# knights-lab/UTree

Hardware: AMD Instinct MI355X
Metric: reads classified/sec, 8 GB L2 CTR, 150 bp reads (higher is better)
Workload: dtype u64; 1 GPU; configs[1]: 1.22e+09-node synthetic L2 CTR (k=32, 21844 labels, image 40.8 GiB, fine_bits=8), 1152000000 x 150 bp reads per GPU (72 steps x 16000000-read batches, 41 distinct batches resident in HBM), RC=0

## Files before the change

### utree_amd/csrc/dev_image.c

```c
#define _FILE_OFFSET_BITS 64
#define _GNU_SOURCE
#define __HIP_PLATFORM_AMD__ 1
#include <hip/hip_runtime_api.h>
#include <fcntl.h>
#include <math.h>
#include <stddef.h>
#include <stdio.h>
#include <stdlib.h>
#include <string.h>
#include <unistd.h>
#include "ctr_host.h"
#include "dev_image.h"

#define HIPCHK(x) do { hipError_t e_ = (x); if (e_ != hipSuccess) { utree_dev_set_hip_error((int)e_, #x); rc = e_ == hipErrorOutOfMemory ? UTREE_E_NOMEM : UTREE_E_HIP; goto fail; } } while (0)
#define KCHK(x) do { int e_ = (x); if (e_ != 0) { utree_dev_set_hip_error(e_, #x); rc = e_ == (int)hipErrorOutOfMemory ? UTREE_E_NOMEM : UTREE_E_HIP; goto fail; } } while (0)

static __thread char g_hip_msg[256];
void utree_dev_set_hip_error(int err, const char *what) {
    snprintf(g_hip_msg, sizeof g_hip_msg, "%s (%d) in %s", hipGetErrorString((hipError_t)err), err, what);
    if (getenv("UTREE_DEBUG")) fprintf(stderr, "[utree_amd] HIP error: %s\n", g_hip_msg);
}
const char *utree_last_hip_error(void) { return g_hip_msg; }
void utree_set_error_text(const char *msg) { snprintf(g_hip_msg, sizeof g_hip_msg, "%s", msg); }

// ... 328 lines not shown
    if (e) { utree_dev_set_hip_error(e, "utk_repack"); return UTREE_E_HIP; }
    return UTREE_OK;
}

static int build_finish(builder *b, const void *d_binix_raw) {
    int rc = UTREE_OK;
    utree_dev *d = b->d;
    const utree_ctr *ctr = b->ctr;
    hipStream_t st = b->stream;
    char *img = (char *)d->image;
    uint64_t *recs = (uint64_t *)(img + d->hdr.off_recs);
    void *coarse = img + d->hdr.off_coarse;
    const int off64 = (d->hdr.flags & UTREE_F_OFF64) != 0;
    unsigned long long counters[2] = {0, 0}, invalid = 0;
    HIPCHK(hipMemcpyAsync(&invalid, b->d_invalid, 8, hipMemcpyDeviceToHost, st));
    HIPCHK(hipMalloc((void **)&b->d_counters, 16));
    HIPCHK(hipMemsetAsync(b->d_counters, 0, 16, st));
    KCHK(utk_fill_recs_pad(recs + d->hdr.n_nodes * d->hdr.rec_words, 8 * d->hdr.rec_words, st));
    KCHK(utk_widen_binix(d_binix_raw, ctr->info.binix_width, off64, coarse, st));
    KCHK(utk_validate(d->hdr.W, d->hdr.I, off64, coarse, recs, d->hdr.n_nodes, (uint32_t *)(img + d->hdr.off_irreg),
                      b->d_counters, st));
    HIPCHK(hipMemcpyAsync(counters, b->d_counters, 16, hipMemcpyDeviceToHost, st));
    HIPCHK(hipStreamSynchronize(st));
    if (timing_on()) fprintf(stderr, "[utree_amd] image: bin table checked (%llu irregular bins%s)\n", counters[0], counters[1] ? ", not monotone" : "");
    d->hdr.n_irregular = counters[0];
    if (invalid) d->hdr.flags |= UTREE_F_INVALID_RANKS;
    uint64_t full_bytes = d->hdr.total_bytes;
    if (d->hdr.W == 4) {
        uint64_t c0 = 0, cN = 0;
        if (!counters[1]) {
            if (ctr->info.binix_width == 4) { uint32_t a, z; memcpy(&a, ctr->binix_raw, 4); memcpy(&z, (const char *)ctr->binix_raw + 4 * (size_t)(UTREE_NUMBINS - 1), 4); c0 = a; cN = z; }
            else { memcpy(&c0, ctr->binix_raw, 8); memcpy(&cN, (const char *)ctr->binix_raw + 8 * (size_t)(UTREE_NUMBINS - 1), 8); }
        } else HIPCHK(hipMemsetAsync(img + d->hdr.off_irreg, 0xFF, (1u << 24) / 8, st));
        KCHK(utk_build_direct(d->hdr.I, off64, counters[1] != 0, coarse, recs, d->hdr.n_nodes, c0, cN - c0, (const uint32_t *)(img + d->hdr.off_irreg), counters[0],
                              img + d->hdr.off_table, st));
        HIPCHK(hipStreamSynchronize(st));
        if (counters[1]) d->hdr.flags |= UTREE_F_GENERIC; else if (counters[0]) d->hdr.flags |= UTREE_F_IRREGULAR;
        d->hdr.n_min = 0;
        d->hdr.total_bytes = d->hdr.off_recs;
        if (timing_on()) fprintf(stderr, "[utree_amd] image: direct-address table of 2^32 x %u bytes built (%llu irregular bins%s answered by the reference's probe order)\n",
                                 d->hdr.I, counters[0], counters[1] ? ", bin table not monotone: every bin" : "");
    } else
    if (counters[1]) {
        d->hdr.flags |= UTREE_F_GENERIC;
        d->hdr.fine_bits = 0;
        d->hdr.n_min = 0;
        HIPCHK(hipMemsetAsync(img + d->hdr.off_irreg, 0xFF, (1u << 24) / 8, st));
    } else {
        if (counters[0]) d->hdr.flags |= UTREE_F_IRREGULAR;
        uint64_t c0, cN;
        if (ctr->info.binix_width == 4) { uint32_t a, z; memcpy(&a, ctr->binix_raw, 4); memcpy(&z, (const char *)ctr->binix_raw + 4 * (size_t)(UTREE_NUMBINS - 1), 4); c0 = a; cN = z; }
        else { memcpy(&c0, ctr->binix_raw, 8); memcpy(&cN, (const char *)ctr->binix_raw + 8 * (size_t)(UTREE_NUMBINS - 1), 8); }
        d->hdr.n_min = cN - c0;
        HIPCHK(hipMemsetAsync(b->d_counters, 0, 16, st));
        HIPCHK(hipMemcpyAsync(img, &d->hdr, sizeof d->hdr, hipMemcpyHostToDevice, st));
        {
            uint64_t n_min = 0;
            int views = 0;
            KCHK(utk_build_min(d->hdr.W, d->hdr.I, off64, coarse, recs, c0, d->hdr.n_min, dup_capacity(d->hdr.n_nodes), (const uint64_t *)(img + offsetof(utree_image_header, regions)),
                               d->hdr.regions, d->hdr.n_slots, d->hdr.bucket_words, (uint64_t *)(img + d->hdr.off_table), (uint64_t *)(img + d->hdr.off_mrecs),
                               (uint32_t *)(img + d->hdr.off_irreg), b->d_counters, &n_min, &views, st));
            if (timing_on()) fprintf(stderr, "[utree_amd] image: %llu records for %llu nodes (second views%s)\n", (unsigned long long)n_min, (unsigned long long)d->hdr.n_min, views ? "" : ": too many, none stored");
            d->hdr.n_min = n_min;
            if (views) d->hdr.flags |= UTREE_F_STRAND_VIEWS;
        }
        KCHK(utk_fill_recs_pad((uint64_t *)(img + d->hdr.off_mrecs) + d->hdr.n_min * d->hdr.rec_words, 8 * d->hdr.rec_words, st));
        HIPCHK(hipMemcpyAsync(counters, b->d_counters, 16, hipMemcpyDeviceToHost, st));
        HIPCHK(hipStreamSynchronize(st));
        if (counters[0]) {
            d->hdr.flags |= UTREE_F_IRREGULAR;
            d->hdr.n_irregular += counters[1];
            if (timing_on()) fprintf(stderr, "[utree_amd] image: %llu bucket(s) beyond the overflow descriptor's range: %llu bins take the exact-probe path\n", counters[0], counters[1]);
        }
        {
            uint64_t kept = 0;
            const utree_image_header o = d->hdr;
            int chains = 0;
            KCHK(utk_compact_overflow(o.W, o.I, (uint64_t *)(img + o.off_table), o.n_slots, o.bucket_words, (uint64_t *)(img + o.off_mrecs), &kept, &chains, st));
            if (chains) d->hdr.flags |= UTREE_F_OVF_CHAINS;
            KCHK(utk_fill_recs_pad((uint64_t *)(img + o.off_mrecs) + kept * o.rec_words, 8 * o.rec_words, st));
            utree_image_header *h = &d->hdr;
            const uint64_t coarse_b = (uint64_t)UTREE_NUMBINS * ((o.flags & UTREE_F_OFF64) ? 8 : 4), irreg_b = (1u << 24) / 8;
            const uint64_t loff_b = ((uint64_t)o.n_labels + 1) * 4, blob_b = o.label_blob_bytes + 64, r2i_b = (uint64_t)o.n_labels * 4;
            const uint64_t vote_b = (uint64_t)o.n_labels * sizeof(utk_vote_rec);
            const uint64_t recs_b = (o.n_nodes + 8) * o.rec_words * 8;
            uint64_t off = align_up(o.off_mrecs + (kept + 8) * o.rec_words * 8, 4096);
            h->n_min = kept;
            h->off_coarse = off; off = align_up(off + coarse_b, 256);
            h->off_irreg = off; off = align_up(off + irreg_b, 256);
            h->off_label_off = off; off = align_up(off + loff_b, 256);
            h->off_label_blob = off; off = align_up(off + blob_b, 256);
            h->off_rank2ix = off; off = align_up(off + r2i_b, 256);
            h->off_vote = off; off = align_up(off + vote_b, 4096);
            h->off_recs = off;
            if (h->flags & UTREE_F_IRREGULAR) off = align_up(off + recs_b, 4096);
            h->total_bytes = off;
            if (move_down(img, h->off_coarse, o.off_coarse, coarse_b, st) || move_down(img, h->off_irreg, o.off_irreg, irreg_b, st) ||
                move_down(img, h->off_label_off, o.off_label_off, loff_b, st) || move_down(img, h->off_label_blob, o.off_label_blob, blob_b, st) ||
                move_down(img, h->off_rank2ix, o.off_rank2ix, r2i_b, st) || move_down(img, h->off_vote, o.off_vote, vote_b, st) ||
                ((h->flags & UTREE_F_IRREGULAR) && move_down(img, h->off_recs, o.off_recs, recs_b, st))) { rc = UTREE_E_HIP; goto fail; }
            HIPCHK(hipStreamSynchronize(st));
            if (timing_on()) fprintf(stderr, "[utree_amd] image: %llu of %llu nodes in overflow runs; packed image %.2f GiB (built in %.2f GiB)\n",
                                     (unsigned long long)kept, (unsigned long long)o.n_nodes, (double)h->total_bytes / 1073741824.0, (double)full_bytes / 1073741824.0);
        }
    }
    d->image_bytes = d->hdr.total_bytes;
    HIPCHK(hipMemcpyAsync(img, &d->hdr, sizeof d->hdr, hipMemcpyHostToDevice, st));
    HIPCHK(hipStreamSynchronize(st));
    if (d->owns && d->hdr.total_bytes + ((uint64_t)256 << 20) < full_bytes && !getenv("UTREE_KEEP_BUILD_AREA")) {
        void *small = NULL;
        if (hipMalloc(&small, d->hdr.total_bytes) == hipSuccess) {
            hipError_t e1 = hipMemcpyAsync(small, d->image, d->hdr.total_bytes, hipMemcpyDeviceToDevice, st), e2 = hipStreamSynchronize(st);
            if (e1 == hipSuccess && e2 == hipSuccess) { hipFree(d->image); d->image = small; }
            else { hipFree(small); (void)hipGetLastError(); }
        } else (void)hipGetLastError();
    }
    bind_image(d);
fail:
    if (b->d_counters) hipFree(b->d_counters);
    if (b->d_ix2rank) hipFree(b->d_ix2rank);
    if (b->d_invalid) hipFree(b->d_invalid);
    b->d_counters = NULL; b->d_ix2rank = NULL; b->d_invalid = NULL;
    if (rc) { utree_dev_free(d); b->d = NULL; }
    return rc;
}

int utree_dev_build(const utree_ctr *ctr, int device, int fine_bits, const void *d_binix, const void *d_records,
                    void *d_image, size_t image_bytes, void *stream, utree_dev **out) {
    if (!ctr || !d_binix || !d_records || !out) return UTREE_E_ARG;
    *out = NULL;
    builder b;
    int rc = build_begin(&b, ctr, device, fine_bits, d_image, image_bytes, (hipStream_t)stream);
    if (rc) return rc;
    rc = build_chunk(&b, d_records, 0, ctr->info.n_nodes);
    if (rc) { hipFree(b.d_ix2rank); hipFree(b.d_invalid); utree_dev_free(b.d); return rc; }
    rc = build_finish(&b, d_binix);
    if (rc) return rc;
    *out = b.d;
    return UTREE_OK;
}

static double g_upload_s[4];
int utree_dev_upload_seconds(double *h_out4) {
    if (!h_out4) return UTREE_E_ARG;
    for (int i = 0; i < 4; ++i) h_out4[i] = g_upload_s[i];
    return UTREE_OK;
}

int utree_dev_upload(const utree_ctr *ctr, int device, int fine_bits, utree_dev **out) {
    if (!ctr || !out) return UTREE_E_ARG;
    *out = NULL;
    if (!ctr->path && !ctr->h_records) return UTREE_E_ARG;
    builder b;
    double t0 = now_s();
    int rc = build_begin(&b, ctr, device, fine_bits, NULL, 0, NULL);
    if (rc) return rc;
    double t1 = now_s(), t2 = t1, t3 = t1;
    const size_t SZ = ctr->info.SZ;
    const size_t chunk_recs = ((size_t)128 << 20) / SZ;
    const size_t chunk_bytes = chunk_recs * SZ;
    void *h_pin[2] = {NULL, NULL}, *d_raw[2] = {NULL, NULL}, *d_binix = NULL;
    hipEvent_t ev[2] = {NULL, NULL};
    int fd = -1;
    for (int i = 0; i < 2; ++i) {
        HIPCHK(hipHostMalloc(&h_pin[i], chunk_bytes, hipHostMallocDefault));
        HIPCHK(hipMalloc(&d_raw[i], chunk_bytes));
        HIPCHK(hipEventCreateWithFlags(&ev[i], hipEventDisableTiming));
    }
    if (ctr->path) {
        fd = open(ctr->path, O_RDONLY);
        if (fd < 0) { rc = UTREE_E_IO; goto fail; }
    }
    uint64_t done = 0, N = ctr->info.n_nodes;
    for (int slot = 0; done < N; slot ^= 1) {
        uint64_t cnt = N - done < chunk_recs ? N - done : chunk_recs;
        size_t bytes = (size_t)cnt * SZ;
        HIPCHK(hipEventSynchronize(ev[slot]));
        if (fd >= 0) {
            int T = 8, bad = 0;
            if ((size_t)T > bytes / ((size_t)4 << 20) + 1) T = (int)(bytes / ((size_t)4 << 20) + 1);
#pragma omp parallel for num_threads(T) schedule(static, 1) reduction(| : bad)
            for (int t = 0; t < T; ++t) {
                size_t a = bytes * (size_t)t / (size_t)T, e = bytes * (size_t)(t + 1) / (size_t)T;
                while (a < e) {
                    ssize_t r = pread(fd, (char *)h_pin[slot] + a, e - a, (off_t)(ctr->records_file_off + done * SZ + a));
                    if (r <= 0) { bad |= 1; break; }
                    a += (size_t)r;
                }
            }
            if (bad) { rc = UTREE_E_FORMAT; goto fail; }
        } else memcpy(h_pin[slot], ctr->h_records + done * SZ, bytes);
        HIPCHK(hipMemcpyAsync(d_raw[slot], h_pin[slot], bytes, hipMemcpyHostToDevice, NULL));
        rc = build_chunk(&b, d_raw[slot], done, cnt);
        if (rc) goto fail;
        HIPCHK(hipEventRecord(ev[slot], NULL));
        done += cnt;
    }
    HIPCHK(hipDeviceSynchronize());
    t2 = now_s();
    if (timing_on()) fprintf(stderr, "[utree_amd] image: %llu nodes streamed and repacked in %.3f s\n", (unsigned long long)N, t2 - t1);
    HIPCHK(hipMalloc(&d_binix, (size_t)UTREE_NUMBINS * ctr->info.binix_width));
    HIPCHK(hipMemcpyAsync(d_binix, ctr->binix_raw, (size_t)UTREE_NUMBINS * ctr->info.binix_width, hipMemcpyHostToDevice, NULL));
    rc = build_finish(&b, d_binix);
    t3 = now_s();
    if (timing_on()) fprintf(stderr, "[utree_amd] image: alloc+labels %.3f s, stream+repack nodes %.3f s, validate+sort+table %.3f s\n", t1 - t0, t2 - t1, t3 - t2);
    g_upload_s[0] = t1 - t0; g_upload_s[1] = t2 - t1; g_upload_s[2] = t3 - t2; g_upload_s[3] = t3 - t0;
    if (!rc) *out = b.d;
    b.d = NULL;
fail:
    if (fd >= 0) close(fd);
    hipDeviceSynchronize();
    for (int i = 0; i < 2; ++i) {
        if (h_pin[i]) hipHostFree(h_pin[i]);
        if (d_raw[i]) hipFree(d_raw[i]);
        if (ev[i]) hipEventDestroy(ev[i]);
    }
    if (d_binix) hipFree(d_binix);
    if (rc && b.d) { if (b.d_ix2rank) hipFree(b.d_ix2rank); if (b.d_invalid) hipFree(b.d_invalid); utree_dev_free(b.d); }
    return rc;
}

int utree_dev_image(const utree_dev *dev, void **d_image, size_t *bytes) {
    if (!dev) return UTREE_E_ARG;
    if (d_image) *d_image = dev->image;
    if (bytes) *bytes = dev->image_bytes;
    return UTREE_OK;
}

int utree_dev_attach(const utree_ctr *ctr, int device, void *d_image, size_t bytes, utree_dev **out) {
    int rc = UTREE_OK, n_cu = 0;
    if (!d_image || !out || bytes < UTREE_IMG_HEADER_BYTES || ((uintptr_t)d_image & 127u)) return UTREE_E_ARG;
    *out = NULL;
    if ((rc = device_ok(device, &n_cu))) return rc;
    utree_dev *d = (utree_dev *)calloc(1, sizeof *d);
    if (!d) return UTREE_E_NOMEM;
    d->device = device; d->n_cu = n_cu; d->image = d_image; d->owns = 0;
    lanes_ring_init(d);
    HIPCHK(hipMemcpy(&d->hdr, d_image, sizeof d->hdr, hipMemcpyDeviceToHost));
    if (d->hdr.magic != UTREE_IMG_MAGIC || d->hdr.version != UTREE_IMG_VERSION || d->hdr.total_bytes > bytes ||
        (d->hdr.bucket_words != 8 && d->hdr.bucket_words != 16)) { rc = UTREE_E_FORMAT; goto fail; }
    if (ctr && (ctr->info.W != d->hdr.W || ctr->info.I != d->hdr.I || ctr->info.n_nodes != d->hdr.n_nodes ||
                ctr->info.n_labels != d->hdr.n_labels)) { rc = UTREE_E_ARG; goto fail; }
    d->image_bytes = d->hdr.total_bytes;
    bind_image(d);
    *out = d;
    return UTREE_OK;
fail:
    if (d->lanes_ring) hipHostFree((void *)d->lanes_ring);
    free(d);
    return rc;
}

static void lanes_ring_init(utree_dev *d) {
    void *p = NULL;
    if (hipSetDevice(d->device) == hipSuccess && hipHostMalloc(&p, 128 * sizeof(unsigned long long), hipHostMallocDefault) == hipSuccess) {
        memset(p, 0xFF, 128 * sizeof(unsigned long long));
        d->lanes_ring = (volatile unsigned long long *)p;
    }
}

void utree_dev_free(utree_dev *d) {
    if (!d) return;
    hipSetDevice(d->device);
    if (d->lanes_ring) hipHostFree((void *)d->lanes_ring);
    for (int i = 0; i < d->n_events; ++i) hipEventDestroy(d->events[i]);
    if (d->search_ctx) utree_search_ctx_free(d->search_ctx);
    if (d->owns && d->image) hipFree(d->image);
    if (d->rank_state) hipFree(d->rank_state);
    free(d);
}

int utree_dev_get_info(const utree_dev *d, utree_dev_info *info) {
    if (!d || !info) return UTREE_E_ARG;
    info->fine_bits = d->hdr.fine_bits;
    info->record_bytes = d->hdr.rec_words * 8;
    info->image_bytes = d->image_bytes;
    info->irregular_bins = d->hdr.n_irregular;
    info->generic_mode = (d->hdr.flags & UTREE_F_GENERIC) != 0;
    info->device = d->device;
    info->vote_table = d->kimg.vote_tab != NULL;
    info->lane_pass = utk_lanes_image_ok(&d->kimg) != 0;
    info->bucket_bytes = 8u * d->hdr.bucket_words;
    info->strand_views = (d->hdr.flags & UTREE_F_STRAND_VIEWS) ? 1u : 0u;
    if (d->hdr.flags & UTREE_F_DIRECT) info->bucket_bytes = 0;
    info->overflow_chains = (d->hdr.flags & UTREE_F_OVF_CHAINS) ? 1u : 0u;
    info->pad0 = 0;
    info->overflow_bytes = (d->hdr.flags & UTREE_F_DIRECT) ? 0 : d->hdr.n_min * d->hdr.rec_words * 8;
    return UTREE_OK;
}

#define LONG_BLOCKS_PER_CU 8

static uint32_t mid_limit(void) {
    static uint32_t v = 0;
    if (!v) {
        const char *e = getenv("UTREE_MID_LIMIT");
        v = UTREE_MID_DEFAULT;
        if (e && atoi(e) >= (int)UTREE_SHORT2_CAP && atoi(e) <= (int)UTREE_MID_CAP) v = (uint32_t)atoi(e);
    }
    return v;
}

static int lanes_enabled(void) { const char *e = getenv("UTREE_LANE_PASS"); return !(e && e[0] == '0'); }

static void ring_lock(utree_dev *d) { while (__atomic_test_and_set(&d->ring_busy, __ATOMIC_ACQUIRE)) ; }
static void ring_unlock(utree_dev *d) { __atomic_clear(&d->ring_busy, __ATOMIC_RELEASE); }

static void ring_collect(utree_dev *d) {
    if (!d->lanes_ring) return;
    ring_lock(d);
    for (unsigned i = 0; i < 64; ++i) {
        const unsigned long long left = d->lanes_ring[2 * i], err = d->lanes_ring[2 * i + 1];
        if (left == ~0ull || err == ~0ull) continue;
        d->lanes_ring[2 * i] = ~0ull; d->lanes_ring[2 * i + 1] = ~0ull;
        d->ring_inflight[i] = 0;
        if (err && !d->dev_error) d->dev_error = err;
        if (timing_on()) fprintf(stderr, "[utree_amd] batch report: %llu of %u reads left by the lane pass, error word %llu\n", left, d->lanes_ring_reads[i], err);
        if (d->lanes_ring_reads[i]) {
            if (left * 4 <= d->lanes_ring_reads[i]) { unsigned long long n = 0, l = 0; for (unsigned w = 0; w < UTREE_LANES_WINDOW; ++w) { n += d->win_reads[w]; l += d->win_left[w]; }
                if (n >= (1u << 18) && l * 4 > n) { memset(d->win_left, 0, sizeof d->win_left); memset(d->win_reads, 0, sizeof d->win_reads); } }
            const unsigned w = d->win_next++ % UTREE_LANES_WINDOW;
            d->win_left[w] = left; d->win_reads[w] = d->lanes_ring_reads[i];
        }
        d->lanes_ring_reads[i] = 0;
    }
    ring_unlock(d);
}
static int lanes_worth(utree_dev *d) {
    unsigned long long n = 0, l = 0;
    ring_lock(d);
    for (unsigned w = 0; w < UTREE_LANES_WINDOW; ++w) { n += d->win_reads[w]; l += d->win_left[w]; }
    int go = !(n >= (1u << 18) && l * 4 > n);
    if (!go && (++d->lanes_skipped & 7u) == 0) go = 1;
    ring_unlock(d);
    return go;
}
static int ring_post(utree_dev *d, const utk_workspace *w, uint32_t lane_reads, hipStream_t st) {
    if (!d->lanes_ring) return 0;
    ring_lock(d);
    unsigned slot = 64;
    for (unsigned k = 0; k < 64; ++k) {
        const unsigned c = (d->lanes_ring_next + k) & 63u;
        if (!d->ring_inflight[c]) { slot = c; break; }
    }
    if (slot < 64) { d->lanes_ring_next = slot + 1; d->ring_inflight[slot] = 1; d->lanes_ring_reads[slot] = lane_reads; }
    ring_unlock(d);
    if (slot == 64) {
        unsigned long long two[2] = {0, 0};
        if (hipMemcpyAsync(two, w->cursors + UTREE_CUR_MID, 16, hipMemcpyDeviceToHost, st) != hipSuccess || hipStreamSynchronize(st) != hipSuccess) return 1;
        ring_lock(d);
        if (two[1] && !d->dev_error) d->dev_error = two[1];
        ring_unlock(d);
        ring_collect(d);
        return 0;
    }
    if (hipMemcpyAsync((void *)&d->lanes_ring[2 * slot], w->cursors + UTREE_CUR_MID, 16, hipMemcpyDeviceToHost, st) != hipSuccess) {
        ring_lock(d);
        d->ring_inflight[slot] = 0; d->lanes_ring_reads[slot] = 0;
        ring_unlock(d);
        return 1;
    }
    return 0;
}

int utree_classify_poll(utree_dev *d) {
    if (!d) return UTREE_E_ARG;
    ring_collect(d);
    ring_lock(d);
    const unsigned long long e = d->dev_error;
    d->dev_error = 0;
    ring_unlock(d);
    if (e) {
        snprintf(g_hip_msg, sizeof g_hip_msg, "a batch's kernels reported error %llu (%s)", e,
                 e == UTREE_DEVERR_TALLY_CAP ? "tally lists beyond the workspace: total_bases / max_len did not describe the batch" :
                 e == UTREE_DEVERR_LONG_CAP ? "more long reads than the workspace holds" :
                 e == UTREE_DEVERR_PIECES_CAP ? "more pieces of long reads than the workspace holds" : "unknown");
        return UTREE_E_DEVICE;
    }
    return UTREE_OK;
}

static uint32_t lanes_long_min(const utree_dev *d, int do_rc) {
    const uint32_t a = utk_lanes_max_len(&d->kimg), b = do_rc ? (UTREE_MID_CAP - 1u) / 2u : UTREE_MID_CAP;
    return (a < b ? a : b) + 1u;
}

static void carve(const utree_dev *d, void *ws, uint32_t n_reads, uint64_t total_bases, uint32_t max_len, int do_rc,
                  utk_workspace *w, size_t *bytes) {
    uint64_t off = 0;
    char *b = (char *)ws;
    w->cursors = (unsigned long long *)(b + off); off = align_up(off + UTREE_CURSOR_BYTES, 256);
    const uint64_t waves_per_cu = 32 + 20 + 5 * 12;
    w->tally_cap = ((do_rc ? 2 : 1) * total_bases + (uint64_t)n_reads) * 9 / 8 + (uint64_t)d->n_cu * waves_per_cu * UTREE_TALLY_CHUNK + 4096;
    { const char *e = getenv("UTREE_TEST_TALLY_CAP"); if (e && atoll(e) > 0 && (uint64_t)atoll(e) < w->tally_cap) w->tally_cap = (uint64_t)atoll(e); }
    { uint64_t room = w->tally_cap; if (room < UTREE_TALLY_CHUNK) room = UTREE_TALLY_CHUNK; if (room < d->hdr.n_labels) room = d->hdr.n_labels;
      w->tally = (uint64_t *)(b + off); off = align_up(off + room * 8, 256); }
    w->long_list = (uint32_t *)(b + off); off = align_up(off + (uint64_t)n_reads * 4, 256);
    w->mid_list = (uint32_t *)(b + off); off = align_up(off + (uint64_t)n_reads * 4, 256);
    uint64_t max_total = do_rc ? 2 * (uint64_t)max_len + 1 : max_len;
    w->long_blocks = 0; w->hist = NULL; w->touch = NULL;
    w->short_cap = max_total > UTREE_SHORT_CAP ? UTREE_SHORT2_CAP : UTREE_SHORT_CAP;
    w->mid_reads = max_total > w->short_cap;
    w->mid_limit = mid_limit();
    const int lanes_img = utk_lanes_image_ok(&d->kimg);
    if (max_total > w->mid_limit || (lanes_img && max_len > utk_lanes_max_len(&d->kimg))) {
        w->long_blocks = (uint32_t)d->n_cu * LONG_BLOCKS_PER_CU;
        if (w->long_blocks > n_reads) w->long_blocks = n_reads;
        w->hist = (uint32_t *)(b + off); off = align_up(off + (uint64_t)w->long_blocks * d->hdr.n_labels * 4, 256);
        w->touch = (uint32_t *)(b + off); off = align_up(off + (uint64_t)w->long_blocks * ((d->hdr.n_labels + 31) / 32) * 4, 256);
    }
    w->pieces = NULL; w->ltab_rank = w->ltab_cnt = w->lflag = w->long_left = NULL; w->n_long_cap = 0; w->ltally_base = 0;
    w->cls_list = NULL; w->cls_stride = 0; w->n_pieces_cap = 0;
    if (lanes_img && max_len > UTREE_LANES_CAP) {
        w->cls_stride = (n_reads + 63u) & ~63u;
        w->cls_list = (uint32_t *)(b + off); off = align_up(off + (uint64_t)5 * w->cls_stride * 4, 256);
    }
    if (lanes_img && w->long_blocks) {
        uint64_t cap = total_bases / lanes_long_min(d, do_rc) + 1;
        if (cap > n_reads) cap = n_reads;
        const uint64_t piece_windows = 16ull * (UTREE_LANES_CAP - 4 * d->hdr.W + 1);
        const uint64_t n_pieces = total_bases / piece_windows + cap + 1;
        w->n_long_cap = (uint32_t)cap;
        w->n_pieces_cap = n_pieces;
        w->pieces = (uint64_t *)(b + off); off = align_up(off + n_pieces * 8, 256);
        w->ltab_rank = (uint32_t *)(b + off); off = align_up(off + cap * UTREE_LONG_SLOTS * 4, 256);
        w->ltab_cnt = (uint32_t *)(b + off); off = align_up(off + cap * UTREE_LONG_SLOTS * 4, 256);
        w->lflag = (uint32_t *)(b + off); off = align_up(off + cap * 4, 256);
        w->long_left = (uint32_t *)(b + off); off = align_up(off + cap * 4, 256);
        w->ltally_base = (uint64_t)((uint64_t *)(b + off) - w->tally); off = align_up(off + cap * UTREE_LONG_SLOTS * 8, 256);
        { const char *e = getenv("UTREE_TEST_LONG_CAP"); if (e && atoll(e) > 0 && (uint64_t)atoll(e) < w->n_long_cap) w->n_long_cap = (uint32_t)atoll(e); }
        { const char *e = getenv("UTREE_TEST_PIECES_CAP"); if (e && atoll(e) > 0 && (uint64_t)atoll(e) < w->n_pieces_cap) w->n_pieces_cap = (uint64_t)atoll(e); }
    }
    *bytes = (size_t)off;
}

size_t utree_classify_workspace_bytes(const utree_dev *dev, uint32_t n_reads, uint64_t total_bases, uint32_t max_len, int do_rc) {
    if (!dev) return 0;
    utk_workspace w; size_t bytes;
    carve(dev, NULL, n_reads, total_bases, max_len, do_rc, &w, &bytes);
    return bytes;
}

int utree_classify_batch(utree_dev *d, const uint8_t *d_bases, const uint64_t *d_off, const uint32_t *d_len,
                         uint32_t n_reads, uint64_t total_bases, uint32_t max_len, int do_rc, utree_result *d_out,
                         void *d_workspace, size_t workspace_bytes, void *stream) {
    int rc = UTREE_OK;
    if (!d || !d_out || (!d_workspace && n_reads)) return UTREE_E_ARG;
    if (!n_reads) return UTREE_OK;
    if (!d_bases || !d_off || !d_len) return UTREE_E_ARG;
    hipStream_t st = (hipStream_t)stream;
    utk_workspace w; size_t need;
    carve(d, d_workspace, n_reads, total_bases, max_len, do_rc, &w, &need);
    if (workspace_bytes < need) return UTREE_E_ARG;
    HIPCHK(hipSetDevice(d->device));
    HIPCHK(hipMemsetAsync(w.cursors, 0, UTREE_CURSOR_BYTES, st));
    if (w.long_blocks) {
        HIPCHK(hipMemsetAsync(w.hist, 0, (size_t)w.long_blocks * d->hdr.n_labels * 4, st));
        HIPCHK(hipMemsetAsync(w.touch, 0, (size_t)w.long_blocks * ((d->hdr.n_labels + 31) / 32) * 4, st));
    }
    hipEvent_t e0 = NULL, e1 = NULL;
    int tslot = -1;
    if (__atomic_load_n(&d->timing_on, __ATOMIC_ACQUIRE)) {
        tslot = __atomic_fetch_add(&d->n_claimed, 1, __ATOMIC_RELAXED);
        if (tslot >= 0 && tslot < UTREE_MAX_PENDING && 2 * tslot + 1 < d->n_events) { e0 = d->events[2 * tslot]; e1 = d->events[2 * tslot + 1]; }
        else tslot = -1;
    }
    ring_collect(d);
    const int lanes = lanes_enabled() && utk_lanes_image_ok(&d->kimg) && lanes_worth(d);
    if (lanes) {
        const int mixed = max_len > UTREE_LANES_CAP;
        d->last_long = w.long_blocks != 0; d->last_mid = 0; d->last_rc = do_rc; d->last_short_cap = w.short_cap;
        d->last_lanes = utk_lanes_segs(&d->kimg, max_len); d->last_mixed = mixed; d->last_pieces = w.long_blocks != 0;
        if (e0 && !w.long_blocks) HIPCHK(hipEventRecord(e0, st));
        if (!mixed) KCHK(utk_classify_lanes(&d->kimg, d_bases, d_off, d_len, n_reads, max_len, do_rc, d_out, &w, d->n_cu, st));
        else KCHK(utk_classify_lanes_mixed(&d->kimg, d_bases, d_off, d_len, n_reads, max_len, do_rc, d_out, &w, d->n_cu, st));
        if (w.long_blocks) {
            if (e0) HIPCHK(hipEventRecord(e0, st));
            HIPCHK(hipMemsetAsync(w.ltab_rank, 0xFF, (size_t)w.n_long_cap * UTREE_LONG_SLOTS * 4, st));
            HIPCHK(hipMemsetAsync(w.ltab_cnt, 0, (size_t)w.n_long_cap * UTREE_LONG_SLOTS * 4, st));
            HIPCHK(hipMemsetAsync(w.lflag, 0, (size_t)w.n_long_cap * 4, st));
            KCHK(utk_classify_long_pieces(&d->kimg, d_bases, d_off, d_len, do_rc, d_out, &w, d->n_cu, st));
            utk_workspace wl = w;
            wl.long_list = w.long_left;
            wl.long_blocks = w.long_blocks >= 8 ? w.long_blocks / 8 : 1;
            KCHK(utk_classify_long(&d->kimg, d_bases, d_off, d_len, do_rc, d_out, &wl, d->n_cu, st));
            if (e0) { HIPCHK(hipEventRecord(e1, st)); d->recorded[tslot] = 1; }
        }
        KCHK(utk_classify_listed(&d->kimg, d_bases, d_off, d_len, n_reads, max_len, do_rc, d_out, &w, d->n_cu, st));
        if (e0 && !w.long_blocks) { HIPCHK(hipEventRecord(e1, st)); d->recorded[tslot] = 1; }
    } else {
        const int dominant = w.long_blocks ? 2 : (w.mid_reads ? 1 : 0);
        d->last_long = dominant == 2; d->last_mid = dominant == 1; d->last_rc = do_rc; d->last_short_cap = w.short_cap;
        d->last_lanes = 0; d->last_mixed = 0; d->last_pieces = 0;
        if (w.mid_reads) KCHK(utk_route(d_len, n_reads, do_rc, &w, st));
        if (e0 && dominant == 0) HIPCHK(hipEventRecord(e0, st));
        KCHK(utk_classify_short(&d->kimg, d_bases, d_off, d_len, n_reads, do_rc, d_out, &w, d->n_cu, st));
        if (e0 && dominant == 0) { HIPCHK(hipEventRecord(e1, st)); d->recorded[tslot] = 1; }
        if (w.mid_reads) {
            if (e0 && dominant == 1) HIPCHK(hipEventRecord(e0, st));
            KCHK(utk_classify_mid(&d->kimg, d_bases, d_off, d_len, n_reads, do_rc, d_out, &w, d->n_cu, st));
            if (e0 && dominant == 1) { HIPCHK(hipEventRecord(e1, st)); d->recorded[tslot] = 1; }
        }
        if (w.long_blocks) {
            if (e0) HIPCHK(hipEventRecord(e0, st));
            KCHK(utk_classify_long(&d->kimg, d_bases, d_off, d_len, do_rc, d_out, &w, d->n_cu, st));
            if (e0) { HIPCHK(hipEventRecord(e1, st)); d->recorded[tslot] = 1; }
        }
    }
    KCHK(utk_vote(&d->kimg, d_out, &w, n_reads, st));
    if (ring_post(d, &w, lanes ? n_reads : 0, st)) { (void)hipGetLastError(); }
    { ring_lock(d); const unsigned long long pe = d->dev_error; ring_unlock(d);
      if (pe) { rc = UTREE_E_DEVICE; snprintf(g_hip_msg, sizeof g_hip_msg, "an earlier batch's kernels reported error %llu: utree_classify_poll returns (and clears) it", pe); } }
#ifdef UTREE_LANES_TIMERS
    { extern void utk_lanes_phase_dump(void); static int lcalls; if (++lcalls == 6) utk_lanes_phase_dump(); }
#endif
#ifdef UTREE_PHASE_TIMERS
    { extern void utk_phase_dump(void); static int calls; if (++calls == 12) utk_phase_dump(); }
#endif
fail:
    return rc;
}

int utree_lookup_words(utree_dev *d, const uint64_t *d_hi, const uint64_t *d_lo, uint64_t n, uint32_t *d_ix, void *stream) {
    int rc = UTREE_OK;
    if (!d || !d_lo || !d_ix) return UTREE_E_ARG;
    if (d->hdr.W == 16 && !d_hi) return UTREE_E_ARG;
    HIPCHK(hipSetDevice(d->device));
    KCHK(utk_lookup(&d->kimg, d_hi, d_lo, n, d_ix, (hipStream_t)stream));
fail:
    return rc;
}

const char *utree_classify_kernel_name(const utree_dev *dc) {
    if (!dc) return "";
    utree_dev *d = (utree_dev *)dc;
    if (d->last_lanes && d->last_pieces) {
        snprintf(d->kernel_sig, sizeof d->kernel_sig, "classify_lanes_k<%u, %u, 16, %s, 2, %u, %s>", d->hdr.W, d->hdr.I, d->kimg.irr_n ? "true" : "false", d->hdr.bucket_words / 8,
                 utk_lanes_both_strands(&d->kimg, d->last_rc) ? "true" : "false");
        return d->kernel_sig;
    }
    if (d->last_lanes && d->last_mixed) {
        snprintf(d->kernel_sig, sizeof d->kernel_sig, "classify_lanes_mixed_k<%u, %u, %s, %u, %s>", d->hdr.W, d->hdr.I, d->kimg.irr_n ? "true" : "false",
                 d->hdr.bucket_words / 8, utk_lanes_both_strands(&d->kimg, d->last_rc) ? "true" : "false");
        return d->kernel_sig;
    }
    if (d->last_lanes) {
        snprintf(d->kernel_sig, sizeof d->kernel_sig, "classify_lanes_k<%u, %u, 1, %s, 0, %u, %s>", d->hdr.W, d->hdr.I, d->kimg.irr_n ? "true" : "false",
                 d->hdr.bucket_words / 8, utk_lanes_both_strands(&d->kimg, d->last_rc) ? "true" : "false");
        return d->kernel_sig;
    }
    return d->last_long ? utk_classify_long_name(&d->kimg, d->kernel_sig, sizeof d->kernel_sig)
                        : utk_classify_short_name(&d->kimg, d->last_short_cap ? d->last_short_cap : UTREE_SHORT_CAP, d->last_mid, d->last_rc,
                                                  d->kernel_sig, sizeof d->kernel_sig);
}

int utree_model_counts(utree_dev *d, const uint8_t *d_bases, const uint64_t *d_off, const uint32_t *d_len, uint32_t n_reads,
                       int do_rc, uint64_t *h_counts5, void *stream) {
    int rc = UTREE_OK;
    unsigned long long *dc = NULL;
    if (!d || !d_bases || !d_off || !d_len || !h_counts5) return UTREE_E_ARG;
    HIPCHK(hipSetDevice(d->device));
    HIPCHK(hipMalloc((void **)&dc, 64));
    HIPCHK(hipMemsetAsync(dc, 0, 64, (hipStream_t)stream));
    KCHK(utk_model_counts(&d->kimg, d_bases, d_off, d_len, n_reads, do_rc, dc, stream));
    HIPCHK(hipMemcpyAsync(h_counts5, dc, 40, hipMemcpyDeviceToHost, (hipStream_t)stream));
    HIPCHK(hipStreamSynchronize((hipStream_t)stream));
fail:
    if (dc) hipFree(dc);
    return rc;
}

int utree_classify_kernel_time(utree_dev *d, int reset, double *ms_total, uint64_t *launches) {
    int rc = UTREE_OK;
    if (!d) return UTREE_E_ARG;
    HIPCHK(hipSetDevice(d->device));
    int claimed = __atomic_load_n(&d->n_claimed, __ATOMIC_RELAXED);
    if (claimed > UTREE_MAX_PENDING) claimed = UTREE_MAX_PENDING;
    for (int i = 0; i < claimed; ++i) {
        float ms = 0.f;
        if (!d->recorded[i]) continue;
        d->recorded[i] = 0;
        HIPCHK(hipEventSynchronize(d->events[2 * i + 1]));
        HIPCHK(hipEventElapsedTime(&ms, d->events[2 * i], d->events[2 * i + 1]));
        d->ms_total += ms; d->launches++;
    }
    while (d->n_events < 2 * UTREE_MAX_PENDING) { HIPCHK(hipEventCreate((hipEvent_t *)&d->events[d->n_events])); d->n_events++; }
    __atomic_store_n(&d->n_claimed, 0, __ATOMIC_RELAXED);
    if (ms_total) *ms_total = d->ms_total;
    if (launches) *launches = d->launches;
    if (reset) { d->ms_total = 0; d->launches = 0; }
    __atomic_store_n(&d->timing_on, 1, __ATOMIC_RELEASE);
fail:
    return rc;
}
```

### utree_amd/csrc/kernels.hip

```cpp
#include <hip/hip_runtime.h>
#include <stdint.h>
#include <stdio.h>
#include <string.h>
#include "device_common.hpp"
#include "wave_common.hpp"

using namespace utk;

namespace {

#ifdef UTREE_PHASE_TIMERS
__device__ unsigned long long g_phase[16];
struct PhaseT { unsigned long long t, acc[12]; };
#define PH_DECL PhaseT ph_; ph_.t = __builtin_readcyclecounter(); for (int q_ = 0; q_ < 12; ++q_) ph_.acc[q_] = 0;
#define TICKP(ph, i) do { const unsigned long long n_ = __builtin_readcyclecounter(); (ph).acc[i] += n_ - (ph).t; (ph).t = n_; } while (0)
#define TICK(i) TICKP(ph_, i)
#define PH_ARG , PhaseT &ph_
#define PH_PASS , ph_
#define PH_WAITVM asm volatile("s_waitcnt vmcnt(0)" ::: "memory")
#else
#define PH_DECL
#define TICK(i)
#define PH_ARG
#define PH_PASS
#define PH_WAITVM
#endif


constexpr uint32_t KEY_TILE = 128;

struct LaneBits {
    const uint32_t *swl;
    uint32_t sh;
};
__device__ __forceinline__ LaneBits lane_bits(const uint32_t *sw, uint32_t lane) {
    LaneBits b;
    const uint32_t r = lane & 15u;
    b.swl = sw + (lane >> 4) - (r == 0 ? 1u : 0u);
    b.sh = (32u - 2u * r) & 31u;
    return b;
}
__device__ __forceinline__ uint32_t mmer_l(const uint32_t *s, uint32_t word, uint32_t sh) {
    return __builtin_amdgcn_alignbit(s[word], s[word + 1], sh);
}

constexpr uint32_t MIN_POS_MASK = (1u << MIN_LOW_BITS) - 1u;
template <int W> struct MinWin { static constexpr uint32_t FIRST = UTREE_MIN_MARGIN(W), NEXT = (W == 16) ? 13u : 1u; };
template <int W, uint32_t NCH>
__device__ __forceinline__ void build_minkeys_n(const uint32_t *s, uint32_t sh, uint32_t *Kl, uint32_t *Hl, uint64_t *Ob, uint32_t lane) {
    uint32_t x[NCH];
#pragma unroll
    for (uint32_t c = 0; c < NCH; ++c) x[c] = mmer_l(s, 4 * c, sh);
    uint32_t lo = lane;
    asm volatile("" : "+v"(lo));
#pragma unroll
    for (uint32_t c = 0; c < NCH; ++c) {
        uint32_t o;
        const uint32_t h = canon_hash(x[c], o);
        Kl[c * 64] = ((h & ~MIN_POS_MASK) | lo) + c * 64;
        Hl[c * 64] = h;
        Ob[c] = __builtin_amdgcn_ballot_w64(o != 0u);
    }
    Kl[NCH * 64] = ~0u;
    wave_lds_fence();
#pragma unroll
    for (uint32_t st = 1; st <= ((W == 16) ? 16u : 8u); st <<= 1) {
        uint32_t a[NCH], b[NCH];
#pragma unroll
        for (uint32_t c = 0; c < NCH; ++c) { a[c] = Kl[c * 64]; b[c] = Kl[c * 64 + st]; }
        wave_lds_fence();
#pragma unroll
        for (uint32_t c = 0; c < NCH; ++c) Kl[c * 64] = b[c] < a[c] ? b[c] : a[c];
        wave_lds_fence();
    }
}
template <int W, uint32_t TILE>
__device__ __forceinline__ void build_minkeys(const uint32_t *s, uint32_t sh, uint32_t *Kl, uint32_t *Hl, uint64_t *Ob, uint32_t npos, uint32_t lane) {
    constexpr uint32_t MAXCH = (TILE + 4 * W - 16 + 63) / 64;
    static_assert(MAXCH <= 5, "tile too large");
    const uint32_t nch = (npos + 63) >> 6;
    if (nch <= 1) build_minkeys_n<W, 1>(s, sh, Kl, Hl, Ob, lane);
    else if (nch == 2) build_minkeys_n<W, 2>(s, sh, Kl, Hl, Ob, lane);
    else if (nch == 3 || MAXCH == 3) build_minkeys_n<W, 3>(s, sh, Kl, Hl, Ob, lane);
    else if (nch == 4) build_minkeys_n<W, MAXCH >= 4 ? 4 : 3>(s, sh, Kl, Hl, Ob, lane);
    else build_minkeys_n<W, MAXCH >= 5 ? 5 : 3>(s, sh, Kl, Hl, Ob, lane);
}

struct RegionLds { const uint64_t *reg; uint64_t table; uint32_t bshift; };

template <int W, int I, bool EXC, typename OFF, uint32_t TILE, bool CHECKBAD, typename HitFn>
__device__ __forceinline__ void wave_scan_windows(const utk_image &im, const LaneBits &lb, const uint64_t *sbad, uint64_t *Kk,
                                                  uint32_t w0, uint32_t n, const RegionLds &rg, uint32_t lane, HitFn &&on_rank PH_ARG) {
    constexpr uint32_t K = 4 * W;
    if constexpr (W == 4) {
        for (uint32_t it = 0; it * 64 < n; ++it) {
            bool ok = lane < n - it * 64;
            if constexpr (CHECKBAD) {
                const uint32_t ch = (w0 + it * 64) >> 6;
                const uint64_t b0 = sbad[ch], b1 = sbad[ch + 1];
                const uint64_t x = (b0 >> lane) | (lane ? (b1 << (64u - lane)) : 0ull);
                ok = ok && ((uint32_t)x & 0xFFFFu) == 0u;
            }
            uint32_t rank = INVALID;
            if (ok) rank = direct_rank<I>(im, mmer_l(lb.swl + ((w0 + it * 64) >> 4), 0, lb.sh));
            on_rank(rank);
        }
        return;
    }
    static_assert(TILE + 64 <= (1u << MIN_LOW_BITS), "tile positions must fit the key's position field");
    uint32_t *Kp = (uint32_t *)Kk;
    uint32_t *Kl = Kp + lane, *Hl = Kp + (TILE + 128) + lane;
    const uint32_t *Hh = Kp + (TILE + 128);
    uint64_t *Ob = Kk + (TILE + 128) - 8;
    static_assert(((TILE + 4 * W - 16 + 63) / 64) * 64 + 16 <= TILE + 128, "the ballots share the hash area");
    const uint32_t nlane = 0u - lane;
    for (uint32_t wb = 0; wb < n; wb += TILE) {
        const uint32_t tn = n - wb < TILE ? n - wb : TILE;
        const uint32_t *st = lb.swl + ((w0 + wb) >> 4);
        build_minkeys<W, TILE>(st, lb.sh, Kl, Hl, Ob, tn + K - 16, lane);
        TICK(2);
        auto locate = [&](uint32_t it, uint64_t &baddr, uint32_t &tag) {
            const uint32_t *Kr = Kl + it * 64;
            const uint32_t ka = Kr[MinWin<W>::FIRST], kb = Kr[MinWin<W>::FIRST + MinWin<W>::NEXT];
            const uint32_t p = (kb < ka ? kb : ka) & MIN_POS_MASK;
            const uint32_t h = Hh[p];
            const uint32_t o = (uint32_t)(Ob[p >> 6] >> (p & 63u)) & 1u;
            const uint32_t pos = p + nlane - it * 64;
            const uint64_t re = rg.reg[h >> 24];
            uint32_t bl = __umulhi(h << 8, (uint32_t)re & ((1u << UTREE_REGION_NB_BITS) - 1u));
            if constexpr (W == 16) {
                const uint32_t *sr = st + it * 4;
                const uint32_t x0 = mmer_l(sr, 0, lb.sh), x1 = mmer_l(sr, 1, lb.sh), x2 = mmer_l(sr, 2, lb.sh), x3 = mmer_l(sr, 3, lb.sh);
                const unsigned __int128 w = ((unsigned __int128)(((uint64_t)x0 << 32) | x1) << 64) | (((uint64_t)x2 << 32) | x3);
                const uint64_t v = (uint64_t)(w >> (92u - 2u * pos));
                const uint32_t sub = (uint32_t)(re >> UTREE_REGION_NB_BITS) & ((1u << UTREE_REGION_SUB_BITS) - 1u);
                bl = bl * sub + ((ext_canon((uint32_t)((v >> 32) & 0xF0u) | (uint32_t)(v & 0xFu), o) * sub) >> 8);
            }
            baddr = rg.table + ((2u * ((re >> UTREE_REGION_BASE_SHIFT) + bl) + o) << rg.bshift);
            tag = ((h & 0xFFu) << 6) | pos;
        };
        auto resolve = [&](uint32_t it, const Bucket<W, I> &bk, uint64_t baddr, uint32_t tag) -> uint32_t {
            const uint32_t *sr = st + it * 4;
            const uint32_t pos = tag & 63u, hlow = tag >> 6;
            if constexpr (W == 8) {
                const uint32_t x0 = mmer_l(sr, 0, lb.sh), x1 = mmer_l(sr, 1, lb.sh);
                const uint32_t M = (uint32_t)(0xFFFFFFFFull >> (2 * pos));
                const uint32_t rest = x0 ^ ((x0 ^ x1) & M);
                return resolve_bucket8<I, EXC, OFF>(im, bk, baddr, hlow, pos, rest, x0, x1);
            } else {
                const uint32_t x0 = mmer_l(sr, 0, lb.sh), x1 = mmer_l(sr, 1, lb.sh), x2 = mmer_l(sr, 2, lb.sh), x3 = mmer_l(sr, 3, lb.sh);
                const uint64_t wh = ((uint64_t)x0 << 32) | x1, wl = ((uint64_t)x2 << 32) | x3;
                uint32_t rh; uint64_t rl;
                min_rest<W>(wh, wl, pos, rh, rl);
                MinKey<W> mk;
                mk.lo = rl; mk.hi = ((uint64_t)hlow << 38) | ((uint64_t)pos << 32) | rh;
                return resolve_bucket<W, I, EXC, OFF>(im, bk, baddr, mk, wh, wl);
            }
        };
        auto window_ok = [&](uint32_t it, uint32_t left) -> bool {
            bool ok = lane < left;
            if constexpr (CHECKBAD) {
                const uint32_t ch = (w0 + wb + it * 64) >> 6;
                const uint64_t b0 = sbad[ch], b1 = sbad[ch + 1];
                const uint64_t x = (b0 >> lane) | (lane ? (b1 << (64u - lane)) : 0ull);
                ok = ok && ((K == 64) ? (x == 0) : ((uint32_t)x == 0));
            }
            return ok;
        };
        for (uint32_t it = 0; it * 64 < tn; ++it) {
            const bool ok = window_ok(it, tn - it * 64);
            uint64_t baddr = 0; uint32_t tag = 0;
            Bucket<W, I> bk;
            if (ok) { locate(it, baddr, tag); bk = load_bucket_at<W, I>(baddr); }
            TICK(3);
            PH_WAITVM;
            TICK(4);
            uint32_t rank = INVALID;
            if (ok) rank = resolve(it, bk, baddr, tag);
            TICK(5);
            on_rank(rank);
            TICK(6);
        }
        wave_lds_fence();
    }
}

__device__ __forceinline__ void stage_regions(const utk_image &im, uint64_t *s_reg) {
    for (uint32_t x = threadIdx.x; x < 256; x += blockDim.x) s_reg[x] = im.regions[x];
    __syncthreads();
}

__device__ __forceinline__ unsigned long long reserve_tally(const utk_workspace &ws, unsigned long long n) {
    unsigned long long nb = atomicAdd(&ws.cursors[0], n);
    if (nb + n > ws.tally_cap) { ws.cursors[UTREE_CUR_ERROR] = UTREE_DEVERR_TALLY_CAP; nb = 0; }
    return nb;
}

__device__ __forceinline__ void store_result(utree_result *out, uint32_t label, int32_t cut, uint32_t found,
                                             uint32_t uix, uint32_t sl, uint32_t ol) {
    uint32_t *o = (uint32_t *)out;
    uint32_t v0 = label, v1 = (uint32_t)cut, v2 = found, v3 = uix, v4 = sl, v5 = ol;
    asm volatile("" : "+v"(v0), "+v"(v1), "+v"(v2), "+v"(v3), "+v"(v4), "+v"(v5));
    o[0] = v0; o[1] = v1; o[2] = v2; o[3] = v3; o[4] = v4; o[5] = v5;
}

__global__ __launch_bounds__(256) void route_k(const uint32_t *__restrict__ len, uint32_t n_reads, int do_rc, utk_workspace ws) {
    const uint32_t r = blockIdx.x * blockDim.x + threadIdx.x;
    uint64_t total = 0;
    if (r < n_reads) total = do_rc ? 2 * (uint64_t)len[r] + 1 : len[r];
    const bool mid = total > ws.short_cap && total <= ws.mid_limit, lng = total > ws.mid_limit;
    const uint64_t mm = __ballot(mid), ml = __ballot(lng);
    const uint32_t lane = lane_id();
    if (mm) {
        unsigned long long b = 0;
        if (lane == 0) b = atomicAdd(&ws.cursors[UTREE_CUR_MID], (unsigned long long)__popcll(mm));
        b = __shfl(b, 0);
        if (mid) ws.mid_list[b + lanes_below(mm)] = r;
    }
    if (ml) {
        unsigned long long b = 0;
        if (lane == 0) b = atomicAdd(&ws.cursors[UTREE_CUR_LONG], (unsigned long long)__popcll(ml));
        b = __shfl(b, 0);
        if (lng) ws.long_list[b + lanes_below(ml)] = r;
    }
}

template <int CAP> struct RawBuf { static constexpr uint32_t DW = ((CAP / 4 + 1 + 63) / 64) * 64; };

__device__ __forceinline__ uint32_t low_bytes(uint32_t n) {
    return n >= 4u ? 0xFFFFFFFFu : ((1u << (8u * n)) - 1u);
}

template <int CAP>
__device__ __forceinline__ void fetch_raw(const uint8_t *__restrict__ bases, uint64_t o, uint32_t L, uint32_t *raw, uint32_t lane) {
    const uint32_t mf = (uint32_t)(uintptr_t)(bases + o) & 3u;
    const uint32_t nd = (L + mf + 3u) >> 2;
    const uint8_t *p = bases + o - mf;
    for (uint32_t d0 = 0; d0 < nd; d0 += 64) {
        const uint32_t d = d0 + lane;
        if (d < nd) {
            const uint8_t *src = p + 4ull * d;
            const uint32_t dst = (uint32_t)(uintptr_t)(__attribute__((address_space(3))) void *)(raw + 1 + d0);
            asm volatile("s_mov_b32 m0, %1\n\ts_nop 0\n\tglobal_load_lds_dword %0, off" : : "v"(src), "s"(dst) : "memory");
        }
    }
}

template <int CAP>
__device__ __forceinline__ bool stage_read(const uint32_t *raw, uint32_t mf, uint32_t L, uint32_t total, int do_rc,
                                           uint8_t *sb, uint8_t *sbadb, uint32_t lane) {
    constexpr uint32_t DW = RawBuf<CAP>::DW;
    const uint32_t ngroups = (total + 3u) >> 2;
    bool any = false;
    const uint32_t mr = (mf + 2u * L + 1u) & 3u;
    for (uint32_t g0 = 0; g0 < ngroups; g0 += 64) {
        const uint32_t g = g0 + lane;
        const uint32_t gi = g < DW ? g : DW - 1u;
        const uint32_t fm = low_bytes(4u * g < L ? L - 4u * g : 0u);
        uint32_t word = __builtin_amdgcn_alignbyte(raw[2u + gi], raw[1u + gi], mf) & fm;
        uint32_t rm = 0;
        if (do_rc) {
            int32_t i4 = ((int32_t)(mf + 2u * L) - 3 - (int32_t)(4u * g)) >> 2;
            i4 = i4 < -1 ? -1 : (i4 > (int32_t)DW - 1 ? (int32_t)DW - 1 : i4);
            const uint32_t w = __builtin_amdgcn_alignbyte(raw[2 + i4], raw[1 + i4], mr);
            const uint32_t rev = __builtin_amdgcn_perm(0u, w, 0x00010203u);
            const uint32_t from = L + 1u > 4u * g ? L + 1u - 4u * g : 0u, to = 2u * L + 1u > 4u * g ? 2u * L + 1u - 4u * g : 0u;
            rm = low_bytes(to) & ~low_bytes(from);
            word |= rev & rm;
        }
        const uint32_t g2 = (word >> 1) & 0x03030303u;
        const uint32_t letter = __builtin_amdgcn_perm(0u, 0x47544341u, g2);
        const uint32_t z = (word & 0xDFDFDFDFu) ^ letter;
        const uint32_t nz = (((z & 0x7F7F7F7Fu) + 0x7F7F7F7Fu) | z) & 0x80808080u;
        any = any || (nz & low_bytes(total > 4u * g ? total - 4u * g : 0u)) != 0u;
        const uint32_t nib = (nz * 0x00204081u) >> 28;
        const uint32_t nib_next = (uint32_t)__builtin_amdgcn_update_dpp(0, (int)nib, 0x101, 0xF, 0xF, true);
        uint32_t code = g2 ^ ((g2 >> 1) & 0x01010101u);
        code ^= rm & 0x03030303u;
        const uint32_t packed = (code * 0x40100401u) >> 24;
        if (g < ngroups) {
            sb[g ^ 3u] = (uint8_t)packed;
            if (!(lane & 1u)) sbadb[g >> 1] = (uint8_t)(nib | (nib_next << 4));
        }
    }
    return __ballot(any) != 0ull;
}

constexpr int SHORT_CAP = UTREE_SHORT_CAP;
constexpr int SHORT2_CAP = UTREE_SHORT2_CAP;
constexpr int MID_CAP = UTREE_MID_CAP;
constexpr int WAVES_PER_BLOCK = 4;
constexpr uint32_t WORK_GRAB = 32;
constexpr uint32_t TALLY_CHUNK = UTREE_TALLY_CHUNK;
constexpr uint32_t TALLY_DIRECT = UTREE_TALLY_CHUNK / 16;
constexpr int32_t CUT_PENDING = -3;
constexpr int32_t RANK_PENDING = -4;

constexpr int SHORT_MIN_WAVES = 8;
template <int W, int I, bool EXC, typename OFF, int CAP, bool LISTED, int RCMODE = 2>
__global__ __launch_bounds__(256, CAP > SHORT2_CAP ? (I == 2 ? 4 : 3) : (I == 2 ? SHORT_MIN_WAVES : 5))
void classify_short_k(utk_image im, const uint8_t *__restrict__ bases, const uint64_t *__restrict__ off,
                      const uint32_t *__restrict__ len, uint32_t n_reads, int do_rc_arg, utree_result *__restrict__ out,
                      utk_workspace ws) {
    if constexpr (LISTED) { if (!ws.cursors[UTREE_CUR_MID]) return; }
    const int do_rc = RCMODE == 2 ? do_rc_arg : RCMODE;
    constexpr uint32_t K = 4 * W;
    constexpr int NCH = CAP / 64, NWORDS = CAP / 16 + 6;
    __shared__ uint32_t s_words[WAVES_PER_BLOCK][NWORDS + 2];
// ... 31 lines not shown
        const uint32_t total_ = do_rc ? 2 * L_ + 1 : L_;
        asm volatile("s_waitcnt vmcnt(0)" ::: "memory");
        wave_lds_fence();
        const bool any_ = stage_read<CAP>(raw, (uint32_t)(uintptr_t)(bases + o_) & 3u, L_, total_, do_rc, sb, (uint8_t *)sbad, lane);
        if (lane == 0) sbad[(total_ + 63) >> 6] = ~0ull;
        wave_lds_fence();
        return any_;
    };
    auto finish = [&](uint32_t r, uint32_t F) {
            if (F == 0) { if (lane == 0) store_result(&out[r], 0, -2, 0, 0, 0, 0); return; }
            const uint32_t h0 = hits[0];
            if (F == 1) { if (lane == 0) store_result(&out[r], h0, RANK_PENDING, 1, 1, 0, 0); return; }
            if (F <= 64) {
                const bool mine = lane < F;
                const uint32_t hv = mine ? hits[lane] : 0u;
                uint64_t left = __ballot(mine);
                uint32_t nu = 0, myv = 0, myc = 0;
                while (left) {
                    const uint32_t lead = (uint32_t)__builtin_ctzll(left);
                    const uint32_t v = (uint32_t)__builtin_amdgcn_readlane((int)hv, (int)lead);
                    const uint64_t m = __ballot(mine && hv == v) & left;
                    if (lane == nu) { myv = v; myc = (uint32_t)__popcll(m); }
                    ++nu; left &= ~m;
                }
                if (nu == 1) { if (lane == 0) store_result(&out[r], h0, RANK_PENDING, F, 1, 0, 0); return; }
                if (nu > chunk_left) {
                    unsigned long long nb = 0;
                    if (lane == 0) nb = reserve_tally(ws, (unsigned long long)TALLY_CHUNK);
                    chunk_base = uni64(nb);
                    chunk_left = TALLY_CHUNK;
                }
                uint32_t place = 0;
                for (uint32_t u = 0; u < nu; ++u) place += (uint32_t)__builtin_amdgcn_readlane((int)myv, (int)u) < myv;
                if (lane < nu) ws.tally[chunk_base + place] = (uint64_t)myv | ((uint64_t)myc << 32);
                if (lane == 0) store_result(&out[r], 0, CUT_PENDING, F, nu, (uint32_t)chunk_base, (uint32_t)(chunk_base >> 32));
                chunk_base += nu; chunk_left -= nu;
                return;
            }
            uint32_t mn = INVALID, mx = 0;
            for (uint32_t j = lane; j < F; j += 64) { uint32_t h = hits[j]; mn = h < mn ? h : mn; mx = h > mx ? h : mx; }
            mn = wave_min_u32(mn);
            mx = ~wave_min_u32(~mx);
            if (mn == mx) { if (lane == 0) store_result(&out[r], h0, RANK_PENDING, F, 1, 0, 0); return; }
            unsigned long long base;
            const bool direct = (uint32_t)CAP >= TALLY_DIRECT && F >= TALLY_DIRECT;
            if (direct) {
                unsigned long long nb = 0;
                if (lane == 0) nb = reserve_tally(ws, (unsigned long long)F);
                base = uni64(nb);
            } else {
                if (F > chunk_left) {
                    unsigned long long nb = 0;
                    if (lane == 0) nb = reserve_tally(ws, (unsigned long long)TALLY_CHUNK);
                    chunk_base = uni64(nb);
                    chunk_left = TALLY_CHUNK;
                }
                base = chunk_base;
            }
            uint32_t uix = 0, cur = mn;
            for (;;) {
                uint32_t c = 0, nxt = INVALID;
                for (uint32_t j = lane; j < F; j += 64) {
                    uint32_t h = hits[j];
                    c += h == cur;
                    if (h > cur && h < nxt) nxt = h;
                }
                c = wave_sum_u32(c);
                nxt = wave_min_u32(nxt);
                if (lane == 0) ws.tally[base + uix] = (uint64_t)cur | ((uint64_t)c << 32);
                ++uix;
                if (nxt == INVALID) break;
                cur = nxt;
            }
            if (!direct) { chunk_base += uix; chunk_left -= uix; }
            if (lane == 0) store_result(&out[r], 0, CUT_PENDING, F, uix, (uint32_t)base, (uint32_t)(base >> 32));
    };
    uint32_t item = 0, item_end = 0;
    PH_DECL
    bool ahead = false;
    bool bad_cur = true, bad_next = true;
    uint32_t r = 0, L = 0;
    uint64_t o = 0;
    uint32_t grab0 = 0, g_r = 0, g_len = 0;
    uint64_t g_off = 0;
    auto params = [&](uint32_t it_, uint32_t &r_, uint32_t &L_, uint64_t &o_) {
        const int k_ = (int)(it_ - grab0);
        r_ = LISTED ? (uint32_t)__builtin_amdgcn_readlane((int)g_r, k_) : it_;
        L_ = (uint32_t)__builtin_amdgcn_readlane((int)g_len, k_);
        o_ = ((uint64_t)(uint32_t)__builtin_amdgcn_readlane((int)(uint32_t)(g_off >> 32), k_) << 32) |
             (uint32_t)__builtin_amdgcn_readlane((int)(uint32_t)g_off, k_);
    };
    static_assert(WORK_GRAB <= 64, "a grab's parameters live in the lanes of one register");
    for (;;) {
        if (item == item_end) {
            bool got = false;
            while (parts_left) {
                unsigned long long *ctr = parts + part * UTREE_WORK_STRIDE;
                const uint64_t lo = (uint64_t)part * part_len;
                const uint32_t avail = lo >= n_items ? 0u : (uint32_t)(n_items - lo < part_len ? n_items - lo : part_len);
                unsigned long long g = ~0ull;
                if (lane == 0 && __hip_atomic_load(ctr, __ATOMIC_RELAXED, __HIP_MEMORY_SCOPE_AGENT) < avail)
                    g = atomicAdd(ctr, (unsigned long long)WORK_GRAB);
                const uint32_t taken = uni32((uint32_t)(g > 0xFFFFFFFFull ? 0xFFFFFFFFull : g));
                if (taken < avail) {
                    item = (uint32_t)lo + taken;
                    item_end = taken + WORK_GRAB < avail ? item + WORK_GRAB : (uint32_t)lo + avail;
                    got = true;
                    break;
                }
                part = part + 1 == UTREE_WORK_PARTS ? 0 : part + 1;
                --parts_left;
            }
            if (!got) break;
            ahead = false;
            grab0 = item;
            if (item + lane < item_end) {
                g_r = LISTED ? ws.mid_list[item + lane] : item + lane;
                g_len = len[g_r]; g_off = off[g_r];
            }
            TICK(0);
        }
        if (!ahead) {
            params(item, r, L, o);
            if (stageable(L)) { fetch_raw<CAP>(bases, o, L, raw, lane); bad_cur = stage(o, L); }
        }
        ++item;
        ahead = PREFETCH && item < item_end;
        uint32_t r_next = 0, L_next = 0;
        uint64_t o_next = 0;
        bool stage_next = false;
        if (ahead) {
            params(item, r_next, L_next, o_next);
            stage_next = stageable(L_next);
            if (stage_next) fetch_raw<CAP>(bases, o_next, L_next, raw, lane);
        }
        TICK(1);
        const uint64_t total64 = do_rc ? 2 * (uint64_t)L + 1 : L;
        if (total64 <= (uint64_t)CAP) {
            const uint32_t total = (uint32_t)total64;
            uint32_t F = 0;
            if (total >= K) {
                auto on_rank = [&](uint32_t rank) {
                    const bool hit = rank != INVALID;
                    const uint64_t hm = __ballot(hit);
                    if (hit) hits[F + lanes_below(hm)] = (HIT)rank;
                    F += (uint32_t)__popcll(hm);
                };
                if constexpr (RCMODE == 1) wave_scan_windows<W, I, EXC, OFF, TILE, true>(im, lb, sbad, Kk, 0u, total - K + 1, rg, lane, on_rank PH_PASS);
                else if (!bad_cur) wave_scan_windows<W, I, EXC, OFF, TILE, false>(im, lb, sbad, Kk, 0u, total - K + 1, rg, lane, on_rank PH_PASS);
                else wave_scan_windows<W, I, EXC, OFF, TILE, true>(im, lb, sbad, Kk, 0u, total - K + 1, rg, lane, on_rank PH_PASS);
                wave_lds_fence();
            }
            TICK(9);
            if (stage_next) bad_next = stage(o_next, L_next);
            TICK(7);
            finish(r, F);
            TICK(8);
        } else if (stage_next) bad_next = stage(o_next, L_next);
        r = r_next; L = L_next; o = o_next; bad_cur = bad_next;
    }
#ifdef UTREE_PHASE_TIMERS
    if (lane == 0) { for (int q = 0; q < 12; ++q) atomicAdd(&g_phase[q], ph_.acc[q]); atomicAdd(&g_phase[12], 1ull); }
#endif
}

constexpr int LONG_TILE = 2048;
constexpr int LONG_THREADS = 256;
constexpr uint32_t LONG_LDS_BITWORDS = 2048;

template <int W, int I, bool EXC, typename OFF>
__global__ __launch_bounds__(LONG_THREADS, EXC ? 5 : 8) void classify_long_k(utk_image im, const uint8_t *__restrict__ bases,
                                                                const uint64_t *__restrict__ off,
                                                                const uint32_t *__restrict__ len, int do_rc,
                                                                utree_result *__restrict__ out, utk_workspace ws) {
    constexpr uint32_t K = 4 * W;
    constexpr uint32_t STAGE = LONG_TILE + 64;
    __shared__ uint32_t s_words_pad[STAGE / 16 + 8 + 2];
    __shared__ uint64_t s_bad[STAGE / 64 + 2];
    __shared__ uint32_t s_scan[LONG_THREADS / 64 + 1];
    __shared__ uint32_t s_touch[LONG_LDS_BITWORDS];
    __shared__ uint64_t s_keys[LONG_THREADS / 64][KEY_TILE + 128];
    __shared__ unsigned long long s_base;
    __shared__ uint64_t s_reg[256];
    __shared__ uint32_t s_work, s_single;
    const uint32_t tid = threadIdx.x, lane = tid & 63u, wv = uni32(tid >> 6);
    uint32_t *s_words = s_words_pad + 2;
    uint8_t *sb = (uint8_t *)s_words;
    const LaneBits lb = lane_bits(s_words, lane);
    const uint32_t nl = im.n_labels, nbw = (nl + 31) >> 5;
    uint32_t *hist = ws.hist + (size_t)blockIdx.x * nl;
    uint32_t *touch = nbw <= LONG_LDS_BITWORDS ? s_touch : ws.touch + (size_t)blockIdx.x * nbw;
    const uint32_t n_long = (uint32_t)ws.cursors[UTREE_CUR_LONG];
    if (nbw <= LONG_LDS_BITWORDS) for (uint32_t x = tid; x < nbw; x += LONG_THREADS) s_touch[x] = 0;
    stage_regions(im, s_reg);
    const RegionLds rg = {s_reg, (uint64_t)(uintptr_t)im.table, im.bucket_words == 16u ? 7u : 6u};

    for (;;) {
        __syncthreads();
        if (tid == 0) s_work = (uint32_t)atomicAdd(&ws.cursors[UTREE_CUR_WORK_LONG], 1ull);
        __syncthreads();
        const uint32_t li = s_work;
        if (li >= n_long) break;
        const uint32_t r = ws.long_list[li];
        const uint64_t L64 = len[r];
        const uint64_t o = off[r];
        const uint64_t total = do_rc ? 2 * L64 + 1 : L64;
        const uint64_t nwin = total >= K ? total - K + 1 : 0;
        uint32_t my_hits = 0;
        if (tid == 0) s_single = INVALID;
        for (uint64_t w0 = 0; w0 < nwin; w0 += LONG_TILE) {
            constexpr uint32_t NW = LONG_THREADS / 64, PER = (STAGE / 64 + NW - 1) / NW;
            uint32_t rawb[PER];
#pragma unroll
            for (uint32_t q = 0; q < PER; ++q) {
                const uint32_t c = wv + q * NW;
                const uint64_t j = w0 + (uint64_t)c * 64 + lane;
                rawb[q] = 0x200u;
                if (c < STAGE / 64) {
                    if (j < L64) rawb[q] = bases[o + j];
                    else if (j > L64 && j < total) rawb[q] = 0x100u | bases[o + (2 * L64 - j)];
                }
            }
#pragma unroll
            for (uint32_t q = 0; q < PER; ++q) {
                const uint32_t c = wv + q * NW;
                if (c >= STAGE / 64) break;
                uint32_t code = 0; bool bad = true;
                if (!(rawb[q] & 0x200u)) { base_code(rawb[q] & 0xFFu, code, bad); code ^= (rawb[q] >> 8) * 3u; }
                uint64_t bm = __ballot(bad);
                uint32_t t = (code << 2) | (uint32_t)__shfl_down((int)code, 1);
                uint32_t u = (t << 4) | (uint32_t)__shfl_down((int)t, 2);
                if ((lane & 3u) == 0) sb[(c * 16 + (lane >> 2)) ^ 3u] = (uint8_t)u;
                if (lane == 0) s_bad[c] = bm;
            }
            if (tid == 0) s_bad[STAGE / 64] = ~0ull;
            __syncthreads();
            const uint32_t tile_n = (uint32_t)(nwin - w0 < LONG_TILE ? nwin - w0 : LONG_TILE);
            constexpr uint32_t PER_WAVE = LONG_TILE / (LONG_THREADS / 64);
            const uint32_t a = wv * PER_WAVE < tile_n ? wv * PER_WAVE : tile_n;
            const uint32_t b = a + PER_WAVE < tile_n ? a + PER_WAVE : tile_n;
            PH_DECL
            wave_scan_windows<W, I, EXC, OFF, KEY_TILE, true>(im, lb, s_bad, s_keys[wv], a, b - a, rg, lane, [&](uint32_t rank) {
                const bool hit = rank != INVALID;
                uint64_t left = __ballot(hit);
                my_hits += hit;
                while (left) {
                    const uint32_t lead = (uint32_t)__builtin_ctzll(left);
                    const uint32_t v = (uint32_t)__builtin_amdgcn_readlane((int)rank, (int)lead);
                    const uint64_t m = __ballot(hit && rank == v) & left;
                    if (lane == lead) {
                        atomicAdd(&hist[v], (uint32_t)__popcll(m));
                        atomicOr(&touch[v >> 5], 1u << (v & 31u));
                    }
                    left &= ~m;
                }
            } PH_PASS);
            __syncthreads();
        }
        uint32_t f = wave_sum_u32(my_hits);
        if (lane == 0) s_scan[wv] = f;
        __syncthreads();
        uint32_t F = 0;
        for (uint32_t w = 0; w < LONG_THREADS / 64; ++w) F += s_scan[w];
        __syncthreads();
        if (F == 0) { if (tid == 0) store_result(&out[r], 0, -2, 0, 0, 0, 0); continue; }
        const uint32_t per = (nbw + LONG_THREADS - 1) / LONG_THREADS;
        const uint32_t lo = tid * per < nbw ? tid * per : nbw, hi = lo + per < nbw ? lo + per : nbw;
        uint32_t cnt = 0;
        for (uint32_t x = lo; x < hi; ++x) cnt += (uint32_t)__popc(__hip_atomic_load(&touch[x], __ATOMIC_RELAXED, __HIP_MEMORY_SCOPE_AGENT));
        uint32_t inc = cnt;
#pragma unroll
        for (int d = 1; d < 64; d <<= 1) { uint32_t t = __shfl_up(inc, d); if (lane >= (uint32_t)d) inc += t; }
        if (lane == 63) s_scan[wv] = inc;
        __syncthreads();
        uint32_t wbase = 0, uix = 0;
        for (uint32_t w = 0; w < LONG_THREADS / 64; ++w) { if (w < wv) wbase += s_scan[w]; uix += s_scan[w]; }
        uint32_t pos = wbase + inc - cnt;
        if (tid == 0) s_base = uix > 1 ? reserve_tally(ws, (unsigned long long)uix) : 0ull;
        __syncthreads();
        const unsigned long long base = s_base;
        for (uint32_t x = lo; x < hi; ++x) {
            uint32_t bits = __hip_atomic_load(&touch[x], __ATOMIC_RELAXED, __HIP_MEMORY_SCOPE_AGENT);
            if (!bits) continue;
            __hip_atomic_store(&touch[x], 0u, __ATOMIC_RELAXED, __HIP_MEMORY_SCOPE_AGENT);
            while (bits) {
                const uint32_t rk = x * 32 + (uint32_t)__builtin_ctz(bits);
                bits &= bits - 1;
                const uint32_t c = __hip_atomic_load(&hist[rk], __ATOMIC_RELAXED, __HIP_MEMORY_SCOPE_AGENT);
                __hip_atomic_store(&hist[rk], 0u, __ATOMIC_RELAXED, __HIP_MEMORY_SCOPE_AGENT);
                if (uix > 1) ws.tally[base + pos] = (uint64_t)rk | ((uint64_t)c << 32);
                else s_single = rk;
                ++pos;
            }
        }
        __syncthreads();
        if (tid == 0) {
            if (uix == 1) store_result(&out[r], im.rank2ix[s_single], -2, F, 1, 0, 0);
            else store_result(&out[r], 0, CUT_PENDING, F, uix, (uint32_t)base, (uint32_t)(base >> 32));
        }
        __syncthreads();
    }
}

__device__ __forceinline__ uint32_t cut_of(uint32_t x) {
    uint32_t c = x - x / 4;
    c += (x >> 1) >= c;
    return c;
}

__device__ __forceinline__ void label16(const char *s, uint32_t p, uint64_t &x, uint64_t &y) {
    typedef unsigned long long u64x2 __attribute__((ext_vector_type(2), aligned(1)));
    const u64x2 v = *(const u64x2 *)(s + p);
    x = v.x; y = v.y;
}

__device__ __forceinline__ uint64_t stop_flags(uint64_t x1, uint64_t x2) {
    const uint64_t semi = x1 ^ 0x3B3B3B3B3B3B3B3Bull, d = x1 ^ x2;
    uint64_t m = (((x1 - 0x0101010101010101ull) & ~x1) | ((semi - 0x0101010101010101ull) & ~semi)) & 0x8080808080808080ull;
    m |= (((d & 0x7F7F7F7F7F7F7F7Full) + 0x7F7F7F7F7F7F7F7Full) | d) & 0x8080808080808080ull;
    return m;
}

__device__ __forceinline__ void pair_scan(const char *s1, const char *s2, uint32_t start, uint32_t &td, uint32_t &a, uint32_t &b, uint32_t &before) {
    uint32_t base = start, prevlast = start ? (uint32_t)(uint8_t)s1[start - 1] : 0u;
    for (;;) {
        uint64_t x1, y1, x2, y2;
        label16(s1, base, x1, y1); label16(s2, base, x2, y2);
        uint64_t m = stop_flags(x1, x2);
        if (!m) { prevlast = (uint32_t)(x1 >> 56); base += 8; x1 = y1; x2 = y2; m = stop_flags(x1, x2); }
        if (m) {
            const uint32_t idx = (uint32_t)(__builtin_ctzll(m) >> 3);
            td = base + idx;
            a = (uint32_t)(x1 >> (8 * idx)) & 0xFFu; b = (uint32_t)(x2 >> (8 * idx)) & 0xFFu;
            before = idx ? ((uint32_t)(x1 >> (8 * idx - 8)) & 0xFFu) : prevlast;
            return;
        }
        prevlast = (uint32_t)(x1 >> 56); base += 8;
    }
}

struct VRec { uint64_t w[4]; };
__device__ __forceinline__ VRec vrec(const uint64_t *vt, uint32_t rank) {
    typedef unsigned long long u64x2 __attribute__((ext_vector_type(2)));
    const u64x2 *p = (const u64x2 *)(vt + (size_t)rank * 4);
    const u64x2 a = p[0], b = p[1];
    VRec v; v.w[0] = a.x; v.w[1] = a.y; v.w[2] = b.x; v.w[3] = b.y;
    return v;
}
__device__ __forceinline__ uint32_t v_pid(const VRec &v, uint32_t t) { return (uint32_t)((t < 4 ? v.w[0] : v.w[1]) >> (16u * (t & 3u))) & 0xFFFFu; }
__device__ __forceinline__ uint32_t v_end(const VRec &v, uint32_t t) { return (uint32_t)(v.w[2] >> (8u * t)) & 0xFFu; }
__device__ __forceinline__ bool v_exists(const VRec &v, uint32_t t) { return ((uint32_t)v.w[3] >> t) & 1u; }
__device__ __forceinline__ bool v_more(const VRec &v, uint32_t t) { return ((uint32_t)v.w[3] >> (8u + t)) & 1u; }
__device__ __forceinline__ bool v_us(const VRec &v, uint32_t t) { return ((uint32_t)v.w[3] >> (16u + t)) & 1u; }
__device__ __forceinline__ uint32_t v_len(const VRec &v) { return (uint32_t)(v.w[3] >> 32) & 0xFFu; }
__device__ __forceinline__ uint32_t v_ix(const VRec &v) { return (uint32_t)(v.w[3] >> 48); }

__device__ __forceinline__ void vote_table(const utk_image &im, utree_result *out_r, const uint64_t *T, uint32_t F, uint32_t uix) {
    const uint64_t *vt = im.vote_tab;
    const char *blob = im.label_blob;
    const uint32_t *loff = im.label_off;
    constexpr uint32_t NONE = 0xFFFFFFFFu;
    uint32_t cutoff = cut_of(F);
    uint32_t st = 0, ed = uix, dv = NONE, t = 0, orun = F, sl, ol;
    uint32_t ix_last, n_last, len_last;
    for (;;) {
        const uint64_t t_st = T[st];
        VRec pv = vrec(vt, (uint32_t)t_st);
        const uint64_t t_ed = ed - 1u == st ? t_st : T[ed - 1u];
        const VRec lv = ed - 1u == st ? pv : vrec(vt, (uint32_t)t_ed);
        {
            const uint64_t d0 = pv.w[0] ^ lv.w[0], d1 = pv.w[1] ^ lv.w[1];
            const uint32_t same = d0 ? (uint32_t)__builtin_ctzll(d0) >> 4 : 4u + (d1 ? (uint32_t)__builtin_ctzll(d1) >> 4 : 4u);
            const uint32_t both = ((uint32_t)(pv.w[3] & lv.w[3]) >> 8) & 0xFFu;
            const uint32_t semis = (uint32_t)__builtin_ctz(~both);
            const uint32_t L = same < semis ? same : semis;
            if (L > t) { dv = v_end(pv, L - 1u); t = L; }
        }
        uint32_t run = (uint32_t)(t_st >> 32), td = dv, c1 = run, rp = (uint32_t)t_st;
        bool td_is_end = false;
        bool stopped = false;
        for (uint32_t z = st + 1; z < ed; ++z) {
            const bool is_last = z == ed - 1u;
            const uint64_t tz = is_last ? t_ed : T[z];
            const uint32_t nz = (uint32_t)(tz >> 32), rc = (uint32_t)tz;
            const VRec cv = is_last ? lv : vrec(vt, rc);
            bool aside = false, stop = false;
            if (t >= 8u || !v_exists(pv, t) || (dv == NONE && v_end(pv, 0) == 0u && !v_more(pv, 0))) aside = true;
            else {
                uint32_t a, b, before;
                bool known = true;
                if (v_exists(cv, t) && v_pid(cv, t) == v_pid(pv, t)) {
                    td = v_end(pv, t); td_is_end = true;
                    a = v_more(pv, t) ? ';' : 0u; b = v_more(cv, t) ? ';' : 0u; before = v_us(pv, t) ? '_' : 'x';
                } else if (v_us(pv, t) || !v_exists(cv, t)) {
                    pair_scan(blob + loff[rp], blob + loff[rc], dv + 1u, td, a, b, before);
                    td_is_end = td == v_end(pv, t);
                } else { a = 'a'; b = 'b'; before = 'x'; known = false; }
                if (a == b) run += nz;
                else if ((!a && b == ';') || ((a == ';' || !a) && before == '_')) aside = true;
                else if (run >= cutoff) {
                    ed = z; stop = true;
                    if (!known) {
                        pair_scan(blob + loff[rp], blob + loff[rc], dv + 1u, td, a, b, before);
                        td_is_end = td == v_end(pv, t);
                    }
                } else { run = nz; st = z; }
            }
            if (aside) {
                run = nz; st = z;
                orun -= c1;
                cutoff = cut_of(orun);
            }
            if (stop) { stopped = true; break; }
            pv = cv; c1 = nz; rp = rc;
        }
        ix_last = stopped ? v_ix(pv) : v_ix(lv);
        n_last = stopped ? c1 : (uint32_t)(t_ed >> 32);
        len_last = stopped ? v_len(pv) : v_len(lv);
        sl = run; ol = orun;
        if (run < cutoff) break;
        if (st + 1 >= ed) {
            if (n_last >= cutoff) dv = 0xFFFFFFFEu;
            break;
        }
        orun = run; cutoff = cut_of(run);
        if (td != dv) { dv = td; if (td_is_end) ++t; }
    }
    int32_t cut;
    if (dv == NONE) cut = -1;
    else if (dv == 0xFFFFFFFEu) cut = -2;
    else cut = (int32_t)(dv < len_last ? dv : len_last);
    store_result(out_r, ix_last, cut, F, uix, sl, ol);
}

__global__ __launch_bounds__(256) void vote_table_k(utk_image im, utree_result *__restrict__ out, utk_workspace ws, uint32_t n_reads) {
    __shared__ uint32_t s_n[2][4];
    __shared__ uint16_t s_who[256];
    const uint32_t tid = threadIdx.x, wv = tid >> 6, lane = tid & 63u;
    const uint32_t r0 = blockIdx.x * blockDim.x + tid;
    uint32_t cls = 2;
    if (r0 < n_reads) {
        const uint32_t *res = (const uint32_t *)&out[r0];
        const int32_t cut = (int32_t)res[1];
        if (cut == RANK_PENDING) {
            uint32_t *o = (uint32_t *)&out[r0];
            o[0] = im.rank2ix[res[0]]; o[1] = (uint32_t)-2;
        } else if (cut == CUT_PENDING) cls = res[3] == 2u ? 0u : 1u;
    }
    const uint64_t m0 = __builtin_amdgcn_ballot_w64(cls == 0u), m1 = __builtin_amdgcn_ballot_w64(cls == 1u);
    s_who[tid] = 0xFFFFu;
    if (lane == 0) { s_n[0][wv] = (uint32_t)__popcll(m0); s_n[1][wv] = (uint32_t)__popcll(m1); }
    __syncthreads();
    if (cls < 2u) {
        uint32_t before = 0;
        for (uint32_t w = 0; w < wv; ++w) before += s_n[cls][w];
        before += (uint32_t)__popcll((cls ? m1 : m0) & ((1ull << lane) - 1ull));
        s_who[cls ? 255u - before : before] = (uint16_t)tid;
    }
    __syncthreads();
    const uint32_t who = s_who[tid];
    if (who == 0xFFFFu) return;
    const uint32_t r = blockIdx.x * blockDim.x + who;
    const uint32_t *res = (const uint32_t *)&out[r];
    vote_table(im, &out[r], ws.tally + ((uint64_t)res[4] | ((uint64_t)res[5] << 32)), res[2], res[3]);
}

__global__ __launch_bounds__(256) void vote_k(utk_image im, utree_result *__restrict__ out, utk_workspace ws, uint32_t n_reads) {
    const uint32_t r = blockIdx.x * blockDim.x + threadIdx.x;
    if (r >= n_reads) return;
    const uint32_t *res = (const uint32_t *)&out[r];
    if ((int32_t)res[1] == RANK_PENDING) {
        uint32_t *o = (uint32_t *)&out[r];
        o[0] = im.rank2ix[res[0]]; o[1] = (uint32_t)-2;
        return;
    }
    if ((int32_t)res[1] != CUT_PENDING) return;
    const uint32_t F = res[2], uix = res[3];
    const uint64_t *T = ws.tally + ((uint64_t)res[4] | ((uint64_t)res[5] << 32));
    const char *blob = im.label_blob;
    const uint32_t *loff = im.label_off;
    uint32_t cutoff = cut_of(F);
    uint32_t st = 0, ed = uix, dv = 0xFFFFFFFFu, orun = F, sl, ol;
    for (;;) {
        const uint64_t t_st = T[st];
        {
            const char *sa = blob + loff[(uint32_t)t_st], *sz = blob + loff[(uint32_t)T[ed - 1]];
            uint32_t base = dv + (dv == 0xFFFFFFFFu), q = 0xFFFFFFFFu;
            bool first = dv != 0xFFFFFFFFu;
            for (;;) {
                uint64_t a[2], b[2];
                label16(sa, base, a[0], a[1]); label16(sz, base, b[0], b[1]);
                bool stop = false;
#pragma unroll
                for (int h = 0; h < 2; ++h) {
                    const uint64_t x = a[h], d = a[h] ^ b[h], sx = a[h] ^ 0x3B3B3B3B3B3B3B3Bull;
                    uint64_t end = ((x - 0x0101010101010101ull) & ~x) & 0x8080808080808080ull;
                    end |= (((d & 0x7F7F7F7F7F7F7F7Full) + 0x7F7F7F7F7F7F7F7Full) | d) & 0x8080808080808080ull;
                    uint64_t semi = ~(((sx & 0x7F7F7F7F7F7F7F7Full) + 0x7F7F7F7F7F7F7F7Full) | sx) & 0x8080808080808080ull;
                    if (h == 0 && first) { end &= ~0xFFull; semi &= ~0xFFull; }
                    if (end) semi &= (end & (0ull - end)) - 1ull;
                    if (semi) q = base + 8u * (uint32_t)h + ((63u - (uint32_t)__builtin_clzll(semi)) >> 3);
                    if (end) { stop = true; break; }
                }
                if (stop) break;
                base += 16; first = false;
            }
            if (q != 0xFFFFFFFFu) dv = q;
        }
        uint32_t run = (uint32_t)(t_st >> 32), td = dv;
        const char *s1 = blob + loff[(uint32_t)t_st];
        uint32_t c1 = run;
        const uint32_t probe = dv + (dv == 0xFFFFFFFFu);
        const bool skip0 = dv != 0xFFFFFFFFu;
        uint64_t x1_first, y1_first;
        label16(s1, probe, x1_first, y1_first);
        for (uint32_t z = st + 1; z < ed; ++z) {
            const uint64_t tz = T[z];
            const uint32_t nz = (uint32_t)(tz >> 32);
            const char *s2 = blob + loff[(uint32_t)tz];
            uint64_t x1 = x1_first, y1 = y1_first;
            uint64_t x2_first, y2_first;
            label16(s2, probe, x2_first, y2_first);
            bool aside = false, stop = false;
            if (!(x1 & 0xFFull)) aside = true;
            else {
                uint64_t x2 = x2_first, y2 = y2_first;
                uint32_t base = probe, idx, prevlast = 0;
                bool first = true;
                for (;;) {
                    uint64_t m = stop_flags(x1, x2);
                    if (first && skip0) m &= ~0xFFull;
                    if (m) { idx = (uint32_t)(__builtin_ctzll(m) >> 3); break; }
                    prevlast = (uint32_t)(x1 >> 56);
                    base += 8; first = false;
                    m = stop_flags(y1, y2);
                    x1 = y1; x2 = y2;
                    if (m) { idx = (uint32_t)(__builtin_ctzll(m) >> 3); break; }
                    prevlast = (uint32_t)(x1 >> 56);
                    base += 8;
                    label16(s1, base, x1, y1); label16(s2, base, x2, y2);
                }
                td = base + idx;
                const uint32_t a = (uint32_t)(x1 >> (8 * idx)) & 0xFFu, b = (uint32_t)(x2 >> (8 * idx)) & 0xFFu;
                const uint32_t before = idx ? ((uint32_t)(x1 >> (8 * idx - 8)) & 0xFFu) : (first ? 0u : prevlast);
                if (a == b) run += nz;
                else if ((!a && b == ';') || ((a == ';' || !a) && before == '_')) aside = true;
                else if (run >= cutoff) { ed = z; stop = true; }
                else { run = nz; st = z; }
            }
            if (aside) {
                run = nz; st = z;
                orun -= c1;
                cutoff = cut_of(orun);
            }
            if (stop) break;
            s1 = s2; c1 = nz; x1_first = x2_first; y1_first = y2_first;
        }
        sl = run; ol = orun;
        if (run < cutoff) break;
        if (st + 1 >= ed) {
            if ((uint32_t)(T[ed - 1] >> 32) >= cutoff) dv = 0xFFFFFFFEu;
            break;
        }
        orun = run; dv = td; cutoff = cut_of(run);
    }
    const uint32_t rk = (uint32_t)T[ed - 1];
    int32_t cut;
    if (dv == 0xFFFFFFFFu) cut = -1;
    else if (dv == 0xFFFFFFFEu) cut = -2;
    else { uint32_t Ls = loff[rk + 1] - loff[rk] - 1; cut = (int32_t)(dv < Ls ? dv : Ls); }
    store_result(&out[r], im.rank2ix[rk], cut, F, uix, sl, ol);
}

template <int W, int I, bool EXC, typename OFF>
__global__ void lookup_k(utk_image im, const uint64_t *__restrict__ hi, const uint64_t *__restrict__ lo, uint64_t n,
                         uint32_t *__restrict__ ix) {
    for (uint64_t i = (uint64_t)blockIdx.x * blockDim.x + threadIdx.x; i < n; i += (uint64_t)gridDim.x * blockDim.x) {
        uint32_t rank = lookup_word<W, I, EXC, OFF>(im, W == 16 ? hi[i] : 0ull, lo[i]);
        ix[i] = rank == INVALID ? INVALID : im.rank2ix[rank];
    }
}

constexpr uint32_t MODEL_CAP = 640;
template <int W, int I>
__global__ __launch_bounds__(256) void model_k(utk_image im, const uint8_t *__restrict__ bases, const uint64_t *__restrict__ off,
                                               const uint32_t *__restrict__ len, uint32_t n_reads, int do_rc,
                                               unsigned long long *__restrict__ counts) {
    constexpr uint32_t K = 4 * W;
    __shared__ uint64_t s_b[4][MODEL_CAP];
    const uint32_t lane = lane_id(), wv = threadIdx.x >> 6;
    unsigned long long c_reads = 0, c_win = 0, c_buck = 0, c_line = 0, c_over = 0;
    for (uint32_t r = blockIdx.x * 4 + wv; r < n_reads; r += gridDim.x * 4) {
        const uint32_t L = len[r];
        const uint64_t o = off[r];
        const uint64_t total = do_rc ? 2ull * L + 1 : L;
        ++c_reads;
        if (total < K) continue;
        const uint64_t nwin_all = total - K + 1;
        for (uint64_t w0 = 0; w0 < nwin_all; w0 += MODEL_CAP) {
            const uint32_t nwin = (uint32_t)(nwin_all - w0 < MODEL_CAP ? nwin_all - w0 : MODEL_CAP);
            for (uint32_t i = lane; i < nwin; i += 64) {
                uint64_t khi = 0, klo = 0;
                bool ok = true;
                for (uint64_t j = w0 + i; j < w0 + i + K; ++j) {
                    uint32_t code = 0; bool bad = true;
                    if (j < L) base_code(bases[o + j], code, bad);
                    else if (j > L) { base_code(bases[o + (2ull * L - j)], code, bad); code ^= 3u; }
                    ok = ok && !bad;
                    khi = (khi << 2) | (klo >> 62); klo = (klo << 2) | code;
                }
                uint64_t bucket = ~0ull;
                if (ok) { MinKey<W> mk; min_split<W>(W == 16 ? khi : 0ull, klo, im.regions, bucket, mk); }
                s_b[wv][i] = bucket;
            }
            wave_lds_fence();
            for (uint32_t i = lane; i < nwin; i += 64) {
                const uint64_t b = s_b[wv][i];
                if (b == ~0ull) continue;
                ++c_win;
                bool first_b = true, first_l = true;
                for (uint32_t j = 0; j < i; ++j) { const uint64_t x = s_b[wv][j]; first_b = first_b && x != b; }
                if (im.bucket_words == 16u) first_l = first_b;
                else for (uint32_t j = 0; j < i; ++j) { const uint64_t x = s_b[wv][j]; first_l = first_l && (x == ~0ull || (x >> 1) != (b >> 1)); }
                c_buck += first_b; c_line += first_l;
                if (first_b) {
                    constexpr int EW = RecTraits<W, I>::EW, KW = RecTraits<W, I>::KW;
                    c_over += (im.table[b * im.bucket_words + (uint64_t)(im.bucket_words / EW - 1) * EW + KW] >> 62) == 2;
                }
            }
            wave_lds_fence();
        }
    }
    unsigned long long v[4] = {c_win, c_buck, c_line, c_over};
#pragma unroll
    for (int q = 0; q < 4; ++q) {
        unsigned long long x = v[q];
#pragma unroll
        for (int d = 32; d > 0; d >>= 1) x += __shfl_xor(x, d);
        if (lane == 0 && x) atomicAdd(&counts[1 + q], x);
    }
    if (lane == 0 && c_reads) atomicAdd(&counts[0], c_reads);
}

}

extern "C" {

int utk_classify_short(const utk_image *im, const uint8_t *d_bases, const uint64_t *d_off, const uint32_t *d_len,
                       uint32_t n_reads, int do_rc, utree_result *d_out, const utk_workspace *ws, int n_cu, void *stream) {
    if (!n_reads) return 0;
    uint32_t blocks = (n_reads + WAVES_PER_BLOCK - 1) / WAVES_PER_BLOCK;
    uint32_t cap = (uint32_t)n_cu * 8u;
    if (blocks > cap) blocks = cap;
    return dispatch_img_all(im, [&](auto w, auto i, auto exc, auto offt) {
        if (ws->short_cap == UTREE_SHORT2_CAP)
            classify_short_k<decltype(w)::value, decltype(i)::value, decltype(exc)::value, decltype(offt), SHORT2_CAP, false>
                <<<dim3(blocks), dim3(256), 0, (hipStream_t)stream>>>(*im, d_bases, d_off, d_len, n_reads, do_rc, d_out, *ws);
        else if (do_rc)
            classify_short_k<decltype(w)::value, decltype(i)::value, decltype(exc)::value, decltype(offt), SHORT_CAP, false, 1>
                <<<dim3(blocks), dim3(256), 0, (hipStream_t)stream>>>(*im, d_bases, d_off, d_len, n_reads, do_rc, d_out, *ws);
        else
            classify_short_k<decltype(w)::value, decltype(i)::value, decltype(exc)::value, decltype(offt), SHORT_CAP, false, 0>
                <<<dim3(blocks), dim3(256), 0, (hipStream_t)stream>>>(*im, d_bases, d_off, d_len, n_reads, do_rc, d_out, *ws);
    });
}

int utk_route(const uint32_t *d_len, uint32_t n_reads, int do_rc, const utk_workspace *ws, void *stream) {
    if (!n_reads) return 0;
    route_k<<<dim3((n_reads + 255) / 256), dim3(256), 0, (hipStream_t)stream>>>(d_len, n_reads, do_rc, *ws);
    return (int)hipGetLastError();
}

int utk_classify_mid(const utk_image *im, const uint8_t *d_bases, const uint64_t *d_off, const uint32_t *d_len,
                     uint32_t n_reads, int do_rc, utree_result *d_out, const utk_workspace *ws, int n_cu, void *stream) {
    if (!n_reads) return 0;
    uint32_t blocks = (n_reads + WAVES_PER_BLOCK - 1) / WAVES_PER_BLOCK;
    uint32_t cap = (uint32_t)n_cu * 5u;
    if (blocks > cap) blocks = cap;
    return dispatch_img_all(im, [&](auto w, auto i, auto exc, auto offt) {
        classify_short_k<decltype(w)::value, decltype(i)::value, decltype(exc)::value, decltype(offt), MID_CAP, true>
            <<<dim3(blocks), dim3(256), 0, (hipStream_t)stream>>>(*im, d_bases, d_off, d_len, n_reads, do_rc, d_out, *ws);
    });
}

int utk_classify_listed(const utk_image *im, const uint8_t *d_bases, const uint64_t *d_off, const uint32_t *d_len,
                        uint32_t n_reads, uint32_t max_len, int do_rc, utree_result *d_out, const utk_workspace *ws, int n_cu, void *stream) {
    if (!n_reads) return 0;
    uint32_t blocks = (n_reads + WAVES_PER_BLOCK - 1) / WAVES_PER_BLOCK;
    uint32_t cap = (uint32_t)n_cu * 2u;
    if (blocks > cap) blocks = cap;
    const uint64_t total = do_rc ? 2ull * max_len + 1 : max_len;
    return dispatch_img(im, [&](auto w, auto i, auto exc, auto offt) {
        if (total > SHORT2_CAP)
            classify_short_k<decltype(w)::value, decltype(i)::value, decltype(exc)::value, decltype(offt), MID_CAP, true>
                <<<dim3(blocks), dim3(256), 0, (hipStream_t)stream>>>(*im, d_bases, d_off, d_len, n_reads, do_rc, d_out, *ws);
        else if (do_rc || total > SHORT_CAP)
            classify_short_k<decltype(w)::value, decltype(i)::value, decltype(exc)::value, decltype(offt), SHORT2_CAP, true>
                <<<dim3(blocks), dim3(256), 0, (hipStream_t)stream>>>(*im, d_bases, d_off, d_len, n_reads, do_rc, d_out, *ws);
        else
            classify_short_k<decltype(w)::value, decltype(i)::value, decltype(exc)::value, decltype(offt), SHORT_CAP, true, 0>
                <<<dim3(blocks), dim3(256), 0, (hipStream_t)stream>>>(*im, d_bases, d_off, d_len, n_reads, do_rc, d_out, *ws);
    });
}

int utk_classify_long(const utk_image *im, const uint8_t *d_bases, const uint64_t *d_off, const uint32_t *d_len,
                      int do_rc, utree_result *d_out, const utk_workspace *ws, int n_cu, void *stream) {
    (void)n_cu;
    if (!ws->long_blocks) return 0;
    return dispatch_img_all(im, [&](auto w, auto i, auto exc, auto offt) {
        classify_long_k<decltype(w)::value, decltype(i)::value, decltype(exc)::value, decltype(offt)>
            <<<dim3(ws->long_blocks), dim3(LONG_THREADS), 0, (hipStream_t)stream>>>(*im, d_bases, d_off, d_len, do_rc, d_out, *ws);
    });
}

int utk_vote(const utk_image *im, utree_result *d_out, const utk_workspace *ws, uint32_t n_reads, void *stream) {
    if (!n_reads) return 0;
    if (im->vote_tab) vote_table_k<<<dim3((n_reads + 255) / 256), dim3(256), 0, (hipStream_t)stream>>>(*im, d_out, *ws, n_reads);
    else vote_k<<<dim3((n_reads + 255) / 256), dim3(256), 0, (hipStream_t)stream>>>(*im, d_out, *ws, n_reads);
    return (int)hipGetLastError();
}

int utk_lookup(const utk_image *im, const uint64_t *d_hi, const uint64_t *d_lo, uint64_t n, uint32_t *d_ix, void *stream) {
    if (!n) return 0;
    uint64_t blocks = (n + 255) / 256;
    if (blocks > 8192) blocks = 8192;
    return dispatch_img_all(im, [&](auto w, auto i, auto exc, auto offt) {
        lookup_k<decltype(w)::value, decltype(i)::value, decltype(exc)::value, decltype(offt)>
            <<<dim3((unsigned)blocks), dim3(256), 0, (hipStream_t)stream>>>(*im, d_hi, d_lo, n, d_ix);
    });
}

#ifdef UTREE_PHASE_TIMERS
void utk_phase_dump(void) {
    unsigned long long h[16];
    static const char *nm[12] = {"grab", "next read's len/off + fetch issue", "minimizers", "round: address (LDS chain) + load issue", "round: wait for the bucket",
                                 "round: scan", "round: hit compaction", "stage next read (waits for its bytes)", "tally + result", "after windows", "", ""};
    if (hipDeviceSynchronize() != hipSuccess || hipMemcpyFromSymbol(h, HIP_SYMBOL(g_phase), sizeof h) != hipSuccess) return;
    unsigned long long tot = 0;
    for (int q = 0; q < 12; ++q) tot += h[q];
    fprintf(stderr, "[phase timers] %llu waves, %.3g cycles per wave\n", h[12], h[12] ? (double)tot / h[12] : 0.0);
    for (int q = 0; q < 10; ++q) fprintf(stderr, "  %-45s %5.1f %%\n", nm[q], tot ? 100.0 * h[q] / tot : 0.0);
    memset(h, 0, sizeof h);
    (void)hipMemcpyToSymbol(HIP_SYMBOL(g_phase), h, sizeof h);
}
#endif

int utk_model_counts(const utk_image *im, const uint8_t *d_bases, const uint64_t *d_off, const uint32_t *d_len, uint32_t n_reads,
                     int do_rc, unsigned long long *d_counts, void *stream) {
    if (!n_reads) return 0;
    uint32_t blocks = (n_reads + 3) / 4;
    if (blocks > 4096) blocks = 4096;
    return dispatch_wi(im->W, im->I, [&](auto w, auto i) {
        model_k<decltype(w)::value, decltype(i)::value><<<dim3(blocks), dim3(256), 0, (hipStream_t)stream>>>(*im, d_bases, d_off, d_len, n_reads,
                                                                                                      do_rc, d_counts);
    });
}

static const char *kernel_signature(char *buf, size_t cap, const char *name, const utk_image *im, int slice, int listed, int rcmode) {
    const bool exc = (im->flags & (UTREE_F_IRREGULAR | UTREE_F_GENERIC)) != 0, o64 = (im->flags & UTREE_F_OFF64) != 0;
    if (slice) snprintf(buf, cap, "%s<%u, %u, %s, %s, %d, %s, %d>", name, im->W, im->I, exc ? "true" : "false", o64 ? "unsigned long" : "unsigned int",
                        slice, listed ? "true" : "false", rcmode);
    else snprintf(buf, cap, "%s<%u, %u, %s, %s>", name, im->W, im->I, exc ? "true" : "false", o64 ? "unsigned long" : "unsigned int");
    return buf;
}
const char *utk_classify_short_name(const utk_image *im, uint32_t short_cap, int mid, int do_rc, char *buf, size_t cap) {
    if (mid) return kernel_signature(buf, cap, "classify_short_k", im, MID_CAP, 1, 2);
    if (short_cap == UTREE_SHORT2_CAP) return kernel_signature(buf, cap, "classify_short_k", im, SHORT2_CAP, 0, 2);
    return kernel_signature(buf, cap, "classify_short_k", im, SHORT_CAP, 0, do_rc ? 1 : 0);
}
const char *utk_classify_long_name(const utk_image *im, char *buf, size_t cap) { return kernel_signature(buf, cap, "classify_long_k", im, 0, 0, 0); }

}
```

### utree_amd/csrc/lanes_core.hpp

```cpp
#pragma once
#include <hip/hip_runtime.h>
#include <stdint.h>
#include <stdio.h>
#include <string.h>
#include "device_common.hpp"
#include "wave_common.hpp"

using namespace utk;

namespace {

#ifdef UTREE_LANES_TIMERS
__device__ unsigned long long g_lphase[8];
#define LT_DECL unsigned long long lt_t = __builtin_readcyclecounter(), lt_acc[6] = {0, 0, 0, 0, 0, 0};
#define LT(i) do { const unsigned long long n_ = __builtin_readcyclecounter(); lt_acc[i] += n_ - lt_t; lt_t = n_; } while (0)
#else
#define LT_DECL
#define LT(i)
#endif

constexpr int LANES_WAVES = 4;
constexpr int LANES_WPS = 3;
constexpr uint32_t LCAP = UTREE_LANES_CAP;
constexpr uint32_t NWORD = LCAP / 16;
static_assert(LCAP % 32 == 0, "slot geometry");
static_assert(LCAP + 16 + 48 <= 256, "positions are 8-bit fields of a run record");
template <int W> struct Geo {
    static constexpr uint32_t K = 4 * W, OFS = UTREE_MIN_MARGIN(W), NB = K - 15 - 2 * OFS;
    static constexpr uint32_t NA = W == 16 ? 3 : 1;
    static constexpr uint32_t FRONT = NA;
    static constexpr uint32_t STRIDE = NWORD + FRONT + 2;
    static constexpr uint32_t RUNS = W == 16 ? 512 : 1280;
    static constexpr uint32_t DNONE = 63;
    static_assert((STRIDE & 1) == 1, "slot geometry");
};
constexpr uint32_t TSLOTS = 12;
constexpr uint32_t T_EMPTY = 0xFFFFFFFFu;
constexpr int32_t CUT_PENDING = -3, RANK_PENDING = -4;

__device__ __forceinline__ uint32_t low_bytes(uint32_t n) { return n >= 4u ? 0xFFFFFFFFu : ((1u << (8u * n)) - 1u); }
__device__ __forceinline__ uint64_t ballot64(bool p) { return __builtin_amdgcn_ballot_w64(p); }
__device__ __forceinline__ uint32_t umin(uint32_t a, uint32_t b) { return a < b ? a : b; }
__device__ __forceinline__ uint32_t wave_max_u32(uint32_t v) { return ~wave_min_u32(~v); }

__device__ __forceinline__ void store_result(utree_result *out, uint32_t label, int32_t cut, uint32_t found, uint32_t uix, uint32_t sl, uint32_t ol) {
    uint32_t *o = (uint32_t *)out;
    o[0] = label; o[1] = (uint32_t)cut; o[2] = found; o[3] = uix; o[4] = sl; o[5] = ol;
}

typedef const __attribute__((address_space(1))) uint32_t *gptr32;


__device__ __forceinline__ void rest96(const uint32_t (&A)[3], const uint32_t (&B)[3], uint32_t pos, uint32_t &r0, uint32_t &r1, uint32_t &r2) {
    const uint32_t sh = 2u * pos, bs = sh & 31u;
    const bool w1 = (sh & 32u) != 0u, w2 = (sh & 64u) != 0u;
    const uint32_t v[6] = {A[0], A[1], A[2], B[0], B[1], B[2]};
    uint32_t y[6];
#pragma unroll
    for (int t = 0; t < 6; ++t) y[t] = w1 ? (t ? v[t - 1] : 0u) : v[t];
    uint32_t x[4];
#pragma unroll
    for (int i = 0; i < 4; ++i) x[i] = w2 ? y[i] : y[2 + i];
    r0 = __builtin_amdgcn_alignbit(x[0], x[1], bs); r1 = __builtin_amdgcn_alignbit(x[1], x[2], bs); r2 = __builtin_amdgcn_alignbit(x[2], x[3], bs);
}

template <int W, int I, int SEGS, bool IRR, int MODE, int NL, bool BS>
__device__ __forceinline__ void lanes_body(const utk_image &im, const uint8_t *__restrict__ bases, const uint64_t *__restrict__ off, const uint32_t *__restrict__ len,
                                           uint32_t n_reads, const int do_rc, utree_result *__restrict__ out, const utk_workspace &ws, const uint32_t cls,
                                           uint32_t *stream, uint32_t *runs, uint32_t *tab, uint32_t *full, uint32_t *pref, uint64_t *ost, const uint64_t *s_reg,
                                           const uint32_t wv) {
    constexpr bool PIECE = MODE == 2, LISTED = MODE == 1;
    static_assert(!BS || NL == 1, "both strands in one pass: 64-byte buckets");
    constexpr int NLX = BS ? 2 : NL;
    using G = Geo<W>;
    constexpr uint32_t K = G::K, NB = G::NB, OFS = G::OFS, NA = G::NA, STRIDE = G::STRIDE, FRONT = G::FRONT, RUNS_CAP = G::RUNS;
    constexpr uint32_t SW = LCAP - K + 1, RPW = 64 / SEGS;
    constexpr uint32_t SEGSH = SEGS == 16 ? 4 : SEGS == 8 ? 3 : SEGS == 4 ? 2 : SEGS == 2 ? 1 : 0;
    constexpr uint32_t TSR = TSLOTS * SEGS < 48u ? TSLOTS * SEGS : 48u;
    static_assert(SEGS == 1 || SEGS == 2 || SEGS == 4 || SEGS == 8 || SEGS == 16, "lanes per read");
    constexpr int EW = RecTraits<W, I>::EW, KW = RecTraits<W, I>::KW;
    static_assert(EW <= 2, "entries of 8 or 16 bytes");
    constexpr uint32_t CB = I == 2 ? 16u : 13u, CMASK = (1u << CB) - 1u;
    constexpr uint32_t QS = I == 2 ? 16u : 20u, QMASK = (1u << QS) - 1u;
    const uint64_t tbl = (uint64_t)(uintptr_t)im.table;
    auto bucket_index = [&](uint32_t h, uint32_t o, uint32_t ext) -> uint32_t {
        const uint64_t re = s_reg[h >> 24];
        uint32_t slot = __umulhi(h << 8, (uint32_t)re & ((1u << UTREE_REGION_NB_BITS) - 1u));
        if constexpr (W == 16) {
            const uint32_t sub = (uint32_t)(re >> UTREE_REGION_NB_BITS) & ((1u << UTREE_REGION_SUB_BITS) - 1u);
            slot = slot * sub + ((ext * sub) >> 8);
        }
        return 2u * ((uint32_t)(re >> UTREE_REGION_BASE_SHIFT) + slot) + o;
    };
    auto bucket_addr = [&](uint32_t h, uint32_t o, uint32_t ext) -> uint64_t { return tbl + ((uint64_t)bucket_index(h, o, ext) << (NL == 2 ? 7 : 6)); };
    auto ext_of = [&](const uint32_t (&A)[G::NA], const uint32_t (&B)[G::NA], uint32_t o) -> uint32_t {
        if constexpr (W == 16) return ext_canon(((A[G::NA - 1u] & 0xFu) << 4) | (B[0] >> 28), o); else return 0u;
    };
    const uint32_t lane = lane_id();
    uint32_t *sl = stream + lane * STRIDE + FRONT;

    unsigned long long chunk_base = 0;
    uint32_t chunk_left = 0;
    const uint32_t wave_gid = blockIdx.x * LANES_WAVES + wv;
    if constexpr (PIECE) {
        const unsigned long long np = ws.cursors[UTREE_CUR_PIECES];
        n_reads = (uint32_t)(np < ws.n_pieces_cap ? np : ws.n_pieces_cap);
    }
    if constexpr (LISTED) n_reads = (uint32_t)ws.cursors[UTREE_CUR_CLASS + cls];
    if constexpr (MODE != 0) { if (!n_reads) return; }
    if constexpr (MODE == 0) { if (cls && !ws.cursors[UTREE_CUR_CLASS]) return; }
    const uint32_t *const lst = LISTED ? ws.cls_list + (size_t)cls * ws.cls_stride : nullptr;
    unsigned long long *parts = ws.cursors + 64 + (PIECE ? 2 : LISTED ? 3 + cls : 0) * (UTREE_WORK_PARTS * UTREE_WORK_STRIDE);
    const uint32_t part_len = ((n_reads + UTREE_WORK_PARTS - 1) / UTREE_WORK_PARTS + 63u) / 64u * 64u;
    uint32_t part = wave_gid % UTREE_WORK_PARTS, parts_left = UTREE_WORK_PARTS;

    LT_DECL
    for (;;) {
        uint32_t item = 0, item_end = 0;
        bool got = false;
        while (parts_left) {
            unsigned long long *ctr = parts + part * UTREE_WORK_STRIDE;
            const uint64_t lo = (uint64_t)part * part_len;
            const uint32_t avail = lo >= n_reads ? 0u : (uint32_t)(n_reads - lo < part_len ? n_reads - lo : part_len);
            unsigned long long g = ~0ull;
            if (lane == 0 && __hip_atomic_load(ctr, __ATOMIC_RELAXED, __HIP_MEMORY_SCOPE_AGENT) < avail) g = atomicAdd(ctr, (unsigned long long)RPW);
            const uint32_t taken = uni32((uint32_t)(g > 0xFFFFFFFFull ? 0xFFFFFFFFull : g));
            if (taken < avail) {
                item = (uint32_t)lo + taken;
                item_end = taken + RPW < avail ? item + RPW : (uint32_t)lo + avail;
                got = true;
                break;
            }
            part = part + 1 == UTREE_WORK_PARTS ? 0 : part + 1;
            --parts_left;
        }
        if (!got) break;
        LT(0);

        uint32_t L = 0;
        uint64_t o = 0;
        bool exc = false, other = false;
        {
            const uint32_t r0 = item + (lane >> SEGSH), piece = lane & (SEGS - 1u);
            if (r0 < item_end) {
                if constexpr (PIECE) {
                    const uint64_t pr = ws.pieces[r0];
                    const uint32_t rd = ws.long_list[(uint32_t)(pr >> 32)];
                    const uint64_t at = (uint64_t)(uint32_t)pr * (SEGS * SW) + piece * SW;
                    const uint64_t Lr = len[rd];
                    if (Lr > at) { L = (uint32_t)(Lr - at < LCAP ? Lr - at : LCAP); o = off[rd] + at; }
                } else {
                    const uint32_t rd = LISTED ? lst[r0] : r0;
                    const uint32_t Lr = len[rd];
                    if (Lr > (SEGS - 1u) * SW + LCAP) { if (MODE == 0 && SEGS == 1 && cls) other = true; else exc = true; }
                    else if (Lr > piece * SW) { L = umin(LCAP, Lr - piece * SW); o = off[rd] + piece * SW; }
                }
            }
        }
        uint32_t badpos;
        {
            const uint64_t a = (uint64_t)(uintptr_t)bases + o;
            const uint32_t mf = (uint32_t)a & 3u;
            const gptr32 p = (gptr32)(a - mf);
            const uint32_t nd = L ? (L + mf + 3u) >> 2 : 0u;
            uint32_t bad = 0, nbad = 0, badg = 0;
            constexpr uint32_t NRAW = LCAP / 4 + 1;
            uint32_t raw[NRAW];
#pragma unroll
            for (uint32_t d = 0; d < NRAW; ++d) raw[d] = 0u;
            if (nd) {
#pragma unroll
                for (uint32_t d = 0; d < NRAW; ++d) raw[d] = p[umin(d, nd - 1u)];
            }
            auto convert = [&](const uint32_t Lm) {
#pragma unroll
                for (uint32_t c = 0; c < NWORD / 2; ++c) {
                    uint32_t w[2] = {0u, 0u};
#pragma unroll
                    for (uint32_t g = 0; g < 8; ++g) {
                        const uint32_t gi = c * 8 + g;
                        const uint32_t fm = low_bytes(Lm > 4u * gi ? Lm - 4u * gi : 0u);
                        const uint32_t word = __builtin_amdgcn_alignbyte(raw[gi + 1], raw[gi], mf) & fm;
                        const uint32_t g2 = (word >> 1) & 0x03030303u;
                        const uint32_t letter = __builtin_amdgcn_perm(0u, 0x47544341u, g2);
                        const uint32_t z = (word & 0xDFDFDFDFu) ^ letter;
                        const uint32_t nz = (((z & 0x7F7F7F7Fu) + 0x7F7F7F7Fu) | z) & 0x80808080u;
                        bad |= nz & fm;
                        { const uint32_t pc = (uint32_t)__builtin_popcount(nz & fm); nbad += pc; badg += pc * gi; }
                        const uint32_t code = g2 ^ ((g2 >> 1) & 0x01010101u);
                        const uint32_t packed = (code * 0x40100401u) >> 24;
                        w[g >> 2] = (w[g >> 2] << 8) | packed;
                    }
                    sl[2 * c] = w[0]; sl[2 * c + 1] = w[1];
                }
            };
            const uint32_t L0 = uni32(L);
            if (ballot64(L != L0) == 0ull) convert(L0); else convert(L);
            if (nbad > 1u) { exc = true; L = 0; }
            badpos = nbad == 1u ? 4u * badg + ((uint32_t)__builtin_ctz(bad) >> 3) : 0xFFFF0000u;
        }
        const uint32_t nwin = L >= K ? L - (K - 1u) : 0u;
#pragma unroll
        for (uint32_t i = 0; i < TSLOTS; ++i) tab[i * 64u + lane] = T_EMPTY;
        if (lane < 2) full[lane] = 0;
        const uint32_t maxnwin = uni32(wave_max_u32(nwin));
        wave_lds_fence();
        LT(1);

        bool wave_full = false;
        for (int strand = 0; strand < (do_rc && !BS ? 2 : 1); ++strand) {
        if (strand) {
            uint32_t rw[NWORD];
#pragma unroll
            for (uint32_t i = 0; i < NWORD; ++i) {
                const uint32_t y = __builtin_bitreverse32(sl[NWORD - 1 - i]);
                rw[i] = ~(((y >> 1) & 0x55555555u) | ((y & 0x55555555u) << 1));
            }
            wave_lds_fence();
#pragma unroll
            for (uint32_t i = 0; i < NWORD; ++i) sl[i] = rw[i];
            wave_lds_fence();
            const uint32_t lead = 16u * NWORD - L, lw = lead >> 4, lb = 2u * (lead & 15u);
#pragma unroll
            for (uint32_t i = 0; i < NWORD; ++i) {
                const uint32_t a = sl[i + lw], b = sl[i + lw + 1];
                rw[i] = lb ? __builtin_amdgcn_alignbit(a, b, 32u - lb) : a;
            }
            wave_lds_fence();
#pragma unroll
            for (uint32_t i = 0; i < NWORD; ++i) sl[i] = rw[i];
            if (badpos < L) badpos = L - 1u - badpos;
            wave_lds_fence();
        }
        uint32_t nruns = 0;
        if (maxnwin) {
            uint32_t A[NB];
            uint32_t m16 = sl[0], r16 = rc16(sl[0]);
#define ROLL16(p_) { const uint32_t b_ = (sl[(p_) >> 4] >> (30u - 2u * ((p_) & 15u))) & 3u; m16 = (m16 << 2) | b_; r16 = __builtin_amdgcn_alignbit(b_ ^ 3u, r16, 2u); }
#define CKEY() (canon_key(m16, r16) & ~0x1FFu)
            auto irregular = [&](uint32_t m, uint32_t u) {
                if constexpr (IRR) {
                    const uint32_t pf = m >> 8;
                    if (u < nwin && (pf == im.irr_p[0] || pf == im.irr_p[1] || pf == im.irr_p[2] || pf == im.irr_p[3])) exc = true;
                }
            };
            irregular(m16, 0u);
#pragma unroll
            for (uint32_t p = 16; p < 16 + OFS; ++p) { ROLL16(p) irregular(m16, p - 15u); }
            A[0] = CKEY() | OFS;
#pragma unroll
            for (uint32_t p = 16 + OFS; p < K - OFS; ++p) {
                ROLL16(p)
                irregular(m16, p - 15u);
                A[p - 15 - OFS] = CKEY() | (p - 15u);
            }
            uint32_t run_first = 0, prev = 0xFFFFFFFFu;
            const uint32_t lanec = lane << 24;
            const uint32_t nwin_u = uni32(nwin);
#define PHASE_A_BLOCKS(CLEAN_) \
            for (uint32_t b = 0;; ++b) { \
_Pragma("unroll") \
                for (int rr = (int)NB - 2; rr >= 0; --rr) A[rr] = umin(A[rr], A[rr + 1]); \
                uint32_t P = 0; \
                bool done = false; \
_Pragma("unroll") \
                for (uint32_t rr = 0; rr < NB; ++rr) { \
                    const uint32_t s = NB * b + rr; \
                    uint32_t wmin; \
                    if (rr == 0) wmin = A[0]; \
                    else { \
                        const uint32_t p = s + (K - 1u - OFS); \
                        ROLL16(p) \
                        irregular(m16, s + (OFS + NB - 1u)); \
                        const uint32_t k = CKEY() | (s + (OFS + NB - 1u)); \
                        const uint32_t Sr = A[rr]; \
                        A[rr - 1] = k; \
                        P = rr == 1 ? k : umin(P, k); \
                        wmin = umin(Sr, P); \
                    } \
                    uint32_t wv; \
                    if (CLEAN_) wv = s < nwin_u ? wmin : 0xFFFFFFFFu; \
                    else wv = ((badpos - s) > (K - 1u) && s < nwin) ? wmin : 0xFFFFFFFFu; \
                    const bool changed = wv != prev; \
                    const bool emit = changed && prev != 0xFFFFFFFFu; \
                    const uint64_t em = ballot64(emit); \
                    if (em) { \
                        const uint32_t idx = __builtin_amdgcn_mbcnt_hi((uint32_t)(em >> 32), __builtin_amdgcn_mbcnt_lo((uint32_t)em, nruns)); \
 \
                        if (emit && idx < RUNS_CAP) runs[idx] = ((prev & 0xFFu) | (run_first << 8)) + ((s << 16) + lanec); \
                        nruns += (uint32_t)__popcll(em); \
                    } \
                    if (changed) run_first = s; \
                    prev = wv; \
                    if ((rr % 6u) == 0u && s >= maxnwin) { done = true; break; } \
                } \
                if (done) break; \
                const uint32_t p = NB * (b + 1u) + (K - 1u - OFS); \
                ROLL16(p) \
                irregular(m16, NB * (b + 1u) + (OFS + NB - 1u)); \
                A[NB - 1] = CKEY() | (NB * (b + 1u) + (OFS + NB - 1u)); \
            }
            const bool clean = ballot64(badpos < 0xFFFF0000u || nwin != nwin_u) == 0ull;
            if (clean) { PHASE_A_BLOCKS(true) } else { PHASE_A_BLOCKS(false) }
#undef PHASE_A_BLOCKS
#undef ROLL16
#undef CKEY
            nruns = uni32(nruns);
        }
        if (nruns > RUNS_CAP) { wave_full = true; nruns = 0; }
        wave_lds_fence();
        LT(2);

        uint32_t n_ovf = 0, ovf_room = 0;
        struct RunRegs { uint32_t b, pk, t, A[NA], B[NA], tr, RA[NA], RB[NA]; };
        constexpr uint32_t TSH = W == 8 ? 1u : 0u, PB = W == 8 ? 5u : 6u;
        constexpr uint32_t KM = K - 16u;
        auto rev_context = [&](const uint32_t (&A)[NA], const uint32_t (&B)[NA], uint32_t (&RA)[NA], uint32_t (&RB)[NA]) {
#pragma unroll
            for (uint32_t i = 0; i < NA; ++i) { RA[i] = rc16(B[NA - 1u - i]); RB[i] = rc16(A[NA - 1u - i]); }
        };
        auto context = [&](uint32_t q, uint32_t ustar, uint32_t &m, uint32_t (&A)[NA], uint32_t (&B)[NA]) {
            const uint32_t *sq = stream + q * STRIDE + FRONT + (ustar >> 4);
            const uint32_t rr = ustar & 15u, sh = (32u - 2u * rr) & 31u;
            uint32_t w[2 * NA + 2];
#pragma unroll
            for (uint32_t t = 0; t < 2 * NA + 2; ++t) w[t] = sq[(int)t - (int)NA];
#pragma unroll
            for (uint32_t i = 0; i < NA; ++i) {
                A[i] = rr ? __builtin_amdgcn_alignbit(w[i], w[i + 1], sh) : w[i];
                B[i] = rr ? __builtin_amdgcn_alignbit(w[NA + 1 + i], w[NA + 2 + i], sh) : w[NA + 1 + i];
            }
            m = rr ? __builtin_amdgcn_alignbit(w[NA], w[NA + 1], sh) : w[NA];
        };
        auto prepare = [&](uint32_t it, RunRegs &c) {
            const uint32_t idx = it * 64u + lane;
            const bool act = idx < nruns;
            const uint32_t rec = runs[act ? idx : nruns - 1u];
            const uint32_t q = rec >> 24, ustar = rec & 0xFFu, first = (rec >> 8) & 0xFFu;
            const uint32_t end = (rec >> 16) & 0xFFu;
            uint32_t m, o;
            context(q, ustar, m, c.A, c.B);
            const uint32_t h = canon_hash(m, o);
            c.b = bucket_index(h, o, ext_of(c.A, c.B, o));
            const uint32_t dl = act ? ((ustar - first) << 8) | ((end - 1u - first) << 14) : (G::DNONE << 8);
            c.pk = first | dl | (q << 20) | (o << 31);
            c.t = act ? (((((h & 0xFFu) << PB) | (ustar - (end - 1u))) << TSH) | (((end - 1u - first) << TSH) << 16)) : 0xFFFFu;
            if constexpr (BS) {
                rev_context(c.A, c.B, c.RA, c.RB);
                c.tr = act ? (((((h & 0xFFu) << PB) | (KM - (ustar - first))) << TSH) | (((end - 1u - first) << TSH) << 16)) : 0xFFFFu;
            }
        };
        typedef uint32_t u32x4 __attribute__((ext_vector_type(4)));
        typedef const __attribute__((address_space(1))) u32x4 *gptr128;
#define QUAD_BCAST(v, k) ((uint32_t)__builtin_amdgcn_mov_dpp((int)(v), (k) * 0x55, 0xF, 0xF, true))
#define ISSUE_K(k, at) { const uint64_t b_ = ((uint64_t)QUAD_BCAST(ahi, k) << 32) | (QUAD_BCAST(alo, k) | mine); \
                         P[at] = *(gptr128)b_; if constexpr (NL == 2) P[at + 1] = *(gptr128)(b_ | 64u); if constexpr (BS) P[at + 1] = *(gptr128)(b_ ^ 64u); }
        auto issue = [&](const RunRegs &c, const uint32_t half, u32x4 (&P)[4]) {
            const uint64_t a = tbl + ((uint64_t)c.b << (NL == 2 ? 7 : 6));
            const uint32_t alo = (uint32_t)a, ahi = (uint32_t)(a >> 32), mine = 16u * (lane & 3u);
            if constexpr (NLX == 1) { ISSUE_K(0, 0) ISSUE_K(1, 1) ISSUE_K(2, 2) ISSUE_K(3, 3) }
            else if (half == 0u) { ISSUE_K(0, 0) ISSUE_K(1, 2) } else { ISSUE_K(2, 0) ISSUE_K(3, 2) }
        };
#undef ISSUE_K
        auto push = [&](uint32_t q, uint32_t rank) {
            const uint32_t rd = q >> SEGSH;
            uint32_t *t = tab + rd;
            uint32_t i = 0;
            for (; i < TSR; ++i) {
                uint32_t cur = t[i * RPW];
                if (cur == T_EMPTY) {
                    cur = atomicCAS(&t[i * RPW], T_EMPTY, (rank << CB) | 1u);
                    if (cur == T_EMPTY) break;
                }
                if ((cur >> CB) == rank) { atomicAdd(&t[i * RPW], 1u); break; }
// ... 64 lines not shown
            if constexpr (NLX == 1) { SCAN_K(0, 0) SCAN_K(1, 1) SCAN_K(2, 2) SCAN_K(3, 3) }
            else if (half == 0u) { SCAN_K(0, 0) SCAN_K(1, 2) } else { SCAN_K(2, 0) SCAN_K(3, 2) }
#undef SCAN_K
            if (ballot64(np != 0u)) {
                if (np >= 1u) push(p0 >> QS, p0 & QMASK);
                if (ballot64(np >= 2u)) { if (np >= 2u) push(p1 >> QS, p1 & QMASK); }
            }
        };
        if (nruns) {
            const uint32_t nit = (nruns + 63u) >> 6;
            RunRegs R0, R1, R2;
            u32x4 P0[4], P1[4], P2[4];
            if constexpr (NLX == 1) {
                prepare(0u, R0); issue(R0, 0u, P0);
                prepare(1u, R1); issue(R1, 0u, P1);
                for (uint32_t it = 0; it < nit; it += 3) {
                    prepare(it + 2, R2); issue(R2, 0u, P2);
                    ovf_room = umin(nruns, 64u * (it + 3u));
                    scan(R0, 0u, P0);
                    prepare(it + 3, R0); issue(R0, 0u, P0);
                    ovf_room = umin(nruns, 64u * (it + 4u));
                    if (it + 1 < nit) scan(R1, 0u, P1);
                    prepare(it + 4, R1); issue(R1, 0u, P1);
                    ovf_room = umin(nruns, 64u * (it + 5u));
                    if (it + 2 < nit) scan(R2, 0u, P2);
                }
            } else {
                prepare(0u, R0); issue(R0, 0u, P0); issue(R0, 1u, P1);
                for (uint32_t it = 0; it < nit; it += 3) {
                    prepare(it + 1, R1); issue(R1, 0u, P2);
                    ovf_room = umin(nruns, 64u * (it + 2u));
                    scan(R0, 0u, P0);
                    issue(R1, 1u, P0);
                    scan(R0, 1u, P1);
                    prepare(it + 2, R2); issue(R2, 0u, P1);
                    ovf_room = umin(nruns, 64u * (it + 3u));
                    if (it + 1 < nit) scan(R1, 0u, P2);
                    issue(R2, 1u, P2);
                    if (it + 1 < nit) scan(R1, 1u, P0);
                    prepare(it + 3, R0); issue(R0, 0u, P0);
                    ovf_room = umin(nruns, 64u * (it + 4u));
                    if (it + 2 < nit) scan(R2, 0u, P1);
                    issue(R0, 1u, P1);
                    if (it + 2 < nit) scan(R2, 1u, P2);
                }
            }
        }
#undef QUAD_BCAST
        LT(5);
        constexpr uint32_t OVF_WAYS = 4;
        const uint32_t OVF_SCAN = im.ovf_scan;
        const bool OVF_CHAINS = W == 8 && (im.flags & UTREE_F_OVF_CHAINS) != 0u;
        auto fetch_desc = [&](uint32_t i) -> uint64_t {
            uint64_t dsc = 0;
            if (i < n_ovf) {
                const uint32_t rec = runs[i];
                uint32_t m, o, A[NA], B[NA];
                context((rec >> 24) & 63u, rec & 0xFFu, m, A, B);
                const uint32_t h = canon_hash(m, o);
                const uint64_t baddr = bucket_addr(h, o ^ (rec >> 31), ext_of(A, B, o));
                dsc = *(const __attribute__((address_space(1))) uint64_t *)(baddr + (64u * NL - 8u * EW + 8u * KW));
            }
            return dsc;
        };
        uint64_t dsc_next = 0;
        for (uint32_t ib = 0; ib < n_ovf; ib += 64) {
            wave_lds_fence();
            const uint32_t i = ib + lane;
            uint32_t nrec = 0, wn = 0;
            uint64_t dsc = ib == 0u ? ost[lane] : dsc_next;
            if (ib + 64u < n_ovf) dsc_next = fetch_desc(i + 64u);
            if (i < n_ovf) {
                const uint32_t rec = runs[i];
                const uint64_t n = ovf_count(dsc);
                ost[lane] = dsc;
                if (n <= OVF_SCAN && !(OVF_CHAINS && (dsc & OVF_HAS_DIR))) nrec = (uint32_t)n; else wn = ((rec >> 16) & 0xFFu) - ((rec >> 8) & 0xFFu);
            }
            auto spread = [&](uint32_t mine) -> uint32_t {
                uint32_t incl = mine;
#pragma unroll
                for (int dd = 1; dd < 64; dd <<= 1) { const uint32_t t = __shfl_up(incl, dd); if (lane >= (uint32_t)dd) incl += t; }
                wave_lds_fence();
                pref[lane] = incl;
                wave_lds_fence();
                return uni32((uint32_t)__shfl(incl, 63));
            };
            auto item_of = [&](uint32_t t, uint32_t &within) -> uint32_t {
                uint32_t lo = 0, hi = 63;
#pragma unroll
                for (int st = 0; st < 6; ++st) { const uint32_t mid = (lo + hi) >> 1; if (pref[mid] <= t) lo = mid + 1; else hi = mid; }
                within = t - (lo ? pref[lo - 1] : 0u);
                return lo;
            };
            const uint32_t total_rec = spread(nrec);
            constexpr uint32_t RB = W == 16 ? 2 : 1;
            for (uint32_t t0 = 0; t0 < total_rec; t0 += 64 * RB) {
                Entry<W, I> e[RB];
                uint32_t recs[RB];
#pragma unroll
                for (uint32_t u = 0; u < RB; ++u) {
                    const uint32_t t = t0 + 64u * u + lane;
                    recs[u] = 0;
#pragma unroll
                    for (int x = 0; x < EW; ++x) e[u].w[x] = 0;
                    if (t < total_rec) {
                        uint32_t j;
                        const uint32_t it_ = item_of(t, j);
                        recs[u] = runs[ib + it_];
                        e[u] = load_entry<W, I>(im.mrecs, ovf_first<W, I>(ost[it_]) + j);
                    }
                }
#pragma unroll
                for (uint32_t u = 0; u < RB; ++u) {
                    const uint32_t t = t0 + 64u * u + lane;
                    if (t < total_rec) {
                        const uint32_t rec = recs[u];
                        const uint32_t q = (rec >> 24) & 63u, ustar = rec & 0xFFu, first = (rec >> 8) & 0xFFu, lenm1 = ((rec >> 16) & 0xFFu) - 1u - first;
                        const bool rev = BS && (rec >> 31) != 0u;
                        uint32_t m, o, A[NA], B[NA];
                        context(q, ustar, m, A, B);
                        if constexpr (BS) { if (rev) { uint32_t RA[NA], RB[NA]; rev_context(A, B, RA, RB);
_Pragma("unroll") for (uint32_t x = 0; x < NA; ++x) { A[x] = RA[x]; B[x] = RB[x]; } } }
                        const uint32_t h = canon_hash(m, o);
                        const uint32_t hlow = h & 0xFFu;
                        const uint32_t wbase = rev ? ustar - first - KM : ustar - first;
                        bool hit;
                        uint32_t rank;
                        if constexpr (W == 8) {
                            const uint32_t lo = (uint32_t)e[u].w[0], hi = (uint32_t)(e[u].w[0] >> 32), pos = (hi >> 17) & 31u;
                            hit = (hi >> 22) == hlow && (rev ? wbase + pos : wbase - pos) <= lenm1 && (uint32_t)((((uint64_t)A[0] << 32) | B[0]) >> (2u * pos)) == lo;
                            if constexpr (I == 2) rank = hi & 0xFFFFu; else { rank = (uint32_t)e[u].w[1]; hit = hit && rank != INVALID; }
                        } else {
                            const uint32_t z = (uint32_t)e[u].w[1], wq = (uint32_t)(e[u].w[1] >> 32), pos = (wq >> 16) & 63u;
                            uint32_t r0, r1, r2;
                            rest96(A, B, pos, r0, r1, r2);
                            hit = (wq >> 22) == hlow && (rev ? wbase + pos : wbase - pos) <= lenm1 && r0 == __builtin_amdgcn_alignbit(wq, z, 16u) &&
                                  r1 == (uint32_t)(e[u].w[0] >> 32) && r2 == (uint32_t)e[u].w[0];
                            rank = z & 0xFFFFu;
                        }
                        if (hit && (I == 4 || rank != 0xFFFFu)) push(q, rank);
                    }
                }
            }
            const uint32_t total_win = spread(wn);
            for (uint32_t t0 = 0; t0 < total_win; t0 += 64 * OVF_WAYS) {
                uint64_t lo[OVF_WAYS], hi[OVF_WAYS];
                MinKey<W> mk[OVF_WAYS];
                uint32_t qs[OVF_WAYS];
                const uint16_t *dirp[OVF_WAYS];
                const uint64_t *chp[OVF_WAYS];
                uint32_t chn[OVF_WAYS], chat[OVF_WAYS];
#pragma unroll
                for (uint32_t u = 0; u < OVF_WAYS; ++u) {
                    const uint32_t t = t0 + 64u * u + lane;
                    lo[u] = hi[u] = 0; qs[u] = 0; mk[u].lo = mk[u].hi = 0;
                    dirp[u] = nullptr;
                    chp[u] = im.mrecs; chn[u] = 0; chat[u] = ~0u;
                    if (t < total_win) {
                        uint32_t j;
                        const uint32_t it_ = item_of(t, j);
                        const uint32_t rec = runs[ib + it_];
                        const uint32_t q = (rec >> 24) & 63u, ustar = rec & 0xFFu, first = (rec >> 8) & 0xFFu;
                        const bool rev = BS && (rec >> 31) != 0u;
                        const uint32_t pos = rev ? KM - (ustar - (first + j)) : ustar - (first + j);
                        uint32_t m, o, A[NA], B[NA];
                        context(q, ustar, m, A, B);
                        if constexpr (BS) { if (rev) { uint32_t RA[NA], RB[NA]; rev_context(A, B, RA, RB);
_Pragma("unroll") for (uint32_t x = 0; x < NA; ++x) { A[x] = RA[x]; B[x] = RB[x]; } } }
                        const uint32_t h = canon_hash(m, o);
                        const uint32_t hlow = h & 0xFFu;
                        const uint64_t dsc = ost[it_];
                        lo[u] = ovf_first<W, I>(dsc); hi[u] = lo[u] + ovf_count(dsc); qs[u] = q;
                        if (OVF_CHAINS && (dsc & OVF_HAS_DIR)) { chp[u] = im.mrecs + (dsc & M39) * EW; chn[u] = (uint32_t)ovf_count(dsc); hi[u] = lo[u]; }
                        else if (dsc & OVF_HAS_DIR) dirp[u] = (const uint16_t *)(im.mrecs + (dsc & M39) * EW) + pos;
                        if constexpr (W == 8) {
                            const uint32_t rest = (uint32_t)((((uint64_t)A[0] << 32) | B[0]) >> (2u * pos));
                            mk[u].hi = 0; mk[u].lo = ((uint64_t)((hlow << 5) | pos) << 32) | rest;
                        } else {
                            uint32_t r0, r1, r2;
                            rest96(A, B, pos, r0, r1, r2);
                            mk[u].lo = ((uint64_t)r1 << 32) | r2; mk[u].hi = ((uint64_t)hlow << 38) | ((uint64_t)pos << 32) | r0;
                        }
                    }
                }
                if constexpr (W == 8) {
                    bool anych = false;
#pragma unroll
                    for (uint32_t u = 0; u < OVF_WAYS; ++u) anych = anych || chn[u] != 0u;
                    if (OVF_CHAINS && ballot64(anych)) {
                        for (uint32_t c = 0;; c += 2) {
                            bool more = false;
#pragma unroll
                            for (uint32_t u = 0; u < OVF_WAYS; ++u) more = more || (c < chn[u] && chat[u] == ~0u);
                            if (!ballot64(more)) break;
                            uint64_t h0[OVF_WAYS][2], h1[OVF_WAYS][2];
#pragma unroll
                            for (uint32_t u = 0; u < OVF_WAYS; ++u) {
                                const uint32_t c0 = c < chn[u] ? c : 0u, c1 = c + 1u < chn[u] ? c + 1u : 0u;
                                h0[u][0] = chp[u][2u * c0]; h0[u][1] = chp[u][2u * c0 + 1u];
                                h1[u][0] = chp[u][2u * c1]; h1[u][1] = chp[u][2u * c1 + 1u];
                            }
#pragma unroll
                            for (uint32_t u = 0; u < OVF_WAYS; ++u) {
                                const uint32_t pos = (uint32_t)(mk[u].lo >> 32) & 31u, rest = (uint32_t)mk[u].lo;
                                const uint32_t a0 = chain_hit(h0[u][0], h0[u][1], pos, rest), a1 = chain_hit(h1[u][0], h1[u][1], pos, rest);
                                if (c < chn[u] && chat[u] == ~0u) chat[u] = a0;
                                if (c + 1u < chn[u] && chat[u] == ~0u) chat[u] = a1;
                            }
                        }
                        uint32_t rk[OVF_WAYS];
#pragma unroll
                        for (uint32_t u = 0; u < OVF_WAYS; ++u) {
                            const uint32_t at = chat[u] == ~0u ? 0u : chat[u];
                            if constexpr (I == 2) rk[u] = ((const uint16_t *)(chp[u] + 2u * chn[u]))[at]; else rk[u] = ((const uint32_t *)(chp[u] + 2u * chn[u]))[at];
                        }
#pragma unroll
                        for (uint32_t u = 0; u < OVF_WAYS; ++u)
                            if (chat[u] != ~0u && (I == 4 ? rk[u] != INVALID : rk[u] != 0xFFFFu)) push(qs[u], rk[u]);
                    }
                }
                bool anydir = false;
#pragma unroll
                for (uint32_t u = 0; u < OVF_WAYS; ++u) anydir = anydir || dirp[u] != nullptr;
                if (ballot64(anydir)) {
                    uint32_t da[OVF_WAYS], db[OVF_WAYS];
#pragma unroll
                    for (uint32_t u = 0; u < OVF_WAYS; ++u) {
                        const uint16_t *dp_ = dirp[u] ? dirp[u] : (const uint16_t *)im.mrecs;
                        da[u] = dp_[0]; db[u] = dp_[1];
                    }
#pragma unroll
                    for (uint32_t u = 0; u < OVF_WAYS; ++u) if (dirp[u]) { hi[u] = lo[u] + db[u]; lo[u] += da[u]; }
                }
                for (;;) {
                    bool any = false;
#pragma unroll
                    for (uint32_t u = 0; u < OVF_WAYS; ++u) any = any || lo[u] < hi[u];
                    if (!ballot64(any)) break;
                    Entry<W, I> e[OVF_WAYS];
                    uint64_t mid[OVF_WAYS];
#pragma unroll
                    for (uint32_t u = 0; u < OVF_WAYS; ++u) { mid[u] = lo[u] + ((hi[u] - lo[u]) >> 1); e[u] = load_entry<W, I>(im.mrecs, mid[u]); }
#pragma unroll
                    for (uint32_t u = 0; u < OVF_WAYS; ++u) {
                        if (lo[u] < hi[u]) {
                            const MinKey<W> k = mrec_key<W, I>(e[u]);
                            if (mkey_lt<W>(k, mk[u])) lo[u] = mid[u] + 1;
                            else if (mkey_eq<W>(k, mk[u])) { const uint32_t rank = mrec_rank<W, I>(e[u]); if (rank != INVALID) push(qs[u], rank); hi[u] = lo[u]; }
                            else hi[u] = mid[u];
                        }
                    }
                }
            }
        }
        wave_lds_fence();
        }
        LT(3);

        const uint64_t excm = ballot64(exc);
        const bool have = lane < RPW && item + lane < item_end && !other;
        const uint32_t r = LISTED ? (have ? lst[item + lane] : 0u) : item + lane;
        exc = ((excm >> ((lane * SEGS) & 63u)) & ((1ull << SEGS) - 1ull)) != 0ull || ((full[lane >> 5] >> (lane & 31u)) & 1u) != 0u || wave_full;
        if constexpr (PIECE) {
            if (have) pref[lane] = (uint32_t)(ws.pieces[r] >> 32);
            if (have && exc) ws.lflag[pref[lane]] = 1u;
            const uint64_t okm = ballot64(have && !exc);
            wave_lds_fence();
            for (uint32_t x0 = 0; x0 < RPW * TSR; x0 += 64) {
                const uint32_t x = x0 + lane, pc = x / TSR, slot = x % TSR;
                if (x < RPW * TSR && ((okm >> pc) & 1ull)) {
                    const uint32_t e = tab[slot * RPW + pc];
                    if (e != T_EMPTY) {
                        const uint32_t li = pref[pc], rank = e >> CB;
                        uint32_t *tr = ws.ltab_rank + (size_t)li * UTREE_LONG_SLOTS, *tc = ws.ltab_cnt + (size_t)li * UTREE_LONG_SLOTS;
                        uint32_t sidx = (rank * 0x9E3779B1u) >> 26, tries = 0;
                        for (; tries < UTREE_LONG_SLOTS; ++tries, sidx = (sidx + 1u) & (UTREE_LONG_SLOTS - 1u)) {
                            uint32_t cur = __hip_atomic_load(&tr[sidx], __ATOMIC_RELAXED, __HIP_MEMORY_SCOPE_AGENT);
                            if (cur == 0xFFFFFFFFu) cur = atomicCAS(&tr[sidx], 0xFFFFFFFFu, rank);
                            if (cur == 0xFFFFFFFFu || cur == rank) { atomicAdd(&tc[sidx], e & CMASK); break; }
                        }
                        if (tries == UTREE_LONG_SLOTS) ws.lflag[li] = 1u;
                    }
                }
            }
            wave_lds_fence();
            LT(4);
            continue;
        }
        const uint64_t xm = ballot64(have && exc);
        if (xm) {
            unsigned long long xb = 0;
            if (lane == 0) xb = atomicAdd(&ws.cursors[UTREE_CUR_MID], (unsigned long long)__popcll(xm));
            xb = uni64(xb);
            if (have && exc) ws.mid_list[xb + lanes_below(xm)] = r;
        }
        const bool live = have && !exc;
        const uint32_t *tq = tab + (lane < RPW ? lane : 0u);
        uint32_t nu = 0, F = 0;
        if (live) {
#pragma unroll
            for (uint32_t i = 0; i < TSR; ++i) { const uint32_t e = tq[i * RPW]; if (e != T_EMPTY) { ++nu; F += e & CMASK; } }
        }
        const uint32_t first_rank = tq[0] >> CB;
        const uint32_t maxnu = uni32(wave_max_u32(nu));
        const uint32_t need = nu >= 2u ? nu : 0u;
        uint32_t incl = need;
#pragma unroll
        for (int dd = 1; dd < 64; dd <<= 1) { const uint32_t t = __shfl_up(incl, dd); if (lane >= (uint32_t)dd) incl += t; }
        const uint32_t total = uni32((uint32_t)__shfl(incl, 63));
        if (total > chunk_left) {
            unsigned long long nb = 0;
            if (lane == 0) {
                nb = atomicAdd(&ws.cursors[0], (unsigned long long)UTREE_TALLY_CHUNK);
                if (nb + UTREE_TALLY_CHUNK > ws.tally_cap) { ws.cursors[UTREE_CUR_ERROR] = UTREE_DEVERR_TALLY_CAP; nb = 0; }
            }
            chunk_base = uni64(nb);
            chunk_left = UTREE_TALLY_CHUNK;
        }
        const unsigned long long my_base = chunk_base + (incl - need);
        chunk_base += total; chunk_left -= total;
        if (maxnu >= 2u) {
            for (uint32_t i = 0; i < maxnu; ++i) {
                const uint32_t e = tq[i * RPW];
                uint32_t place = 0;
                for (uint32_t j = 0; j < maxnu; ++j) { const uint32_t x = tq[j * RPW]; place += (j < nu && (x >> CB) < (e >> CB)) ? 1u : 0u; }
                if (need && i < nu) ws.tally[my_base + place] = (uint64_t)(e >> CB) | ((uint64_t)(e & CMASK) << 32);
            }
        }
        if (live) {
            if (F == 0) store_result(&out[r], 0, -2, 0, 0, 0, 0);
            else if (nu == 1) store_result(&out[r], first_rank, RANK_PENDING, F, 1, 0, 0);
            else store_result(&out[r], 0, CUT_PENDING, F, nu, (uint32_t)my_base, (uint32_t)(my_base >> 32));
        }
        wave_lds_fence();
        LT(4);
    }
#ifdef UTREE_LANES_TIMERS
    if (lane == 0) { for (int q = 0; q < 6; ++q) atomicAdd(&g_lphase[q], lt_acc[q]); atomicAdd(&g_lphase[7], 1ull); }
#endif
}

#define LANES_PROLOGUE(W_) \
    using G_ = Geo<W_>; \
    __shared__ uint32_t s_stream[LANES_WAVES][64 * G_::STRIDE]; \
    __shared__ uint32_t s_runs[LANES_WAVES][G_::RUNS]; \
    __shared__ uint32_t s_tab[LANES_WAVES][64 * TSLOTS]; \
    __shared__ uint32_t s_full[LANES_WAVES][2]; \
    __shared__ uint32_t s_pref[LANES_WAVES][64]; \
    __shared__ uint64_t s_ost[LANES_WAVES][64]; \
    __shared__ uint64_t s_reg[256]; \
    for (uint32_t x = threadIdx.x; x < 256; x += blockDim.x) s_reg[x] = im.regions[x]; \
    const uint32_t wv = uni32(threadIdx.x >> 6); \
    { uint32_t *sl_ = s_stream[wv] + lane_id() * G_::STRIDE + G_::FRONT; \
      _Pragma("unroll") for (uint32_t i = 1; i <= G_::FRONT; ++i) sl_[-(int)i] = 0;       \
      sl_[NWORD] = 0; sl_[NWORD + 1] = 0; } \
    __syncthreads();
#define LANES_LDS s_stream[wv], s_runs[wv], s_tab[wv], s_full[wv], s_pref[wv], s_ost[wv], s_reg, wv

template <int W, int I, int SEGS, bool IRR, int MODE, int NL, bool BS>
__global__ __launch_bounds__(LANES_WAVES * 64, LANES_WPS)
void classify_lanes_k(utk_image im, const uint8_t *__restrict__ bases, const uint64_t *__restrict__ off, const uint32_t *__restrict__ len,
                      uint32_t n_reads, int do_rc, utree_result *__restrict__ out, utk_workspace ws, uint32_t cls) {
    LANES_PROLOGUE(W)
    lanes_body<W, I, SEGS, IRR, MODE, NL, BS>(im, bases, off, len, n_reads, do_rc, out, ws, cls, LANES_LDS);
}

template <int W, int I, bool IRR, int NL, bool BS>
__global__ __launch_bounds__(LANES_WAVES * 64, LANES_WPS)
void classify_lanes_mixed_k(utk_image im, const uint8_t *__restrict__ bases, const uint64_t *__restrict__ off, const uint32_t *__restrict__ len,
                            uint32_t n_reads, int do_rc, utree_result *__restrict__ out, utk_workspace ws, uint32_t max_cls) {
    LANES_PROLOGUE(W)
    lanes_body<W, I, 1, IRR, 0, NL, BS>(im, bases, off, len, n_reads, do_rc, out, ws, 1u, LANES_LDS);
    if (max_cls >= 1u) lanes_body<W, I, 2, IRR, 1, NL, BS>(im, bases, off, len, n_reads, do_rc, out, ws, 1u, LANES_LDS);
    if (max_cls >= 2u) lanes_body<W, I, 4, IRR, 1, NL, BS>(im, bases, off, len, n_reads, do_rc, out, ws, 2u, LANES_LDS);
    if (max_cls >= 3u) lanes_body<W, I, 8, IRR, 1, NL, BS>(im, bases, off, len, n_reads, do_rc, out, ws, 3u, LANES_LDS);
    if (max_cls >= 4u) lanes_body<W, I, 16, IRR, 1, NL, BS>(im, bases, off, len, n_reads, do_rc, out, ws, 4u, LANES_LDS);
}

static inline uint32_t lanes_resident_blocks(int n_cu) {
    static_assert(4 * LANES_WPS >= LANES_WAVES, "a CU holds at least one workgroup");
    return (uint32_t)n_cu * (4u * LANES_WPS / LANES_WAVES);
}

template <int W, int I, int SEGS, bool IRR, int MODE, int NL, bool BS = false>
static int launch_lanes(const utk_image *im, const uint8_t *d_bases, const uint64_t *d_off, const uint32_t *d_len, uint32_t n_reads,
                        int do_rc, utree_result *d_out, const utk_workspace *ws, int n_cu, void *stream, uint32_t cls = 0) {
    static_assert(NL == 1 || NL == 2, "bucket size");
    uint32_t blocks = (n_reads + (64u / SEGS) * LANES_WAVES - 1) / ((64u / SEGS) * LANES_WAVES);
    const uint32_t cap = lanes_resident_blocks(n_cu);
    if (blocks > cap) blocks = cap;
    classify_lanes_k<W, I, SEGS, IRR, MODE, NL, BS><<<dim3(blocks), dim3(LANES_WAVES * 64), 0, (hipStream_t)stream>>>(*im, d_bases, d_off, d_len, n_reads, do_rc, d_out, *ws, cls);
    return (int)hipGetLastError();
}

template <int W, int I, bool IRR, int NL, bool BS = false>
static int launch_lanes_mixed(const utk_image *im, const uint8_t *d_bases, const uint64_t *d_off, const uint32_t *d_len, uint32_t n_reads,
                              int do_rc, utree_result *d_out, const utk_workspace *ws, int n_cu, void *stream, uint32_t max_cls) {
    uint32_t blocks = (n_reads + 64u * LANES_WAVES - 1) / (64u * LANES_WAVES);
    const uint32_t cap = lanes_resident_blocks(n_cu);
    if (blocks > cap) blocks = cap;
    classify_lanes_mixed_k<W, I, IRR, NL, BS><<<dim3(blocks), dim3(LANES_WAVES * 64), 0, (hipStream_t)stream>>>(*im, d_bases, d_off, d_len, n_reads, do_rc, d_out, *ws, max_cls);
    return (int)hipGetLastError();
}

}
```

### utree_amd/csrc/utree_internal.h

```cpp
#ifndef UTREE_INTERNAL_H
#define UTREE_INTERNAL_H
#include <stddef.h>
#include <stdint.h>
#include "../../include/utree_amd.h"

#ifdef __cplusplus
extern "C" {
#endif

#define UTREE_NUMBINS ((1u << 24) + 1u)
#define UTREE_INVALID 0xFFFFFFFFu
#define UTREE_IMG_MAGIC 0x31474d4945525455ull
#define UTREE_IMG_HEADER_BYTES 4096u
#define UTREE_IMG_VERSION 14u
#define UTREE_REGION_NB_BITS 25
#define UTREE_REGION_SUB_BITS 9
#define UTREE_REGION_BASE_SHIFT (UTREE_REGION_NB_BITS + UTREE_REGION_SUB_BITS)
#define UTREE_MIN_MARGIN(W_) ((W_) == 16 ? 2u : 0u)
#define UTREE_TALLY_CHUNK 8192u
#define UTREE_CUR_LONG 32
#define UTREE_CUR_MID 16
#define UTREE_CUR_WORK 48
#define UTREE_CUR_WORK_LONG 40
#define UTREE_CUR_WORK_MID 56
#define UTREE_WORK_PARTS 64
#define UTREE_WORK_STRIDE 16
#define UTREE_CUR_PIECES 8
#define UTREE_CUR_LEFT 24
#define UTREE_CUR_CLASS 9
#define UTREE_CUR_ERROR 17
#define UTREE_CURSOR_BYTES (512 + 8 * UTREE_WORK_PARTS * UTREE_WORK_STRIDE * 8)
#define UTREE_DEVERR_TALLY_CAP 1ull
#define UTREE_DEVERR_LONG_CAP 2ull
#define UTREE_DEVERR_PIECES_CAP 3ull
#define UTREE_LONG_SLOTS 64u
#define UTREE_SHORT_CAP 320u
#define UTREE_SHORT2_CAP 640u
#define UTREE_MID_DEFAULT 2112u
#define UTREE_LANES_CAP 160u
#define UTREE_MID_CAP 2112u

#define UTREE_F_IRREGULAR 1u
#define UTREE_F_GENERIC   2u
#define UTREE_F_OFF64     4u
#define UTREE_F_VOTE_TABLE 16u
#define UTREE_F_STRAND_VIEWS 32u
#define UTREE_F_DIRECT 64u
#define UTREE_F_OVF_CHAINS 128u
#define UTREE_F_INVALID_RANKS 8u

typedef struct {
    uint64_t magic;
    uint32_t version, W, I, k;
    uint32_t fine_bits, rec_words, n_labels, flags;
    uint64_t n_nodes;
    uint64_t n_slots;
    uint64_t n_min;
    uint64_t off_table, off_mrecs, off_recs, off_coarse, off_irreg, off_label_off, off_label_blob, off_rank2ix;
    uint64_t label_blob_bytes;
    uint64_t n_irregular;
    uint64_t total_bytes;
    uint64_t off_vote;
    uint32_t bucket_words, pad0;
    uint64_t regions[256];
} utree_image_header;

typedef struct {
    uint16_t pid[8];
    uint8_t tok_end[8];
    uint8_t exists, more, us, n_tok;
    uint8_t len, pad;
    uint16_t ix;
} utk_vote_rec;

typedef struct {
    const uint64_t *table;
    const uint64_t *regions;
    const uint64_t *mrecs;
    const uint64_t *recs;
    const void *coarse;
    const uint32_t *irreg;
    const uint32_t *label_off;
    const char *label_blob;
    const uint32_t *rank2ix;
    const uint64_t *vote_tab;
    uint64_t n_nodes;
    uint32_t n_labels, fine_bits, flags, W, I;
    uint32_t bucket_words;
    uint32_t ovf_scan;
    uint32_t irr_n, irr_p[4];
} utk_image;

static inline uint32_t utree_rec_words(uint32_t W, uint32_t I) { return (W == 16 ? 2u : 1u) * (I == 4 ? 2u : 1u); }

int utk_repack(uint32_t W, uint32_t I, const void *d_raw, uint64_t count, const uint32_t *d_ix2rank,
               uint32_t n_labels, uint64_t *d_recs_at_first, unsigned long long *d_invalid, void *stream);
int utk_widen_binix(const void *d_raw_binix, uint32_t width, int off64, void *d_coarse, void *stream);
int utk_validate(uint32_t W, uint32_t I, int off64, const void *d_coarse, const uint64_t *d_recs, uint64_t n_nodes,
                 uint32_t *d_irreg, unsigned long long *d_counters, void *stream);
int utk_build_min(uint32_t W, uint32_t I, int off64, const void *d_coarse, const uint64_t *d_recs, uint64_t c0, uint64_t m, uint64_t dup_cap,
                  const uint64_t *d_regions, const uint64_t *h_regions, uint64_t n_buckets, uint32_t bucket_words, uint64_t *d_table, uint64_t *d_mrecs,
                  uint32_t *d_irreg, unsigned long long *d_overflow, uint64_t *n_min, int *views, void *stream);
int utk_build_direct(uint32_t I, int off64, int generic, const void *d_coarse, const uint64_t *d_recs, uint64_t n_nodes, uint64_t c0, uint64_t m,
                     const uint32_t *d_irreg, uint64_t n_irregular, void *d_table, void *stream);
int utk_compact_overflow(uint32_t W, uint32_t I, uint64_t *d_table, uint64_t n_buckets, uint32_t bucket_words, uint64_t *d_mrecs, uint64_t *n_kept, int *chains, void *stream);
int utk_compress_chunk(uint32_t W, uint32_t I, const void *d_in, uint64_t first, uint64_t count, unsigned long long *d_first,
                       void *d_out, void *stream);
int utk_fill_recs_pad(uint64_t *d_recs_end, uint32_t words, void *stream);

typedef struct {
    unsigned long long *cursors;
    uint64_t *tally;
    uint64_t tally_cap;
    uint32_t *long_list;
    uint32_t *mid_list;
    uint32_t *hist;
    uint32_t *touch;
    uint32_t long_blocks, mid_reads;
    uint32_t short_cap;
    uint32_t mid_limit;
    uint64_t *pieces;
    uint32_t *ltab_rank, *ltab_cnt;
    uint32_t *lflag;
    uint32_t *long_left;
    uint32_t n_long_cap;
    uint64_t n_pieces_cap;
    uint32_t *cls_list;
    uint32_t cls_stride;
    uint64_t ltally_base;
} utk_workspace;

int utk_classify_short(const utk_image *im, const uint8_t *d_bases, const uint64_t *d_off, const uint32_t *d_len,
                       uint32_t n_reads, int do_rc, utree_result *d_out, const utk_workspace *ws, int n_cu,
                       void *stream);
int utk_lanes_ok(const utk_image *im, uint32_t max_len, int do_rc);
int utk_lanes_segs(const utk_image *im, uint32_t max_len);
int utk_lanes_image_ok(const utk_image *im);
int utk_lanes_both_strands(const utk_image *im, int do_rc);
int utk_classify_long_pieces(const utk_image *im, const uint8_t *d_bases, const uint64_t *d_off, const uint32_t *d_len, int do_rc,
                             utree_result *d_out, const utk_workspace *ws, int n_cu, void *stream);
int utk_classify_lanes(const utk_image *im, const uint8_t *d_bases, const uint64_t *d_off, const uint32_t *d_len, uint32_t n_reads,
                       uint32_t max_len, int do_rc, utree_result *d_out, const utk_workspace *ws, int n_cu, void *stream);
int utk_classify_lanes_mixed(const utk_image *im, const uint8_t *d_bases, const uint64_t *d_off, const uint32_t *d_len, uint32_t n_reads,
                             uint32_t max_len, int do_rc, utree_result *d_out, const utk_workspace *ws, int n_cu, void *stream);
uint32_t utk_lanes_max_len(const utk_image *im);
int utk_route(const uint32_t *d_len, uint32_t n_reads, int do_rc, const utk_workspace *ws, void *stream);
int utk_classify_mid(const utk_image *im, const uint8_t *d_bases, const uint64_t *d_off, const uint32_t *d_len,
                     uint32_t n_reads, int do_rc, utree_result *d_out, const utk_workspace *ws, int n_cu, void *stream);
int utk_classify_listed(const utk_image *im, const uint8_t *d_bases, const uint64_t *d_off, const uint32_t *d_len,
                        uint32_t n_reads, uint32_t max_len, int do_rc, utree_result *d_out, const utk_workspace *ws, int n_cu, void *stream);
int utk_classify_long(const utk_image *im, const uint8_t *d_bases, const uint64_t *d_off, const uint32_t *d_len,
                      int do_rc, utree_result *d_out, const utk_workspace *ws, int n_cu, void *stream);
int utk_vote(const utk_image *im, utree_result *d_out, const utk_workspace *ws, uint32_t n_reads, void *stream);
int utk_lookup(const utk_image *im, const uint64_t *d_hi, const uint64_t *d_lo, uint64_t n, uint32_t *d_ix,
               void *stream);
typedef struct {
    unsigned long long *cursors;
    uint32_t *nh;
    uint64_t *hoff;
    uint32_t *hits;
    uint64_t hits_cap;
    uint32_t *lvl[3];
    uint32_t nlvl[3];
    uint32_t *hist;
    uint32_t hist_waves;
    uint32_t *state;
    uint32_t state_cap;
    uint32_t step;
    uint32_t slack, tolerance;
} utk_rank_ws;

int utk_rank_hits(const utk_image *im, const uint8_t *d_bases, const uint64_t *d_off, const uint32_t *d_len,
                  uint32_t n_reads, int do_rc, const utk_rank_ws *ws, int n_cu, void *stream);
int utk_rank_levels(const utk_rank_ws *ws, uint32_t n_reads, void *stream);
int utk_rank_vote(const utk_image *im, utree_result *d_out, uint32_t n_reads, const utk_rank_ws *ws, int n_cu,
                  void *stream);
int utk_rank_state(uint32_t n_reads, const utk_rank_ws *ws, void *stream);

const char *utk_classify_short_name(const utk_image *im, uint32_t short_cap, int mid, int do_rc, char *buf, size_t cap);
const char *utk_classify_long_name(const utk_image *im, char *buf, size_t cap);
int utk_model_counts(const utk_image *im, const uint8_t *d_bases, const uint64_t *d_off, const uint32_t *d_len, uint32_t n_reads,
                     int do_rc, unsigned long long *d_counts, void *stream);

#ifdef __cplusplus
}
#endif
#endif
```

### utree_amd/lib.py

```python
from __future__ import annotations

import ctypes as C
import os

_HERE = os.path.dirname(os.path.abspath(__file__))
SO_PATH = os.environ.get("UTREE_AMD_SO") or os.path.join(_HERE, "libutree_amd.so")
CLI_PATH = os.path.join(_HERE, "xtree-searchGG")
COMPRESS_CLI_PATH = os.path.join(_HERE, "xtree-compress")
RANK_CLI_PATH = os.path.join(_HERE, "xtree-search")
BUILD_GG_CLI_PATH = os.path.join(_HERE, "utree-buildGG")
BUILD_CLI_PATH = os.path.join(_HERE, "utree-build")
_LIB = None

OK, E_IO, E_FORMAT, E_UNSUPPORTED, E_NOMEM, E_HIP, E_ARG, E_NOLABELS, E_FASTA, E_RCCL, E_BUILD, E_DEVICE, E_PROFILE, E_COVERAGE = range(14)
BUILD_E_MAP_EMPTY, BUILD_E_MAP, BUILD_E_FASTA, BUILD_E_NO_KMERS, BUILD_E_NAME = range(1, 6)
FINE_AUTO = -1
FANOUT_NONE, FANOUT_BROADCAST, FANOUT_UPLOAD = range(3)
REPLICATE_FN = C.CFUNCTYPE(C.c_int, C.c_void_p, C.c_void_p, C.POINTER(C.c_int), C.c_int, C.POINTER(C.c_void_p))
UPLOAD_FN = C.CFUNCTYPE(C.c_int, C.c_void_p, C.c_int, C.c_int, C.POINTER(C.c_void_p))
INPUT_REFERENCE, INPUT_FASTQ, INPUT_FASTA_MULTILINE, INPUT_AUTO = range(4)


class CtrInfo(C.Structure):
    _fields_ = [("W", C.c_uint32), ("I", C.c_uint32), ("k", C.c_uint32), ("SZ", C.c_uint32), ("n_nodes", C.c_uint64),
                ("n_labels", C.c_uint32), ("binix_width", C.c_uint32), ("bin_total", C.c_uint64),
                ("file_bytes", C.c_uint64)]


class DevInfo(C.Structure):
    _fields_ = [("fine_bits", C.c_uint32), ("record_bytes", C.c_uint32), ("image_bytes", C.c_uint64),
                ("irregular_bins", C.c_uint64), ("generic_mode", C.c_uint32), ("device", C.c_int32),
                ("vote_table", C.c_uint32), ("lane_pass", C.c_uint32), ("bucket_bytes", C.c_uint32), ("strand_views", C.c_uint32),
                ("overflow_chains", C.c_uint32), ("pad0", C.c_uint32), ("overflow_bytes", C.c_uint64)]


class FastaError(C.Structure):
    _fields_ = [("code", C.c_int), ("read_index", C.c_uint64)]


class SearchStats(C.Structure):
    _fields_ = [("n_reads", C.c_uint64), ("good_finds", C.c_uint64), ("seconds_total", C.c_double),
                ("seconds_kernels", C.c_double), ("fasta_error", FastaError), ("pipeline", C.c_int), ("n_lanes", C.c_int),
                ("seconds_read", C.c_double), ("seconds_frame", C.c_double), ("seconds_classify_format", C.c_double),
                ("seconds_order_wait", C.c_double), ("seconds_d2h", C.c_double), ("seconds_write", C.c_double),
                ("bytes_in", C.c_uint64), ("bytes_out", C.c_uint64)]


class CompressStats(C.Structure):
    _fields_ = [("n_nodes", C.c_uint64), ("n_labels", C.c_uint64), ("label_count_total", C.c_uint64), ("W", C.c_uint32),
                ("I", C.c_uint32), ("seconds", C.c_double)]


class BuildStats(C.Structure):
    _fields_ = [("n_seqs", C.c_uint64), ("n_kmers", C.c_uint64), ("n_nodes", C.c_uint64), ("n_labels", C.c_uint64),
                ("error_line", C.c_uint64), ("error_kind", C.c_int), ("W", C.c_uint32), ("I", C.c_uint32),
                ("seconds", C.c_double), ("n_distinct", C.c_uint64), ("map_bytes", C.c_uint64), ("map_lines", C.c_uint64),
                ("map_error", C.c_int)]


class RankParams(C.Structure):
    _fields_ = [("slack", C.c_uint32), ("sparsity", C.c_uint32), ("tolerance", C.c_uint32)]


class ProfileEntry(C.Structure):
    _fields_ = [("label", C.c_uint32), ("cut", C.c_int32), ("reads", C.c_uint64)]


class CoverageEntry(C.Structure):
    _fields_ = [("label", C.c_uint32), ("pad", C.c_uint32), ("db_kmers", C.c_uint64), ("covered", C.c_uint64), ("hits", C.c_uint64)]


class Result(C.Structure):
    _fields_ = [("label", C.c_uint32), ("cut", C.c_int32), ("found", C.c_uint32), ("uix", C.c_uint32),
                ("sl", C.c_uint32), ("ol", C.c_uint32)]


SYMBOLS = {
    "utree_strerror": (C.c_char_p, [C.c_int]),
    "utree_abi_version": (C.c_int, []),
    "utree_last_hip_error": (C.c_char_p, []),
    "utree_ctr_open": (C.c_int, [C.c_char_p, C.POINTER(C.c_void_p)]),
    "utree_ctr_from_memory": (C.c_int, [C.c_uint32, C.c_uint32, C.c_uint64, C.c_void_p, C.c_uint32, C.c_void_p,
                                        C.c_char_p, C.c_size_t, C.POINTER(C.c_void_p)]),
    "utree_ctr_close": (None, [C.c_void_p]),
    "utree_ctr_get_info": (C.c_int, [C.c_void_p, C.POINTER(CtrInfo)]),
    "utree_ctr_label": (C.c_void_p, [C.c_void_p, C.c_uint32, C.POINTER(C.c_uint32)]),
    "utree_dev_image_bytes": (C.c_size_t, [C.c_void_p, C.c_int]),
    "utree_dev_upload": (C.c_int, [C.c_void_p, C.c_int, C.c_int, C.POINTER(C.c_void_p)]),
    "utree_dev_upload_seconds": (C.c_int, [C.POINTER(C.c_double)]),
    "utree_dev_build": (C.c_int, [C.c_void_p, C.c_int, C.c_int, C.c_void_p, C.c_void_p, C.c_void_p, C.c_size_t,
                                  C.c_void_p, C.POINTER(C.c_void_p)]),
    "utree_dev_image": (C.c_int, [C.c_void_p, C.POINTER(C.c_void_p), C.POINTER(C.c_size_t)]),
    "utree_dev_attach": (C.c_int, [C.c_void_p, C.c_int, C.c_void_p, C.c_size_t, C.POINTER(C.c_void_p)]),
    "utree_dev_free": (None, [C.c_void_p]),
    "utree_dev_get_info": (C.c_int, [C.c_void_p, C.POINTER(DevInfo)]),
    "utree_dev_replicate": (C.c_int, [C.c_void_p, C.c_void_p, C.POINTER(C.c_int), C.c_int, C.POINTER(C.c_void_p)]),
    "utree_dev_replicate_seconds": (C.c_double, []),
    "utree_dev_fanout": (C.c_int, [C.c_void_p, C.c_void_p, C.POINTER(C.c_int), C.c_int, C.c_int, C.POINTER(C.c_void_p), C.POINTER(C.c_int)]),
    "utree_dev_fanout_with": (C.c_int, [C.c_void_p, C.c_void_p, C.POINTER(C.c_int), C.c_int, C.c_int, C.POINTER(C.c_void_p), C.POINTER(C.c_int),
                                        C.c_void_p, C.c_void_p]),
    "utree_rccl_unique_id": (C.c_int, [C.c_void_p, C.c_size_t]),
    "utree_dev_replicate_rank": (C.c_int, [C.c_void_p, C.c_void_p, C.c_int, C.c_int, C.c_int, C.c_int, C.c_void_p, C.c_size_t,
                                           C.POINTER(C.c_void_p)]),
    "utree_classify_workspace_bytes": (C.c_size_t, [C.c_void_p, C.c_uint32, C.c_uint64, C.c_uint32, C.c_int]),
    "utree_classify_batch": (C.c_int, [C.c_void_p, C.c_void_p, C.c_void_p, C.c_void_p, C.c_uint32, C.c_uint64,
                                       C.c_uint32, C.c_int, C.c_void_p, C.c_void_p, C.c_size_t, C.c_void_p]),
    "utree_classify_poll": (C.c_int, [C.c_void_p]),
    "utree_lookup_words": (C.c_int, [C.c_void_p, C.c_void_p, C.c_void_p, C.c_uint64, C.c_void_p, C.c_void_p]),
    "utree_classify_kernel_name": (C.c_char_p, [C.c_void_p]),
    "utree_model_counts": (C.c_int, [C.c_void_p, C.c_void_p, C.c_void_p, C.c_void_p, C.c_uint32, C.c_int, C.c_void_p, C.c_void_p]),
    "utree_classify_kernel_time": (C.c_int, [C.c_void_p, C.c_int, C.POINTER(C.c_double), C.POINTER(C.c_uint64)]),
    "utree_fasta_frame": (C.c_int, [C.c_void_p, C.c_size_t, C.c_int, C.c_size_t, C.c_void_p, C.c_void_p, C.c_void_p,
                                    C.c_void_p, C.POINTER(C.c_size_t), C.POINTER(C.c_size_t), C.POINTER(FastaError)]),
    "utree_format_records": (C.c_size_t, [C.c_void_p, C.c_void_p, C.c_void_p, C.c_void_p, C.c_void_p, C.c_size_t,
                                          C.c_void_p, C.c_size_t, C.POINTER(C.c_uint64)]),
    "utree_compress_file": (C.c_int, [C.c_char_p, C.c_char_p, C.c_int, C.POINTER(CompressStats)]),
    "utree_rank_params_default": (None, [C.POINTER(RankParams)]),
    "utree_rank_workspace_bytes": (C.c_size_t, [C.c_void_p, C.c_uint32, C.c_uint64, C.c_uint32, C.c_int,
                                                C.POINTER(RankParams)]),
    "utree_rank_batch": (C.c_int, [C.c_void_p, C.c_void_p, C.c_void_p, C.c_void_p, C.c_uint32, C.c_uint64, C.c_uint32,
                                   C.c_int, C.POINTER(RankParams), C.c_void_p, C.c_void_p, C.c_size_t, C.c_void_p]),
    "utree_rank_reset": (C.c_int, [C.c_void_p]),
    "utree_format_rank_records": (C.c_size_t, [C.c_void_p, C.c_void_p, C.c_void_p, C.c_void_p, C.c_void_p, C.c_size_t,
                                               C.c_void_p, C.c_size_t, C.POINTER(C.c_uint64)]),
    "utree_rank_search_file": (C.c_int, [C.c_void_p, C.c_void_p, C.c_char_p, C.c_char_p, C.c_int, C.POINTER(RankParams),
                                         C.c_int, C.POINTER(SearchStats)]),
    "utree_reads_frame": (C.c_int, [C.c_void_p, C.c_size_t, C.c_int, C.c_int, C.c_size_t, C.c_void_p, C.c_void_p, C.c_void_p,
                                    C.c_void_p, C.POINTER(C.c_size_t), C.POINTER(C.c_size_t), C.POINTER(FastaError)]),
    "utree_search_file_opts": (C.c_int, [C.c_void_p, C.POINTER(C.c_void_p), C.c_int, C.c_char_p, C.c_char_p, C.c_int, C.c_int,
                                         C.c_int, C.POINTER(SearchStats)]),
    "utree_rank_search_file_opts": (C.c_int, [C.c_void_p, C.c_void_p, C.c_char_p, C.c_char_p, C.c_int, C.POINTER(RankParams),
                                              C.c_int, C.c_int, C.POINTER(SearchStats)]),
    "utree_build_file": (C.c_int, [C.c_char_p, C.c_char_p, C.c_char_p, C.c_uint32, C.c_uint32, C.c_int, C.c_int, C.c_int,
                                   C.POINTER(BuildStats)]),
    "utree_search_prepare": (C.c_int, [C.c_void_p, C.POINTER(C.c_void_p), C.c_int, C.c_int]),
    "utree_search_file": (C.c_int, [C.c_void_p, C.POINTER(C.c_void_p), C.c_int, C.c_char_p, C.c_char_p, C.c_int, C.c_int,
                                    C.POINTER(SearchStats)]),
    "utree_profile_create": (C.c_int, [C.c_void_p, C.c_uint32, C.POINTER(C.c_void_p)]),
    "utree_profile_add": (C.c_int, [C.c_void_p, C.c_void_p, C.c_uint32, C.c_void_p]),
    "utree_profile_reset": (C.c_int, [C.c_void_p]),
    "utree_profile_max_entries": (C.c_size_t, [C.c_void_p]),
    "utree_profile_read": (C.c_int, [C.c_void_p, C.c_void_p, C.c_size_t, C.POINTER(C.c_size_t), C.POINTER(C.c_uint64),
                                     C.POINTER(C.c_uint64)]),
    "utree_profile_free": (None, [C.c_void_p]),
    "utree_profile_write": (C.c_int, [C.c_void_p, C.c_void_p, C.c_size_t, C.c_uint64, C.c_char_p]),
    "utree_search_file_profile": (C.c_int, [C.c_void_p, C.POINTER(C.c_void_p), C.c_int, C.c_char_p, C.c_char_p, C.c_int, C.c_int,
                                            C.c_int, C.c_char_p, C.POINTER(SearchStats)]),
    "utree_coverage_bytes": (C.c_size_t, [C.c_void_p]),
    "utree_coverage_create": (C.c_int, [C.c_void_p, C.c_void_p, C.c_void_p, C.c_void_p, C.POINTER(C.c_void_p)]),
    "utree_coverage_add": (C.c_int, [C.c_void_p, C.c_void_p, C.c_void_p, C.c_void_p, C.c_uint32, C.c_int, C.c_void_p]),
    "utree_coverage_reset": (C.c_int, [C.c_void_p]),
    "utree_coverage_merge": (C.c_int, [C.c_void_p, C.c_void_p]),
    "utree_coverage_read": (C.c_int, [C.c_void_p, C.c_void_p, C.c_size_t, C.POINTER(C.c_size_t), C.POINTER(C.c_uint64),
                                      C.POINTER(C.c_uint64)]),
    "utree_coverage_free": (None, [C.c_void_p]),
    "utree_coverage_write": (C.c_int, [C.c_void_p, C.c_void_p, C.c_size_t, C.c_uint64, C.c_char_p]),
    "utree_search_file_coverage": (C.c_int, [C.c_void_p, C.POINTER(C.c_void_p), C.c_int, C.c_char_p, C.c_char_p, C.c_int, C.c_int,
                                             C.c_int, C.c_char_p, C.c_char_p, C.POINTER(SearchStats)]),
    "utree_rank_search_file_profile": (C.c_int, [C.c_void_p, C.c_void_p, C.c_char_p, C.c_char_p, C.c_int, C.POINTER(RankParams),
                                                 C.c_int, C.c_int, C.c_char_p, C.POINTER(SearchStats)]),
}


def kernel_source_sha256() -> str:
    import hashlib
    h = hashlib.sha256()
    for f in ("kernels.hip", "lanes_kernel.hip", "lanes_core.hpp", "lanes_part.hip", "wave_common.hpp", "device_common.hpp", "utree_internal.h", "Makefile"):
        with open(os.path.join(_HERE, "csrc", f), "rb") as fh:
            h.update(f.encode() + b"\0" + fh.read() + b"\0")
    return h.hexdigest()


class UtreeError(RuntimeError):
    def __init__(self, code, what=""):
        self.code = code
        msg = load().utree_strerror(code).decode() if _LIB is not None else str(code)
        if _LIB is not None and code in (4, 5, 11, 12, 13):
            hip = (_LIB.utree_last_hip_error() or b"").decode(errors="replace")
            if hip:
                msg += " [" + hip + "]"
        super().__init__("%s: %s (code %d)" % (what, msg, code))


def load():
    global _LIB
    if _LIB is None:
        if not os.path.exists(SO_PATH):
            raise ImportError("utree_amd: %s is missing -- build it with `make -C utree_amd/csrc` "
                              "(or __graft_entry__.build()); there is no CPU fallback" % SO_PATH)
        try:
            import torch
        except ImportError:
            pass
        L = C.CDLL(SO_PATH, mode=C.RTLD_GLOBAL)
        for name, (res, args) in SYMBOLS.items():
            f = getattr(L, name)
            f.restype = res
            f.argtypes = args
        _LIB = L
    return _LIB


def check(code, what=""):
    if code != OK:
        raise UtreeError(code, what)
```

Measured before the change: 2.332 billion reads/s.

## Fuse vote resolution into lanes classifier with closed-form two-rank vote

Moves vote resolution into the lanes classification kernel for the single-segment, I=2 path. Reads with one rank are finished inline, and reads with two ranks use a new closed-form vote2 routine. Remaining pending reads are pooled per wave in LDS and voted in 64-read batches, so the separate per-read vote kernel becomes a small grid-stride pass over a listed subset. In exchange the lanes kernel uses more LDS for the pool and more registers, which may lower occupancy. It also adds extra fences and divergent vote work inside the hot kernel.

```diff
diff --git a/utree_amd/csrc/dev_image.c b/utree_amd/csrc/dev_image.c
--- a/utree_amd/csrc/dev_image.c
+++ b/utree_amd/csrc/dev_image.c
@@ -654,6 +654,7 @@
 }
 
 static int lanes_enabled(void) { const char *e = getenv("UTREE_LANE_PASS"); return !(e && e[0] == '0'); }
+static int vote_fused_enabled(void) { const char *e = getenv("UTREE_VOTE_FUSED"); return !(e && e[0] == '0'); }
 
 static void ring_lock(utree_dev *d) { while (__atomic_test_and_set(&d->ring_busy, __ATOMIC_ACQUIRE)) ; }
 static void ring_unlock(utree_dev *d) { __atomic_clear(&d->ring_busy, __ATOMIC_RELEASE); }
@@ -751,6 +752,7 @@
     w->mid_list = (uint32_t *)(b + off); off = align_up(off + (uint64_t)n_reads * 4, 256);
     uint64_t max_total = do_rc ? 2 * (uint64_t)max_len + 1 : max_len;
     w->long_blocks = 0; w->hist = NULL; w->touch = NULL;
+    w->vote_fused = 0;
     w->short_cap = max_total > UTREE_SHORT_CAP ? UTREE_SHORT2_CAP : UTREE_SHORT_CAP;
     w->mid_reads = max_total > w->short_cap;
     w->mid_limit = mid_limit();
@@ -821,6 +823,7 @@
     const int lanes = lanes_enabled() && utk_lanes_image_ok(&d->kimg) && lanes_worth(d);
     if (lanes) {
         const int mixed = max_len > UTREE_LANES_CAP;
+        w.vote_fused = !mixed && !w.long_blocks && d->kimg.vote_tab != NULL && d->kimg.I == 2 && vote_fused_enabled();
         d->last_long = w.long_blocks != 0; d->last_mid = 0; d->last_rc = do_rc; d->last_short_cap = w.short_cap;
         d->last_lanes = utk_lanes_segs(&d->kimg, max_len); d->last_mixed = mixed; d->last_pieces = w.long_blocks != 0;
         if (e0 && !w.long_blocks) HIPCHK(hipEventRecord(e0, st));
diff --git a/utree_amd/csrc/kernels.hip b/utree_amd/csrc/kernels.hip
--- a/utree_amd/csrc/kernels.hip
+++ b/utree_amd/csrc/kernels.hip
@@ -4,6 +4,7 @@
 #include <string.h>
 #include "device_common.hpp"
 #include "wave_common.hpp"
+#include "vote_common.hpp"
 
 using namespace utk;
 
@@ -641,137 +642,6 @@
     }
 }
 
-__device__ __forceinline__ uint32_t cut_of(uint32_t x) {
-    uint32_t c = x - x / 4;
-    c += (x >> 1) >= c;
-    return c;
-}
-
-__device__ __forceinline__ void label16(const char *s, uint32_t p, uint64_t &x, uint64_t &y) {
-    typedef unsigned long long u64x2 __attribute__((ext_vector_type(2), aligned(1)));
-    const u64x2 v = *(const u64x2 *)(s + p);
-    x = v.x; y = v.y;
-}
-
-__device__ __forceinline__ uint64_t stop_flags(uint64_t x1, uint64_t x2) {
-    const uint64_t semi = x1 ^ 0x3B3B3B3B3B3B3B3Bull, d = x1 ^ x2;
-    uint64_t m = (((x1 - 0x0101010101010101ull) & ~x1) | ((semi - 0x0101010101010101ull) & ~semi)) & 0x8080808080808080ull;
-    m |= (((d & 0x7F7F7F7F7F7F7F7Full) + 0x7F7F7F7F7F7F7F7Full) | d) & 0x8080808080808080ull;
-    return m;
-}
-
-__device__ __forceinline__ void pair_scan(const char *s1, const char *s2, uint32_t start, uint32_t &td, uint32_t &a, uint32_t &b, uint32_t &before) {
-    uint32_t base = start, prevlast = start ? (uint32_t)(uint8_t)s1[start - 1] : 0u;
-    for (;;) {
-        uint64_t x1, y1, x2, y2;
-        label16(s1, base, x1, y1); label16(s2, base, x2, y2);
-        uint64_t m = stop_flags(x1, x2);
-        if (!m) { prevlast = (uint32_t)(x1 >> 56); base += 8; x1 = y1; x2 = y2; m = stop_flags(x1, x2); }
-        if (m) {
-            const uint32_t idx = (uint32_t)(__builtin_ctzll(m) >> 3);
-            td = base + idx;
-            a = (uint32_t)(x1 >> (8 * idx)) & 0xFFu; b = (uint32_t)(x2 >> (8 * idx)) & 0xFFu;
-            before = idx ? ((uint32_t)(x1 >> (8 * idx - 8)) & 0xFFu) : prevlast;
-            return;
-        }
-        prevlast = (uint32_t)(x1 >> 56); base += 8;
-    }
-}
-
-struct VRec { uint64_t w[4]; };
-__device__ __forceinline__ VRec vrec(const uint64_t *vt, uint32_t rank) {
-    typedef unsigned long long u64x2 __attribute__((ext_vector_type(2)));
-    const u64x2 *p = (const u64x2 *)(vt + (size_t)rank * 4);
-    const u64x2 a = p[0], b = p[1];
-    VRec v; v.w[0] = a.x; v.w[1] = a.y; v.w[2] = b.x; v.w[3] = b.y;
-    return v;
-}
-__device__ __forceinline__ uint32_t v_pid(const VRec &v, uint32_t t) { return (uint32_t)((t < 4 ? v.w[0] : v.w[1]) >> (16u * (t & 3u))) & 0xFFFFu; }
-__device__ __forceinline__ uint32_t v_end(const VRec &v, uint32_t t) { return (uint32_t)(v.w[2] >> (8u * t)) & 0xFFu; }
-__device__ __forceinline__ bool v_exists(const VRec &v, uint32_t t) { return ((uint32_t)v.w[3] >> t) & 1u; }
-__device__ __forceinline__ bool v_more(const VRec &v, uint32_t t) { return ((uint32_t)v.w[3] >> (8u + t)) & 1u; }
-__device__ __forceinline__ bool v_us(const VRec &v, uint32_t t) { return ((uint32_t)v.w[3] >> (16u + t)) & 1u; }
-__device__ __forceinline__ uint32_t v_len(const VRec &v) { return (uint32_t)(v.w[3] >> 32) & 0xFFu; }
-__device__ __forceinline__ uint32_t v_ix(const VRec &v) { return (uint32_t)(v.w[3] >> 48); }
-
-__device__ __forceinline__ void vote_table(const utk_image &im, utree_result *out_r, const uint64_t *T, uint32_t F, uint32_t uix) {
-    const uint64_t *vt = im.vote_tab;
-    const char *blob = im.label_blob;
-    const uint32_t *loff = im.label_off;
-    constexpr uint32_t NONE = 0xFFFFFFFFu;
-    uint32_t cutoff = cut_of(F);
-    uint32_t st = 0, ed = uix, dv = NONE, t = 0, orun = F, sl, ol;
-    uint32_t ix_last, n_last, len_last;
-    for (;;) {
-        const uint64_t t_st = T[st];
-        VRec pv = vrec(vt, (uint32_t)t_st);
-        const uint64_t t_ed = ed - 1u == st ? t_st : T[ed - 1u];
-        const VRec lv = ed - 1u == st ? pv : vrec(vt, (uint32_t)t_ed);
-        {
-            const uint64_t d0 = pv.w[0] ^ lv.w[0], d1 = pv.w[1] ^ lv.w[1];
-            const uint32_t same = d0 ? (uint32_t)__builtin_ctzll(d0) >> 4 : 4u + (d1 ? (uint32_t)__builtin_ctzll(d1) >> 4 : 4u);
-            const uint32_t both = ((uint32_t)(pv.w[3] & lv.w[3]) >> 8) & 0xFFu;
-            const uint32_t semis = (uint32_t)__builtin_ctz(~both);
-            const uint32_t L = same < semis ? same : semis;
-            if (L > t) { dv = v_end(pv, L - 1u); t = L; }
-        }
-        uint32_t run = (uint32_t)(t_st >> 32), td = dv, c1 = run, rp = (uint32_t)t_st;
-        bool td_is_end = false;
-        bool stopped = false;
-        for (uint32_t z = st + 1; z < ed; ++z) {
-            const bool is_last = z == ed - 1u;
-            const uint64_t tz = is_last ? t_ed : T[z];
-            const uint32_t nz = (uint32_t)(tz >> 32), rc = (uint32_t)tz;
-            const VRec cv = is_last ? lv : vrec(vt, rc);
-            bool aside = false, stop = false;
-            if (t >= 8u || !v_exists(pv, t) || (dv == NONE && v_end(pv, 0) == 0u && !v_more(pv, 0))) aside = true;
-            else {
-                uint32_t a, b, before;
-                bool known = true;
-                if (v_exists(cv, t) && v_pid(cv, t) == v_pid(pv, t)) {
-                    td = v_end(pv, t); td_is_end = true;
-                    a = v_more(pv, t) ? ';' : 0u; b = v_more(cv, t) ? ';' : 0u; before = v_us(pv, t) ? '_' : 'x';
-                } else if (v_us(pv, t) || !v_exists(cv, t)) {
-                    pair_scan(blob + loff[rp], blob + loff[rc], dv + 1u, td, a, b, before);
-                    td_is_end = td == v_end(pv, t);
-                } else { a = 'a'; b = 'b'; before = 'x'; known = false; }
-                if (a == b) run += nz;
-                else if ((!a && b == ';') || ((a == ';' || !a) && before == '_')) aside = true;
-                else if (run >= cutoff) {
-                    ed = z; stop = true;
-                    if (!known) {
-                        pair_scan(blob + loff[rp], blob + loff[rc], dv + 1u, td, a, b, before);
-                        td_is_end = td == v_end(pv, t);
-                    }
-                } else { run = nz; st = z; }
-            }
-            if (aside) {
-                run = nz; st = z;
-                orun -= c1;
-                cutoff = cut_of(orun);
-            }
-            if (stop) { stopped = true; break; }
-            pv = cv; c1 = nz; rp = rc;
-        }
-        ix_last = stopped ? v_ix(pv) : v_ix(lv);
-        n_last = stopped ? c1 : (uint32_t)(t_ed >> 32);
-        len_last = stopped ? v_len(pv) : v_len(lv);
-        sl = run; ol = orun;
-        if (run < cutoff) break;
-        if (st + 1 >= ed) {
-            if (n_last >= cutoff) dv = 0xFFFFFFFEu;
-            break;
-        }
-        orun = run; cutoff = cut_of(run);
-        if (td != dv) { dv = td; if (td_is_end) ++t; }
-    }
-    int32_t cut;
-    if (dv == NONE) cut = -1;
-    else if (dv == 0xFFFFFFFEu) cut = -2;
-    else cut = (int32_t)(dv < len_last ? dv : len_last);
-    store_result(out_r, ix_last, cut, F, uix, sl, ol);
-}
-
 __global__ __launch_bounds__(256) void vote_table_k(utk_image im, utree_result *__restrict__ out, utk_workspace ws, uint32_t n_reads) {
     __shared__ uint32_t s_n[2][4];
     __shared__ uint16_t s_who[256];
@@ -802,6 +672,16 @@
     const uint32_t r = blockIdx.x * blockDim.x + who;
     const uint32_t *res = (const uint32_t *)&out[r];
     vote_table(im, &out[r], ws.tally + ((uint64_t)res[4] | ((uint64_t)res[5] << 32)), res[2], res[3]);
+}
+
+constexpr uint32_t VOTE_LISTED_BLOCKS = 64;
+__global__ __launch_bounds__(256) void vote_listed_k(utk_image im, utree_result *__restrict__ out, utk_workspace ws, uint32_t n_reads) {
+    const unsigned long long nl = ws.cursors[UTREE_CUR_MID];
+    const uint32_t n = (uint32_t)(nl < n_reads ? nl : n_reads);
+    for (uint32_t i = blockIdx.x * blockDim.x + threadIdx.x; i < n; i += gridDim.x * blockDim.x) {
+        const uint32_t r = ws.mid_list[i];
+        if (r < n_reads) vote_pending(im, &out[r], ws.tally);
+    }
 }
 
 __global__ __launch_bounds__(256) void vote_k(utk_image im, utree_result *__restrict__ out, utk_workspace ws, uint32_t n_reads) {
@@ -1054,6 +934,10 @@
 
 int utk_vote(const utk_image *im, utree_result *d_out, const utk_workspace *ws, uint32_t n_reads, void *stream) {
     if (!n_reads) return 0;
+    if (ws->vote_fused) {
+        vote_listed_k<<<dim3(VOTE_LISTED_BLOCKS), dim3(256), 0, (hipStream_t)stream>>>(*im, d_out, *ws, n_reads);
+        return (int)hipGetLastError();
+    }
     if (im->vote_tab) vote_table_k<<<dim3((n_reads + 255) / 256), dim3(256), 0, (hipStream_t)stream>>>(*im, d_out, *ws, n_reads);
     else vote_k<<<dim3((n_reads + 255) / 256), dim3(256), 0, (hipStream_t)stream>>>(*im, d_out, *ws, n_reads);
     return (int)hipGetLastError();
diff --git a/utree_amd/csrc/lanes_core.hpp b/utree_amd/csrc/lanes_core.hpp
--- a/utree_amd/csrc/lanes_core.hpp
+++ b/utree_amd/csrc/lanes_core.hpp
@@ -5,6 +5,7 @@
 #include <string.h>
 #include "device_common.hpp"
 #include "wave_common.hpp"
+#include "vote_common.hpp"
 
 using namespace utk;
 
@@ -37,6 +38,7 @@
 constexpr uint32_t TSLOTS = 12;
 constexpr uint32_t T_EMPTY = 0xFFFFFFFFu;
 constexpr int32_t CUT_PENDING = -3, RANK_PENDING = -4;
+constexpr uint32_t VPOOL = 128;
 
 __device__ __forceinline__ uint32_t low_bytes(uint32_t n) { return n >= 4u ? 0xFFFFFFFFu : ((1u << (8u * n)) - 1u); }
 __device__ __forceinline__ uint64_t ballot64(bool p) { return __builtin_amdgcn_ballot_w64(p); }
@@ -64,12 +66,28 @@
     r0 = __builtin_amdgcn_alignbit(x[0], x[1], bs); r1 = __builtin_amdgcn_alignbit(x[1], x[2], bs); r2 = __builtin_amdgcn_alignbit(x[2], x[3], bs);
 }
 
-template <int W, int I, int SEGS, bool IRR, int MODE, int NL, bool BS>
+template <int W, int I, int SEGS, bool IRR, int MODE, int NL, bool BS, bool FUSE_OK = true>
 __device__ __forceinline__ void lanes_body(const utk_image &im, const uint8_t *__restrict__ bases, const uint64_t *__restrict__ off, const uint32_t *__restrict__ len,
                                            uint32_t n_reads, const int do_rc, utree_result *__restrict__ out, const utk_workspace &ws, const uint32_t cls,
                                            uint32_t *stream, uint32_t *runs, uint32_t *tab, uint32_t *full, uint32_t *pref, uint64_t *ost, const uint64_t *s_reg,
-                                           const uint32_t wv) {
+                                           uint32_t *vpool, const uint32_t wv) {
     constexpr bool PIECE = MODE == 2, LISTED = MODE == 1;
+    constexpr bool FUSE = FUSE_OK && MODE == 0 && SEGS == 1 && I == 2;
+    const bool fuse = FUSE && ws.vote_fused != 0u;
+    uint32_t npool = 0;
+    auto pool_vote = [&](const uint32_t cnt) {
+        if constexpr (FUSE) {
+            __builtin_amdgcn_fence(__ATOMIC_RELEASE, "workgroup");
+            __builtin_amdgcn_fence(__ATOMIC_ACQUIRE, "workgroup");
+            wave_lds_fence();
+            if (lane_id() < cnt) {
+                const uint32_t r = vpool[npool - cnt + lane_id()];
+                vote_pending(im, &out[r], ws.tally);
+            }
+            npool -= cnt;
+            wave_lds_fence();
+        }
+    };
     static_assert(!BS || NL == 1, "both strands in one pass: 64-byte buckets");
     constexpr int NLX = BS ? 2 : NL;
     using G = Geo<W>;
@@ -740,8 +758,21 @@
             for (uint32_t i = 0; i < TSR; ++i) { const uint32_t e = tq[i * RPW]; if (e != T_EMPTY) { ++nu; F += e & CMASK; } }
         }
         const uint32_t first_rank = tq[0] >> CB;
-        const uint32_t maxnu = uni32(wave_max_u32(nu));
-        const uint32_t need = nu >= 2u ? nu : 0u;
+        bool voted = false;
+        uint32_t fin[6] = {0u, 0u, 0u, 0u, 0u, 0u};
+        if constexpr (FUSE) {
+            if (fuse && live && nu >= 1u && nu <= 2u) {
+                if (nu == 1u) { fin[0] = im.rank2ix[first_rank]; fin[1] = (uint32_t)-2; fin[2] = F; fin[3] = 1u; voted = true; }
+                else {
+                    const uint32_t ea = tq[0], eb = tq[RPW];
+                    const uint32_t e0 = umin(ea, eb), e1 = ea ^ eb ^ e0;
+                    const VRec pv = vrec(im.vote_tab, e0 >> CB), lv = vrec(im.vote_tab, e1 >> CB);
+                    voted = vote2_closed(pv, lv, e0 & CMASK, e1 & CMASK, F, fin);
+                }
+            }
+        }
+        const uint32_t need = nu >= 2u && !voted ? nu : 0u;
+        const uint32_t maxnu = uni32(wave_max_u32(need));
         uint32_t incl = need;
 #pragma unroll
         for (int dd = 1; dd < 64; dd <<= 1) { const uint32_t t = __shfl_up(incl, dd); if (lane >= (uint32_t)dd) incl += t; }
@@ -767,12 +798,24 @@
         }
         if (live) {
             if (F == 0) store_result(&out[r], 0, -2, 0, 0, 0, 0);
+            else if (voted) store_result(&out[r], fin[0], (int32_t)fin[1], fin[2], fin[3], fin[4], fin[5]);
             else if (nu == 1) store_result(&out[r], first_rank, RANK_PENDING, F, 1, 0, 0);
             else store_result(&out[r], 0, CUT_PENDING, F, nu, (uint32_t)my_base, (uint32_t)(my_base >> 32));
+        }
+        if constexpr (FUSE) {
+            if (fuse) {
+                const uint64_t pm = ballot64(live && need != 0u);
+                if (pm) {
+                    if ((pm >> lane) & 1ull) vpool[npool + lanes_below(pm)] = r;
+                    npool += (uint32_t)__popcll(pm);
+                    if (npool >= 64u) pool_vote(64u);
+                }
+            }
         }
         wave_lds_fence();
         LT(4);
     }
+    if constexpr (FUSE) { if (npool) pool_vote(npool); }
 #ifdef UTREE_LANES_TIMERS
     if (lane == 0) { for (int q = 0; q < 6; ++q) atomicAdd(&g_lphase[q], lt_acc[q]); atomicAdd(&g_lphase[7], 1ull); }
 #endif
@@ -786,6 +829,7 @@
     __shared__ uint32_t s_full[LANES_WAVES][2]; \
     __shared__ uint32_t s_pref[LANES_WAVES][64]; \
     __shared__ uint64_t s_ost[LANES_WAVES][64]; \
+    __shared__ uint32_t s_vpool[LANES_WAVES][VPOOL]; \
     __shared__ uint64_t s_reg[256]; \
     for (uint32_t x = threadIdx.x; x < 256; x += blockDim.x) s_reg[x] = im.regions[x]; \
     const uint32_t wv = uni32(threadIdx.x >> 6); \
@@ -793,7 +837,7 @@
       _Pragma("unroll") for (uint32_t i = 1; i <= G_::FRONT; ++i) sl_[-(int)i] = 0;       \
       sl_[NWORD] = 0; sl_[NWORD + 1] = 0; } \
     __syncthreads();
-#define LANES_LDS s_stream[wv], s_runs[wv], s_tab[wv], s_full[wv], s_pref[wv], s_ost[wv], s_reg, wv
+#define LANES_LDS s_stream[wv], s_runs[wv], s_tab[wv], s_full[wv], s_pref[wv], s_ost[wv], s_reg, s_vpool[wv], wv
 
 template <int W, int I, int SEGS, bool IRR, int MODE, int NL, bool BS>
 __global__ __launch_bounds__(LANES_WAVES * 64, LANES_WPS)
@@ -808,7 +852,7 @@
 void classify_lanes_mixed_k(utk_image im, const uint8_t *__restrict__ bases, const uint64_t *__restrict__ off, const uint32_t *__restrict__ len,
                             uint32_t n_reads, int do_rc, utree_result *__restrict__ out, utk_workspace ws, uint32_t max_cls) {
     LANES_PROLOGUE(W)
-    lanes_body<W, I, 1, IRR, 0, NL, BS>(im, bases, off, len, n_reads, do_rc, out, ws, 1u, LANES_LDS);
+    lanes_body<W, I, 1, IRR, 0, NL, BS, false>(im, bases, off, len, n_reads, do_rc, out, ws, 1u, LANES_LDS);
     if (max_cls >= 1u) lanes_body<W, I, 2, IRR, 1, NL, BS>(im, bases, off, len, n_reads, do_rc, out, ws, 1u, LANES_LDS);
     if (max_cls >= 2u) lanes_body<W, I, 4, IRR, 1, NL, BS>(im, bases, off, len, n_reads, do_rc, out, ws, 2u, LANES_LDS);
     if (max_cls >= 3u) lanes_body<W, I, 8, IRR, 1, NL, BS>(im, bases, off, len, n_reads, do_rc, out, ws, 3u, LANES_LDS);
diff --git a/utree_amd/csrc/utree_internal.h b/utree_amd/csrc/utree_internal.h
--- a/utree_amd/csrc/utree_internal.h
+++ b/utree_amd/csrc/utree_internal.h
@@ -128,6 +128,7 @@
     uint32_t *cls_list;
     uint32_t cls_stride;
     uint64_t ltally_base;
+    uint32_t vote_fused;
 } utk_workspace;
 
 int utk_classify_short(const utk_image *im, const uint8_t *d_bases, const uint64_t *d_off, const uint32_t *d_len,
diff --git a/utree_amd/csrc/vote_common.hpp b/utree_amd/csrc/vote_common.hpp
--- /dev/null
+++ b/utree_amd/csrc/vote_common.hpp
@@ -0,0 +1,201 @@
+#pragma once
+#include <stdint.h>
+
+#if defined(__HIPCC__)
+#define UTK_HD __host__ __device__ __forceinline__
+#else
+#define UTK_HD inline
+#endif
+
+namespace utk {
+
+UTK_HD uint32_t cut_of(uint32_t x) {
+    uint32_t c = x - x / 4;
+    c += (x >> 1) >= c;
+    return c;
+}
+
+struct VRec { uint64_t w[4]; };
+UTK_HD uint32_t v_pid(const VRec &v, uint32_t t) { return (uint32_t)((t < 4 ? v.w[0] : v.w[1]) >> (16u * (t & 3u))) & 0xFFFFu; }
+UTK_HD uint32_t v_end(const VRec &v, uint32_t t) { return (uint32_t)(v.w[2] >> (8u * t)) & 0xFFu; }
+UTK_HD bool v_exists(const VRec &v, uint32_t t) { return ((uint32_t)v.w[3] >> t) & 1u; }
+UTK_HD bool v_more(const VRec &v, uint32_t t) { return ((uint32_t)v.w[3] >> (8u + t)) & 1u; }
+UTK_HD bool v_us(const VRec &v, uint32_t t) { return ((uint32_t)v.w[3] >> (16u + t)) & 1u; }
+UTK_HD uint32_t v_len(const VRec &v) { return (uint32_t)(v.w[3] >> 32) & 0xFFu; }
+UTK_HD uint32_t v_ix(const VRec &v) { return (uint32_t)(v.w[3] >> 48); }
+
+UTK_HD uint32_t v_shared(const VRec &pv, const VRec &lv) {
+    const uint64_t d0 = pv.w[0] ^ lv.w[0], d1 = pv.w[1] ^ lv.w[1];
+    const uint32_t same = d0 ? (uint32_t)__builtin_ctzll(d0) >> 4 : 4u + (d1 ? (uint32_t)__builtin_ctzll(d1) >> 4 : 4u);
+    const uint32_t both = ((uint32_t)(pv.w[3] & lv.w[3]) >> 8) & 0xFFu;
+    const uint32_t semis = (uint32_t)__builtin_ctz(~both);
+    return same < semis ? same : semis;
+}
+
+UTK_HD bool vote2_closed(const VRec &pv, const VRec &lv, uint32_t n0, uint32_t n1, uint32_t F, uint32_t (&res)[6]) {
+    constexpr uint32_t NONE = 0xFFFFFFFFu;
+    uint32_t cutoff = cut_of(F), orun = F, run = n0, dv = NONE;
+    const uint32_t t = v_shared(pv, lv);
+    if (t) dv = v_end(pv, t - 1u);
+    bool aside = false, stopped = false;
+    if (t >= 8u || !v_exists(pv, t) || (dv == NONE && v_end(pv, 0) == 0u && !v_more(pv, 0))) aside = true;
+    else {
+        bool differs = true;
+        if (v_exists(lv, t) && v_pid(lv, t) == v_pid(pv, t)) {
+            const bool a = v_more(pv, t), b = v_more(lv, t);
+            if (a == b) return false;
+            if (!a || v_us(pv, t)) { aside = true; differs = false; }
+        } else if (v_us(pv, t) || !v_exists(lv, t)) return false;
+        if (differs) {
+            if (run >= cutoff) stopped = true;
+            else run = n1;
+        }
+    }
+    if (aside) { run = n1; orun -= n0; cutoff = cut_of(orun); }
+    const VRec &last = stopped ? pv : lv;
+    const uint32_t n_last = stopped ? n0 : n1;
+    if (run >= cutoff && n_last >= cutoff) dv = 0xFFFFFFFEu;
+    const uint32_t len_last = v_len(last);
+    res[0] = v_ix(last);
+    res[1] = dv == NONE ? (uint32_t)-1 : dv == 0xFFFFFFFEu ? (uint32_t)-2 : (dv < len_last ? dv : len_last);
+    res[2] = F; res[3] = 2u; res[4] = run; res[5] = orun;
+    return true;
+}
+
+}
+
+#if defined(__HIPCC__)
+#include "device_common.hpp"
+
+namespace utk {
+
+constexpr int32_t VOTE_CUT_PENDING = -3;
+constexpr int32_t VOTE_RANK_PENDING = -4;
+
+__device__ __forceinline__ void vote_store(utree_result *out, uint32_t label, int32_t cut, uint32_t found, uint32_t uix, uint32_t sl, uint32_t ol) {
+    uint32_t *o = (uint32_t *)out;
+    o[0] = label; o[1] = (uint32_t)cut; o[2] = found; o[3] = uix; o[4] = sl; o[5] = ol;
+}
+
+__device__ __forceinline__ void label16(const char *s, uint32_t p, uint64_t &x, uint64_t &y) {
+    typedef unsigned long long u64x2 __attribute__((ext_vector_type(2), aligned(1)));
+    const u64x2 v = *(const u64x2 *)(s + p);
+    x = v.x; y = v.y;
+}
+
+__device__ __forceinline__ uint64_t stop_flags(uint64_t x1, uint64_t x2) {
+    const uint64_t semi = x1 ^ 0x3B3B3B3B3B3B3B3Bull, d = x1 ^ x2;
+    uint64_t m = (((x1 - 0x0101010101010101ull) & ~x1) | ((semi - 0x0101010101010101ull) & ~semi)) & 0x8080808080808080ull;
+    m |= (((d & 0x7F7F7F7F7F7F7F7Full) + 0x7F7F7F7F7F7F7F7Full) | d) & 0x8080808080808080ull;
+    return m;
+}
+
+__device__ __forceinline__ void pair_scan(const char *s1, const char *s2, uint32_t start, uint32_t &td, uint32_t &a, uint32_t &b, uint32_t &before) {
+    uint32_t base = start, prevlast = start ? (uint32_t)(uint8_t)s1[start - 1] : 0u;
+    for (;;) {
+        uint64_t x1, y1, x2, y2;
+        label16(s1, base, x1, y1); label16(s2, base, x2, y2);
+        uint64_t m = stop_flags(x1, x2);
+        if (!m) { prevlast = (uint32_t)(x1 >> 56); base += 8; x1 = y1; x2 = y2; m = stop_flags(x1, x2); }
+        if (m) {
+            const uint32_t idx = (uint32_t)(__builtin_ctzll(m) >> 3);
+            td = base + idx;
+            a = (uint32_t)(x1 >> (8 * idx)) & 0xFFu; b = (uint32_t)(x2 >> (8 * idx)) & 0xFFu;
+            before = idx ? ((uint32_t)(x1 >> (8 * idx - 8)) & 0xFFu) : prevlast;
+            return;
+        }
+        prevlast = (uint32_t)(x1 >> 56); base += 8;
+    }
+}
+
+__device__ __forceinline__ VRec vrec(const uint64_t *vt, uint32_t rank) {
+    typedef unsigned long long u64x2 __attribute__((ext_vector_type(2)));
+    const u64x2 *p = (const u64x2 *)(vt + (size_t)rank * 4);
+    const u64x2 a = p[0], b = p[1];
+    VRec v; v.w[0] = a.x; v.w[1] = a.y; v.w[2] = b.x; v.w[3] = b.y;
+    return v;
+}
+
+__device__ __forceinline__ void vote_table(const utk_image &im, utree_result *out_r, const uint64_t *T, uint32_t F, uint32_t uix) {
+    const uint64_t *vt = im.vote_tab;
+    const char *blob = im.label_blob;
+    const uint32_t *loff = im.label_off;
+    constexpr uint32_t NONE = 0xFFFFFFFFu;
+    uint32_t cutoff = cut_of(F);
+    uint32_t st = 0, ed = uix, dv = NONE, t = 0, orun = F, sl, ol;
+    uint32_t ix_last, n_last, len_last;
+    for (;;) {
+        const uint64_t t_st = T[st];
+        VRec pv = vrec(vt, (uint32_t)t_st);
+        const uint64_t t_ed = ed - 1u == st ? t_st : T[ed - 1u];
+        const VRec lv = ed - 1u == st ? pv : vrec(vt, (uint32_t)t_ed);
+        {
+            const uint32_t L = v_shared(pv, lv);
+            if (L > t) { dv = v_end(pv, L - 1u); t = L; }
+        }
+        uint32_t run = (uint32_t)(t_st >> 32), td = dv, c1 = run, rp = (uint32_t)t_st;
+        bool td_is_end = false;
+        bool stopped = false;
+        for (uint32_t z = st + 1; z < ed; ++z) {
+            const bool is_last = z == ed - 1u;
+            const uint64_t tz = is_last ? t_ed : T[z];
+            const uint32_t nz = (uint32_t)(tz >> 32), rc = (uint32_t)tz;
+            const VRec cv = is_last ? lv : vrec(vt, rc);
+            bool aside = false, stop = false;
+            if (t >= 8u || !v_exists(pv, t) || (dv == NONE && v_end(pv, 0) == 0u && !v_more(pv, 0))) aside = true;
+            else {
+                uint32_t a, b, before;
+                bool known = true;
+                if (v_exists(cv, t) && v_pid(cv, t) == v_pid(pv, t)) {
+                    td = v_end(pv, t); td_is_end = true;
+                    a = v_more(pv, t) ? ';' : 0u; b = v_more(cv, t) ? ';' : 0u; before = v_us(pv, t) ? '_' : 'x';
+                } else if (v_us(pv, t) || !v_exists(cv, t)) {
+                    pair_scan(blob + loff[rp], blob + loff[rc], dv + 1u, td, a, b, before);
+                    td_is_end = td == v_end(pv, t);
+                } else { a = 'a'; b = 'b'; before = 'x'; known = false; }
+                if (a == b) run += nz;
+                else if ((!a && b == ';') || ((a == ';' || !a) && before == '_')) aside = true;
+                else if (run >= cutoff) {
+                    ed = z; stop = true;
+                    if (!known) {
+                        pair_scan(blob + loff[rp], blob + loff[rc], dv + 1u, td, a, b, before);
+                        td_is_end = td == v_end(pv, t);
+                    }
+                } else { run = nz; st = z; }
+            }
+            if (aside) {
+                run = nz; st = z;
+                orun -= c1;
+                cutoff = cut_of(orun);
+            }
+            if (stop) { stopped = true; break; }
+            pv = cv; c1 = nz; rp = rc;
+        }
+        ix_last = stopped ? v_ix(pv) : v_ix(lv);
+        n_last = stopped ? c1 : (uint32_t)(t_ed >> 32);
+        len_last = stopped ? v_len(pv) : v_len(lv);
+        sl = run; ol = orun;
+        if (run < cutoff) break;
+        if (st + 1 >= ed) {
+            if (n_last >= cutoff) dv = 0xFFFFFFFEu;
+            break;
+        }
+        orun = run; cutoff = cut_of(run);
+        if (td != dv) { dv = td; if (td_is_end) ++t; }
+    }
+    int32_t cut;
+    if (dv == NONE) cut = -1;
+    else if (dv == 0xFFFFFFFEu) cut = -2;
+    else cut = (int32_t)(dv < len_last ? dv : len_last);
+    vote_store(out_r, ix_last, cut, F, uix, sl, ol);
+}
+
+__device__ __forceinline__ void vote_pending(const utk_image &im, utree_result *out_r, const uint64_t *tally) {
+    const uint32_t *res = (const uint32_t *)out_r;
+    const int32_t cut = (int32_t)res[1];
+    if (cut == VOTE_RANK_PENDING) { uint32_t *o = (uint32_t *)out_r; o[0] = im.rank2ix[res[0]]; o[1] = (uint32_t)-2; }
+    else if (cut == VOTE_CUT_PENDING) vote_table(im, out_r, tally + ((uint64_t)res[4] | ((uint64_t)res[5] << 32)), res[2], res[3]);
+}
+
+}
+#endif
diff --git a/utree_amd/lib.py b/utree_amd/lib.py
--- a/utree_amd/lib.py
+++ b/utree_amd/lib.py
@@ -165,7 +165,7 @@
 def kernel_source_sha256() -> str:
     import hashlib
     h = hashlib.sha256()
-    for f in ("kernels.hip", "lanes_kernel.hip", "lanes_core.hpp", "lanes_part.hip", "wave_common.hpp", "device_common.hpp", "utree_internal.h", "Makefile"):
+    for f in ("kernels.hip", "lanes_kernel.hip", "lanes_core.hpp", "lanes_part.hip", "wave_common.hpp", "device_common.hpp", "vote_common.hpp", "utree_internal.h", "Makefile"):
         with open(os.path.join(_HERE, "csrc", f), "rb") as fh:
             h.update(f.encode() + b"\0" + fh.read() + b"\0")
     return h.hexdigest()
```

Result: no change. 2.301 billion reads/s (median of 2 runs) (-1.3%).
